# eglrp/PSBA

Measured on AMD Instinct MI355X. Metric: M-observations/sec through Jacobian+Schur build+solve (ms/LM-iter in ms_per_step), higher is better.
Workload: dtype f64; 1 GPU; venice-shaped; n_cams=52, n_pts=64053, n_obs=345364, lm=levmar, TR hand-off disabled, parallelism=points sharded x1

## Files before the change

include/psba_hip.h:

```cpp
#ifndef PSBA_HIP_H
#define PSBA_HIP_H

#ifdef __cplusplus
extern "C" {
#endif

typedef struct psba_ctx *psba_handle;

#define PSBA_OK 0
#define PSBA_NOT_SPD 1
#define PSBA_SINGULAR_V 2
#define PSBA_PCG_MAXIT 4
#define PSBA_E_INVALID (-1)
#define PSBA_E_HIP (-2)
#define PSBA_E_RCCL (-3)
#define PSBA_E_IO (-4)
#define PSBA_E_NOMEM (-5)
#define PSBA_E_STATE (-6)

#define PSBA_ITER_TURN_TO_LM 1
#define PSBA_ITER_TURN_TO_TR 2
#define PSBA_ITER_CONTINUE 3
#define PSBA_ITER_ERR 4
#define PSBA_ITER_DP_NO_CHANGE 5
#define PSBA_ITER_ERR_SMALL_ENOUGH 6
#define PSBA_ITER_PASS 7

#define PSBA_PARAMS_CUR 0
#define PSBA_PARAMS_NEW 1

int psba_create(int device, psba_handle *out);
int psba_destroy(psba_handle h);
const char *psba_last_error(psba_handle h);
const char *psba_version(void);

int psba_upload_problem(psba_handle h, int nCams, int n3Dpts, int n2Dprojs, const double *Kparas,
                        const double *impts, const double *initrot, const double *camsEx,
                        const double *pts3D, const int *iidx, const int *jidx);
int psba_set_params(psba_handle h, const double *camsEx, const double *pts3D);
int psba_reset_params(psba_handle h);
int psba_get_params(psba_handle h, int which, double *camsEx, double *pts3D);
int psba_get_dims(psba_handle h, int *nCams, int *n3Dpts, int *n2Dprojs);

#define PSBA_CAMERA_FIXED_K 0
#define PSBA_CAMERA_FREE_K 1
#define PSBA_CAMERA_FREE_KD 2
int psba_set_camera_model(psba_handle h, int model);
int psba_camera_block(psba_handle h, int *cnp);

int psba_set_intrinsics_mask(psba_handle h, const unsigned char free10[10]);
int psba_intrinsics_mask(psba_handle h, unsigned char out10[10]);

int psba_set_distortion(psba_handle h, const double *kc);
int psba_set_obs_covariance(psba_handle h, const double *cov);
int psba_lens_model(psba_handle h, int *has_distortion, int *has_covariance);

#define PSBA_LOSS_NONE 0
#define PSBA_LOSS_HUBER 1
#define PSBA_LOSS_CAUCHY 2
#define PSBA_LOSS_SOFT_L1 3
int psba_set_robust_loss(psba_handle h, int kind, double scale);
int psba_robust_loss(psba_handle h, int *kind, double *scale);
int psba_obs_sq_residuals(psba_handle h, int which, double *s);

int psba_set_fixed(psba_handle h, const unsigned char *fixed_cams, const unsigned char *fixed_pts);
int psba_fixed_counts(psba_handle h, int *n_fixed_cams, int *n_fixed_pts);
int psba_schur_path(psba_handle h, int *path);


int psba_residual(psba_handle h, int which, double *cost);
int psba_linearize(psba_handle h, double coeff, double coeff_g);
int psba_max_diag(psba_handle h, double *out);
int psba_begin(psba_handle h, double coeff, double coeff_g, double *cost, double *max_diag);
int psba_schur_assemble(psba_handle h, double mu);
int psba_schur_reduce(psba_handle h);
int psba_schur_solve(psba_handle h);

typedef struct {
  int status;
  double dp_l2;
  double gain_den;
  double new_cost;
  double newp_l2;
} psba_try_scalars;

int psba_backsub(psba_handle h, double mu, psba_try_scalars *out);
int psba_backsub_async(psba_handle h, double mu);
int psba_linearize_ahead(psba_handle h);
int psba_backsub_wait(psba_handle h, psba_try_scalars *out);
int psba_accept(psba_handle h);

int psba_compute_exQT(psba_handle h, int which, double *ex);
int psba_compute_jacobiQT(psba_handle h, double *jac_A, double *jac_B);
int psba_compute_U(psba_handle h, double coeff, double *out);
int psba_compute_V(psba_handle h, double coeff, double *out);
int psba_maxElmOfUV(psba_handle h, double *out);
int psba_update_UV(psba_handle h, double mu, double *U, double *V);
int psba_restore_UVdiag(psba_handle h);
int psba_compute_Vinv(psba_handle h, double *Vinv );
int psba_compute_Wblks(psba_handle h, double coeff, double *Wblks);
int psba_compute_Yblks(psba_handle h, double *Yblks);
int psba_compute_S(psba_handle h, double *S );
int psba_compute_g(psba_handle h, double coeff, double *g);
int psba_compute_ea(psba_handle h, double *ea);
int psba_SPDinv_matVec(psba_handle h, double *dpa);
int psba_compute_eb(psba_handle h, double *eb );
int psba_compute_dpb(psba_handle h, double *dp );
int psba_compute_newp(psba_handle h, double *new_p );
int psba_update_p(psba_handle h, double *p );

typedef struct {
  int max_iter;
  int tr_handoff;
  int verbose;
  int log_cap;
  int start_itno;
  double init_mu;
  double stop_cost;
} psba_lm_options;

typedef struct {
  int flag;
  int iters;
  int tries;
  double init_err, final_err, mu0, mu_final;
  int n_log;
  double seconds;
  int pcg_unconverged;
} psba_lm_result;

void psba_lm_default_options(psba_lm_options *o);
int psba_levmar(psba_handle h, const psba_lm_options *opts, psba_lm_result *res, double *log);

int psba_compute_Jmultiply(psba_handle h, const double *x, double *Jmul);
int psba_jmul_dots(psba_handle h, const double *x1, const double *x2, double dots[3]);
int psba_allreduce_scalars(psba_handle h, double *v, int n);
int psba_get_gradient(psba_handle h, double *g);
int psba_get_dp(psba_handle h, double *dp);
int psba_set_step(psba_handle h, const double *dp);
int psba_cholmod_lambda(psba_handle h, int reassemble, double *lambda, double *info3);

typedef struct {
  int max_iter;
  int start_itno;
  int verbose;
  int log_cap;
  double init_lambda;
} psba_tr_options;

typedef struct {
  int flag;
  int iters;
  int tries;
  int chol_fail;
  double init_err, final_err, lambda, delta;
  int n_log;
  double seconds;
} psba_tr_result;

void psba_tr_default_options(psba_tr_options *o);
int psba_trust_region(psba_handle h, const psba_tr_options *opts, psba_tr_result *res, double *log);

typedef struct {
  int flag, iters, lm_calls, tr_calls;
  double init_err, final_err, seconds;
} psba_solve_result;
int psba_solve(psba_handle h, int max_iter, int verbose, psba_solve_result *res);

int psba_partition_points(int n3Dpts, const int *iidx, int n2Dprojs, int nranks, int *pt_begin);
int psba_comm_unique_id(void *id128);
int psba_comm_init(psba_handle h, int nranks, int rank, const void *id128);
int psba_comm_rank(psba_handle h, int *nranks, int *rank);
int psba_set_rank_layout(psba_handle h, int nranks, int rank);
int psba_reduce_buffer_size(psba_handle h, long long *n_doubles);
int psba_get_reduce_buffer(psba_handle h, double *out);
int psba_set_reduce_buffer(psba_handle h, const double *in);

typedef struct {
  int nCams, n3Dpts, n2Dprojs;
  double *Kparas, *impts, *initrot, *camsEx, *pts3D;
  int *iidx, *jidx;
} psba_problem;
int psba_read_problem(const char *cams_file, const char *pts_file, const double *fixedK,
                      psba_problem *out);
void psba_free_problem(psba_problem *p);
typedef struct {
  psba_problem base;
  double *kc, *cov;
} psba_problem_ex;
int psba_read_problem_ex(const char *cams_file, const char *pts_file, const double *fixedK, psba_problem_ex *out);
void psba_free_problem_ex(psba_problem_ex *p);
int psba_write_problem(const char *cams_file, const char *pts_file, int nCams, int n3Dpts, int n2Dprojs,
                       const double *Kparas, const double *initrot, const double *camsEx, const double *pts3D,
                       const double *impts, const int *iidx, const int *jidx, int with_K);
int psba_convert_bal(const char *bal_file, const char *cams_out, const char *pts_out, double *max_abs_k);
int psba_convert_bal_kd(const char *bal_file, const char *cams_out, const char *pts_out);

#define PSBA_K_LINEARIZE 0
#define PSBA_K_SCHUR 1
#define PSBA_K_CHOLESKY 2
#define PSBA_K_BACKSUB 3
#define PSBA_K_RESIDUAL 4
#define PSBA_K_ALLREDUCE 5
#define PSBA_K_SCHUR_REDUCE 6
#define PSBA_K_COUNT 7
int psba_profile_enable(psba_handle h, int on);
int psba_profile_reset(psba_handle h);
int psba_profile_get(psba_handle h, int kernel, double *total_ms, int *launches);
int psba_algorithmic_bytes(psba_handle h, int kernel, double *bytes);

#define PSBA_SOLVER_DENSE 0
#define PSBA_SOLVER_PCG 1
int psba_set_solver(psba_handle h, int solver, double tol, int max_iter);
int psba_pcg_info(psba_handle h, int *iters, double *relres, long long *blocks, long long *dense_blocks);
int psba_get_sparse_S(psba_handle h, int *jk, double *val, double *ea);
int psba_set_sparse_S(psba_handle h, const double *val, const double *ea);
int psba_sparse_pattern(int nCams, int n3Dpts, int n2Dprojs, const int *iidx, const int *jidx, unsigned char *flags);
int psba_set_sparse_pattern(psba_handle h, const unsigned char *flags, long long n);

int psba_chol_dist_shape(psba_handle h, int *n32, int *NB, int *sharded);
int psba_chol_shape(psba_handle h, int *out8);
int psba_chol_dist_exchange_plan(int n32, int NB, int nranks, int JE, long long *out4, int cap);
int psba_chol_dist_begin(psba_handle h);
int psba_chol_dist_superpanel(psba_handle h, int J);
int psba_chol_dist_block(psba_handle h, int B, int set, double *buf, long long *n_doubles);
int psba_chol_dist_finish(psba_handle h);

typedef struct psba_schur_plan *psba_schur_plan_t;
psba_schur_plan_t psba_schur_plan_create(int nCams, int n3Dpts, int n2Dprojs, const int *iidx,
                                         const int *jidx);
int psba_schur_plan_info(psba_schur_plan_t p, long long info[8]);
int psba_schur_plan_copy(psba_schur_plan_t p, unsigned long long *items, long long *wg,
                         int *blockpos, int *glo);
void psba_schur_plan_destroy(psba_schur_plan_t p);

typedef struct psba_owner_plan *psba_owner_plan_t;
psba_owner_plan_t psba_owner_plan_create(int nCams, int n3Dpts, int n2Dprojs, const int *iidx, const int *jidx,
                                         const unsigned char *pattern);
int psba_owner_plan_info(psba_owner_plan_t p, long long info[4]);
int psba_owner_plan_copy(psba_owner_plan_t p, long long *waves, int *units, int *prod, int *blocks, int *diag_slot);
void psba_owner_plan_destroy(psba_owner_plan_t p);

typedef struct psba_blockprod_plan *psba_blockprod_plan_t;
// ... 21 lines not shown
```

psba_amd/build.py:

```python
import os
import subprocess
import sys

HERE = os.path.dirname(os.path.abspath(__file__))
CSRC = os.path.join(HERE, "csrc")
SOURCES = ["psba_api.cpp", "schur_plan.cpp", "lm_loop.cpp", "tr_loop.cpp", "sba_io.cpp", "kernels_linearize.hip",
           "kernels_tr.hip",
           "kernels_schur.hip", "kernels_freek.hip", "kernels_freekd.hip", "blockprod_plan.cpp", "kernels_chol.hip", "kernels_pcg.hip", "kernels_chol_graph.hip", "kernels_backsub.hip"]
EXPERIMENTS = bool(os.environ.get("PSBA_BUILD_EXPERIMENTS"))
if EXPERIMENTS:
    SOURCES += ["kernels_schur_ring.hip", "schur_ring_plan.cpp", "kernels_schur_modes.hip"]
OUT = os.path.join(HERE, "libpsba_hip_exp.so" if EXPERIMENTS else "libpsba_hip.so")
HEADERS = ["psba_internal.h", "dev_buf.h", "camera_model.h", "chol_factor32.h", "schur_common.h", "schur_lds_args.h", os.path.join("..", "..", "include", "psba_hip.h")]
ROCM = os.environ.get("ROCM_PATH", "/opt/rocm")
FLAGS = ["--offload-arch=gfx950", "-O3", "-std=c++17", "-fPIC", "-munsafe-fp-atomics",
         "-Wall", "-Wno-unused-result", "-x", "hip"] + (["-DPSBA_BUILD_EXPERIMENTS"] if EXPERIMENTS else [])


def _stale(obj, deps):
    if not os.path.exists(obj):
        return True
    t = os.path.getmtime(obj)
    return any(os.path.getmtime(d) > t for d in deps)


def build(force=False, verbose=False):
    hipcc = os.path.join(ROCM, "bin", "hipcc")
    objdir = os.path.join(HERE, "build_exp" if EXPERIMENTS else "build")
    os.makedirs(objdir, exist_ok=True)
    hdrs = [os.path.normpath(os.path.join(CSRC, h)) for h in HEADERS]
    objs, rebuilt = [], False
    for s in SOURCES:
        src = os.path.join(CSRC, s)
        obj = os.path.join(objdir, s + ".o")
        objs.append(obj)
        if force or _stale(obj, [src] + hdrs):
            cmd = [hipcc] + FLAGS + ["-c", src, "-o", obj]
            if verbose:
                print(" ".join(cmd), flush=True)
            subprocess.check_call(cmd)
            rebuilt = True
    if rebuilt or not os.path.exists(OUT):
        cmd = [hipcc, "--offload-arch=gfx950", "-shared", "-fPIC", "-o", OUT] + objs + [
            "-L" + os.path.join(ROCM, "lib"), "-lrccl", "-Wl,-rpath," + os.path.join(ROCM, "lib")]
        if verbose:
            print(" ".join(cmd), flush=True)
        subprocess.check_call(cmd)
    return OUT


if __name__ == "__main__":
    print(build(force="--force" in sys.argv, verbose=True))
```

psba_amd/capi.py:

```python
import ctypes as C
import os

import numpy as np

_HERE = os.path.dirname(os.path.abspath(__file__))
lib_path = os.environ.get("PSBA_LIB") or os.path.join(_HERE, "libpsba_hip.so")

if not os.path.exists(lib_path):
    raise ImportError(
        f"{lib_path} is missing: build the HIP extension first (python -m psba_amd.build, or "
        "__graft_entry__.build()). psba_amd has no CPU fallback.")
lib = C.CDLL(lib_path)

PSBA_OK, PSBA_NOT_SPD, PSBA_SINGULAR_V = 0, 1, 2
PARAMS_CUR, PARAMS_NEW = 0, 1
LOSS_NONE, LOSS_HUBER, LOSS_CAUCHY, LOSS_SOFT_L1 = 0, 1, 2, 3
CAMERA_FIXED_K, CAMERA_FREE_K, CAMERA_FREE_KD = 0, 1, 2
INTRINSICS_BAL = (1, 0, 0, 0, 0, 1, 1, 0, 0, 0)
ITER_TURN_TO_LM, ITER_TURN_TO_TR, ITER_CONTINUE, ITER_ERR = 1, 2, 3, 4
ITER_DP_NO_CHANGE, ITER_ERR_SMALL_ENOUGH, ITER_PASS = 5, 6, 7
K_LINEARIZE, K_SCHUR, K_CHOLESKY, K_BACKSUB, K_RESIDUAL, K_ALLREDUCE, K_SCHUR_REDUCE = range(7)
KERNEL_NAMES = ["linearize", "schur", "cholesky", "backsub", "residual", "allreduce", "schur_reduce"]

_h = C.c_void_p
_dp = C.POINTER(C.c_double)
_ip = C.POINTER(C.c_int)


class TryScalars(C.Structure):
    _fields_ = [("status", C.c_int), ("dp_l2", C.c_double), ("gain_den", C.c_double),
                ("new_cost", C.c_double), ("newp_l2", C.c_double)]


class LmOptions(C.Structure):
    _fields_ = [("max_iter", C.c_int), ("tr_handoff", C.c_int), ("verbose", C.c_int),
                ("log_cap", C.c_int), ("start_itno", C.c_int), ("init_mu", C.c_double),
                ("stop_cost", C.c_double)]


class LmResult(C.Structure):
    _fields_ = [("flag", C.c_int), ("iters", C.c_int), ("tries", C.c_int), ("init_err", C.c_double),
                ("final_err", C.c_double), ("mu0", C.c_double), ("mu_final", C.c_double),
                ("n_log", C.c_int), ("seconds", C.c_double), ("pcg_unconverged", C.c_int)]


class TrOptions(C.Structure):
    _fields_ = [("max_iter", C.c_int), ("start_itno", C.c_int), ("verbose", C.c_int), ("log_cap", C.c_int),
                ("init_lambda", C.c_double)]


class TrResult(C.Structure):
    _fields_ = [("flag", C.c_int), ("iters", C.c_int), ("tries", C.c_int), ("chol_fail", C.c_int),
                ("init_err", C.c_double), ("final_err", C.c_double), ("lambda_", C.c_double),
                ("delta", C.c_double), ("n_log", C.c_int), ("seconds", C.c_double)]


class SolveResult(C.Structure):
    _fields_ = [("flag", C.c_int), ("iters", C.c_int), ("lm_calls", C.c_int), ("tr_calls", C.c_int),
                ("init_err", C.c_double), ("final_err", C.c_double), ("seconds", C.c_double)]


class CProblem(C.Structure):
    _fields_ = [("nCams", C.c_int), ("n3Dpts", C.c_int), ("n2Dprojs", C.c_int), ("Kparas", _dp),
                ("impts", _dp), ("initrot", _dp), ("camsEx", _dp), ("pts3D", _dp), ("iidx", _ip),
                ("jidx", _ip)]


class CProblemEx(C.Structure):
    _fields_ = [("base", CProblem), ("kc", _dp), ("cov", _dp)]


SIGNATURES = [
    ("psba_create", C.c_int, [C.c_int, C.POINTER(_h)]),
    ("psba_destroy", C.c_int, [_h]),
    ("psba_last_error", C.c_char_p, [_h]),
    ("psba_version", C.c_char_p, []),
    ("psba_upload_problem", C.c_int, [_h, C.c_int, C.c_int, C.c_int, _dp, _dp, _dp, _dp, _dp, _ip, _ip]),
    ("psba_set_params", C.c_int, [_h, _dp, _dp]),
    ("psba_reset_params", C.c_int, [_h]),
    ("psba_get_params", C.c_int, [_h, C.c_int, _dp, _dp]),
    ("psba_get_dims", C.c_int, [_h, _ip, _ip, _ip]),
    ("psba_schur_path", C.c_int, [_h, C.POINTER(C.c_int)]),
    ("psba_residual", C.c_int, [_h, C.c_int, _dp]),
    ("psba_linearize", C.c_int, [_h, C.c_double, C.c_double]),
    ("psba_max_diag", C.c_int, [_h, _dp]),
    ("psba_begin", C.c_int, [_h, C.c_double, C.c_double, _dp, _dp]),
    ("psba_schur_assemble", C.c_int, [_h, C.c_double]),
    ("psba_schur_reduce", C.c_int, [_h]),
    ("psba_schur_solve", C.c_int, [_h]),
    ("psba_backsub", C.c_int, [_h, C.c_double, C.POINTER(TryScalars)]),
    ("psba_backsub_async", C.c_int, [_h, C.c_double]),
    ("psba_linearize_ahead", C.c_int, [_h]),
    ("psba_backsub_wait", C.c_int, [_h, C.POINTER(TryScalars)]),
    ("psba_accept", C.c_int, [_h]),
    ("psba_compute_exQT", C.c_int, [_h, C.c_int, _dp]),
    ("psba_compute_jacobiQT", C.c_int, [_h, _dp, _dp]),
    ("psba_compute_U", C.c_int, [_h, C.c_double, _dp]),
    ("psba_compute_V", C.c_int, [_h, C.c_double, _dp]),
    ("psba_maxElmOfUV", C.c_int, [_h, _dp]),
    ("psba_update_UV", C.c_int, [_h, C.c_double, _dp, _dp]),
    ("psba_restore_UVdiag", C.c_int, [_h]),
    ("psba_compute_Vinv", C.c_int, [_h, _dp]),
    ("psba_compute_Wblks", C.c_int, [_h, C.c_double, _dp]),
    ("psba_compute_Yblks", C.c_int, [_h, _dp]),
    ("psba_compute_S", C.c_int, [_h, _dp]),
    ("psba_compute_g", C.c_int, [_h, C.c_double, _dp]),
    ("psba_compute_ea", C.c_int, [_h, _dp]),
    ("psba_SPDinv_matVec", C.c_int, [_h, _dp]),
    ("psba_compute_eb", C.c_int, [_h, _dp]),
    ("psba_compute_dpb", C.c_int, [_h, _dp]),
    ("psba_compute_newp", C.c_int, [_h, _dp]),
    ("psba_update_p", C.c_int, [_h, _dp]),
    ("psba_lm_default_options", None, [C.POINTER(LmOptions)]),
    ("psba_levmar", C.c_int, [_h, C.POINTER(LmOptions), C.POINTER(LmResult), _dp]),
    ("psba_partition_points", C.c_int, [C.c_int, _ip, C.c_int, C.c_int, _ip]),
    ("psba_comm_unique_id", C.c_int, [C.c_void_p]),
    ("psba_comm_init", C.c_int, [_h, C.c_int, C.c_int, C.c_void_p]),
    ("psba_comm_rank", C.c_int, [_h, _ip, _ip]),
    ("psba_set_rank_layout", C.c_int, [_h, C.c_int, C.c_int]),
    ("psba_reduce_buffer_size", C.c_int, [_h, C.POINTER(C.c_longlong)]),
    ("psba_get_reduce_buffer", C.c_int, [_h, _dp]),
    ("psba_set_reduce_buffer", C.c_int, [_h, _dp]),
    ("psba_read_problem", C.c_int, [C.c_char_p, C.c_char_p, _dp, C.POINTER(CProblem)]),
    ("psba_free_problem", None, [C.POINTER(CProblem)]),
    ("psba_profile_enable", C.c_int, [_h, C.c_int]),
    ("psba_profile_reset", C.c_int, [_h]),
    ("psba_profile_get", C.c_int, [_h, C.c_int, _dp, _ip]),
    ("psba_algorithmic_bytes", C.c_int, [_h, C.c_int, _dp]),
    ("psba_compute_Jmultiply", C.c_int, [_h, _dp, _dp]),
    ("psba_jmul_dots", C.c_int, [_h, _dp, _dp, _dp]),
    ("psba_get_gradient", C.c_int, [_h, _dp]),
    ("psba_get_dp", C.c_int, [_h, _dp]),
    ("psba_set_step", C.c_int, [_h, _dp]),
    ("psba_cholmod_lambda", C.c_int, [_h, C.c_int, _dp, _dp]),
    ("psba_tr_default_options", None, [C.POINTER(TrOptions)]),
    ("psba_trust_region", C.c_int, [_h, C.POINTER(TrOptions), C.POINTER(TrResult), _dp]),
    ("psba_solve", C.c_int, [_h, C.c_int, C.c_int, C.POINTER(SolveResult)]),
    ("psba_write_problem", C.c_int, [C.c_char_p, C.c_char_p, C.c_int, C.c_int, C.c_int, _dp, _dp, _dp, _dp, _dp, _ip, _ip, C.c_int]),
    ("psba_convert_bal", C.c_int, [C.c_char_p, C.c_char_p, C.c_char_p, _dp]),
    ("psba_allreduce_scalars", C.c_int, [_h, _dp, C.c_int]),
    ("psba_set_solver", C.c_int, [_h, C.c_int, C.c_double, C.c_int]),
    ("psba_pcg_info", C.c_int, [_h, _ip, _dp, C.POINTER(C.c_longlong), C.POINTER(C.c_longlong)]),
    ("psba_get_sparse_S", C.c_int, [_h, _ip, _dp, _dp]),
    ("psba_set_sparse_S", C.c_int, [_h, _dp, _dp]),
    ("psba_sparse_pattern", C.c_int, [C.c_int, C.c_int, C.c_int, _ip, _ip, C.POINTER(C.c_ubyte)]),
    ("psba_set_sparse_pattern", C.c_int, [_h, C.POINTER(C.c_ubyte), C.c_longlong]),
    ("psba_set_camera_model", C.c_int, [_h, C.c_int]),
    ("psba_camera_block", C.c_int, [_h, _ip]),
    ("psba_set_distortion", C.c_int, [_h, _dp]),
    ("psba_set_obs_covariance", C.c_int, [_h, _dp]),
    ("psba_lens_model", C.c_int, [_h, _ip, _ip]),
    ("psba_set_robust_loss", C.c_int, [_h, C.c_int, C.c_double]),
    ("psba_robust_loss", C.c_int, [_h, _ip, _dp]),
    ("psba_obs_sq_residuals", C.c_int, [_h, C.c_int, _dp]),
    ("psba_set_fixed", C.c_int, [_h, C.POINTER(C.c_ubyte), C.POINTER(C.c_ubyte)]),
    ("psba_fixed_counts", C.c_int, [_h, _ip, _ip]),
    ("psba_read_problem_ex", C.c_int, [C.c_char_p, C.c_char_p, _dp, C.POINTER(CProblemEx)]),
    ("psba_free_problem_ex", None, [C.POINTER(CProblemEx)]),
    ("psba_convert_bal_kd", C.c_int, [C.c_char_p, C.c_char_p, C.c_char_p]),
    ("psba_chol_dist_exchange_plan", C.c_int, [C.c_int, C.c_int, C.c_int, C.c_int, C.POINTER(C.c_longlong), C.c_int]),
    ("psba_chol_dist_shape", C.c_int, [_h, _ip, _ip, _ip]),
    ("psba_chol_shape", C.c_int, [_h, _ip]),
    ("psba_chol_dist_begin", C.c_int, [_h]),
    ("psba_chol_dist_superpanel", C.c_int, [_h, C.c_int]),
    ("psba_chol_dist_block", C.c_int, [_h, C.c_int, C.c_int, _dp, C.POINTER(C.c_longlong)]),
    ("psba_chol_dist_finish", C.c_int, [_h]),
    ("psba_schur_plan_create", C.c_void_p, [C.c_int, C.c_int, C.c_int, _ip, _ip]),
    ("psba_schur_plan_info", C.c_int, [C.c_void_p, C.POINTER(C.c_longlong)]),
    ("psba_schur_plan_copy", C.c_int, [C.c_void_p, C.POINTER(C.c_ulonglong), C.POINTER(C.c_longlong), _ip, _ip]),
    ("psba_schur_plan_destroy", None, [C.c_void_p]),
    ("psba_owner_plan_create", C.c_void_p, [C.c_int, C.c_int, C.c_int, _ip, _ip, C.POINTER(C.c_ubyte)]),
    ("psba_owner_plan_info", C.c_int, [C.c_void_p, C.POINTER(C.c_longlong)]),
    ("psba_owner_plan_copy", C.c_int, [C.c_void_p, C.POINTER(C.c_longlong), _ip, _ip, _ip, _ip]),
    ("psba_owner_plan_destroy", None, [C.c_void_p]),
    ("psba_set_intrinsics_mask", C.c_int, [_h, C.POINTER(C.c_ubyte)]),
    ("psba_intrinsics_mask", C.c_int, [_h, C.POINTER(C.c_ubyte)]),
    ("psba_blockprod_plan_create", C.c_void_p, [C.c_int, C.c_int, C.c_int, _ip, _ip, C.c_int]),
    ("psba_blockprod_plan_info", C.c_int, [C.c_void_p, C.POINTER(C.c_longlong)]),
    ("psba_blockprod_plan_copy", C.c_int, [C.c_void_p, _ip, _ip, _ip]),
    ("psba_blockprod_plan_destroy", None, [C.c_void_p]),
]
EXPERIMENT_SIGNATURES = [
    ("psba_ring_plan_create", C.c_void_p, [C.c_int, C.c_int, C.c_int, _ip, _ip]),
    ("psba_ring_plan_info", C.c_int, [C.c_void_p, C.POINTER(C.c_longlong)]),
    ("psba_ring_plan_copy", C.c_int, [C.c_void_p, C.POINTER(C.c_longlong), _ip, C.POINTER(C.c_uint), _ip, _ip, _ip, _ip, _ip]),
    ("psba_ring_plan_destroy", None, [C.c_void_p]),
]
HAS_EXPERIMENTS = hasattr(lib, "psba_ring_plan_create")
for _name, _res, _args in SIGNATURES + (EXPERIMENT_SIGNATURES if HAS_EXPERIMENTS else []):
    _f = getattr(lib, _name)
    _f.restype = _res
    _f.argtypes = _args


class PsbaError(RuntimeError):
    def __init__(self, code, msg):
        super().__init__(f"psba error {code}: {msg}")
        self.code = code


def _d(a):
    return None if a is None else a.ctypes.data_as(_dp)


def _i(a):
    return None if a is None else a.ctypes.data_as(_ip)


def _c(a, dt=np.float64):
    return np.ascontiguousarray(a, dtype=dt)


class Problem(dict):
    """K[nC,5] initrot[nC,4] cams[nC,6] pts[nP,3] impts[nO,2] iidx[nO] jidx[nO] nC nP nO.
    Optional: kc[nC,5], cov[nO,2,2] (read_problem_ex); fixed_cams[nC], fixed_pts[nP] (masks for Psba.set_fixed)."""


def sparse_pattern(prob):
    nC = int(prob["nC"])
    flags = np.zeros(nC * (nC + 1) // 2, dtype=np.uint8)
    ii = np.ascontiguousarray(prob["iidx"], dtype=np.int32)
    jj = np.ascontiguousarray(prob["jidx"], dtype=np.int32)
    rc = lib.psba_sparse_pattern(nC, int(prob["nP"]), int(prob["nO"]), _i(ii), _i(jj),
                                 flags.ctypes.data_as(C.POINTER(C.c_ubyte)))
    if rc != 0:
        raise PsbaError(rc, "psba_sparse_pattern failed")
    return flags


def _problem_from(cp):
    nC, nP, nO = cp.nCams, cp.n3Dpts, cp.n2Dprojs
    arr = lambda p, n, shape: np.ctypeslib.as_array(p, shape=(n,)).copy().reshape(shape)
    return Problem(K=arr(cp.Kparas, 5 * nC, (nC, 5)), initrot=arr(cp.initrot, 4 * nC, (nC, 4)),
                  cams=arr(cp.camsEx, 6 * nC, (nC, 6)), pts=arr(cp.pts3D, 3 * nP, (nP, 3)),
                  impts=arr(cp.impts, 2 * nO, (nO, 2)), iidx=arr(cp.iidx, nO, (nO,)).astype(np.int32),
                  jidx=arr(cp.jidx, nO, (nO,)).astype(np.int32), nC=nC, nP=nP, nO=nO)


def read_problem(cams_file, pts_file, fixedK=None):
    cp = CProblem()
    k = None if fixedK is None else _c(fixedK)
    rc = lib.psba_read_problem(os.fsencode(cams_file), os.fsencode(pts_file), _d(k), C.byref(cp))
    if rc != 0:
        raise PsbaError(rc, f"psba_read_problem({cams_file}, {pts_file}) failed")
    out = _problem_from(cp)
    lib.psba_free_problem(C.byref(cp))
    return out
# ... 186 lines not shown
            self._h = _h()

    def __del__(self):
        try:
            self.close()
        except Exception:
            pass

    def _ck(self, rc):
        if rc < 0:
            raise PsbaError(rc, lib.psba_last_error(self._h).decode())
        return rc

    def set_camera_model(self, model):
        self._ck(lib.psba_set_camera_model(self._h, int(model)))

    def set_intrinsics_mask(self, free=None):
        if free is None:
            return self._ck(lib.psba_set_intrinsics_mask(self._h, None))
        m = np.ascontiguousarray((np.asarray(free).reshape(-1) != 0).astype(np.uint8))
        if m.size != 10:
            raise PsbaError(-1, f"set_intrinsics_mask: {m.size} flags for 10 intrinsics")
        self._ck(lib.psba_set_intrinsics_mask(self._h, m.ctypes.data_as(C.POINTER(C.c_ubyte))))

    def intrinsics_mask(self):
        m = np.zeros(10, dtype=np.uint8)
        self._ck(lib.psba_intrinsics_mask(self._h, m.ctypes.data_as(C.POINTER(C.c_ubyte))))
        return tuple(int(v) for v in m)

    def set_distortion(self, kc):
        k = None if kc is None else _c(kc).reshape(-1)
        if k is not None and k.size != 5 * self.nC:
            raise PsbaError(-1, f"set_distortion: {k.size} values for {self.nC} cameras (5 each)")
        self._ck(lib.psba_set_distortion(self._h, _d(k)))

    def set_obs_covariance(self, cov):
        c = None if cov is None else _c(cov).reshape(-1)
        if c is not None and c.size != 4 * self.nO:
            raise PsbaError(-1, f"set_obs_covariance: {c.size} values for {self.nO} observations (4 each)")
        self._ck(lib.psba_set_obs_covariance(self._h, _d(c)))

    def lens_model(self):
        d, c = C.c_int(), C.c_int()
        self._ck(lib.psba_lens_model(self._h, C.byref(d), C.byref(c)))
        return bool(d.value), bool(c.value)

    def set_robust_loss(self, kind, scale=1.0):
        self._ck(lib.psba_set_robust_loss(self._h, int(kind), float(scale)))

    def robust_loss(self):
        k, c = C.c_int(), C.c_double()
        self._ck(lib.psba_robust_loss(self._h, C.byref(k), C.byref(c)))
        return k.value, c.value

    def set_fixed(self, cams=None, pts=None):
        def mask(a, n, what):
            if a is None:
                return None
            m = (np.asarray(a).reshape(-1) != 0).astype(np.uint8)
            if m.size != n:
                raise PsbaError(-1, f"set_fixed: {m.size} flags for {n} {what}")
            return np.ascontiguousarray(m)
        c, p = mask(cams, self.nC, "cameras"), mask(pts, self.nP, "points")
        ub = C.POINTER(C.c_ubyte)
        self._ck(lib.psba_set_fixed(self._h, None if c is None else c.ctypes.data_as(ub),
                                    None if p is None else p.ctypes.data_as(ub)))

    def fixed_counts(self):
        c, p = C.c_int(), C.c_int()
        self._ck(lib.psba_fixed_counts(self._h, C.byref(c), C.byref(p)))
        return c.value, p.value

    def obs_sq_residuals(self, which=PARAMS_CUR):
        return self._out(lib.psba_obs_sq_residuals, self.nO, which)[1]

    def camera_block(self):
        n = C.c_int()
        self._ck(lib.psba_camera_block(self._h, C.byref(n)))
        return n.value

    def upload_problem(self, prob):
        self.nC, self.nP, self.nO = int(prob["nC"]), int(prob["nP"]), int(prob["nO"])
        self.cnp = self.camera_block()
        self.nA, self.nB = self.cnp * self.nC, 3 * self.nP
        self.nT = self.nA + self.nB
        a = [_c(prob[k]).reshape(-1) for k in ("K", "impts", "initrot", "cams", "pts")]
        ii, jj = _c(prob["iidx"], np.int32), _c(prob["jidx"], np.int32)
        self._ck(lib.psba_upload_problem(self._h, self.nC, self.nP, self.nO, _d(a[0]), _d(a[1]),
                                         _d(a[2]), _d(a[3]), _d(a[4]), _i(ii), _i(jj)))

    def set_params(self, cams, pts):
        c, p = _c(cams).reshape(-1), _c(pts).reshape(-1)
        self._ck(lib.psba_set_params(self._h, _d(c), _d(p)))

    def reset_params(self):
        self._ck(lib.psba_reset_params(self._h))

    def get_params(self, which=PARAMS_CUR):
        c, p = np.empty(self.nA), np.empty(self.nB)
        self._ck(lib.psba_get_params(self._h, which, _d(c), _d(p)))
        return c.reshape(self.nC, self.cnp), p.reshape(self.nP, 3)

    def schur_path(self):
        v = C.c_int()
        self._ck(lib.psba_schur_path(self._h, C.byref(v)))
        return v.value

    def residual(self, which=PARAMS_CUR):
        v = C.c_double()
        self._ck(lib.psba_residual(self._h, which, C.byref(v)))
        return v.value

    def linearize(self, coeff=1.0, coeff_g=1.0):
        self._ck(lib.psba_linearize(self._h, coeff, coeff_g))

    def begin(self, coeff=1.0, coeff_g=1.0):
        c, m = C.c_double(), C.c_double()
        self._ck(lib.psba_begin(self._h, coeff, coeff_g, C.byref(c), C.byref(m)))
        return c.value, m.value

    def max_diag(self):
        v = C.c_double()
        self._ck(lib.psba_max_diag(self._h, C.byref(v)))
        return v.value

    def schur_assemble(self, mu):
        self._ck(lib.psba_schur_assemble(self._h, mu))

    def schur_reduce(self):
        self._ck(lib.psba_schur_reduce(self._h))

    def schur_solve(self):
        return self._ck(lib.psba_schur_solve(self._h))

    def backsub(self, mu):
        s = TryScalars()
        self._ck(lib.psba_backsub(self._h, mu, C.byref(s)))
        return s

    def backsub_async(self, mu):
        self._ck(lib.psba_backsub_async(self._h, mu))

    def linearize_ahead(self):
        self._ck(lib.psba_linearize_ahead(self._h))

    def backsub_wait(self):
        s = TryScalars()
        self._ck(lib.psba_backsub_wait(self._h, C.byref(s)))
        return s

    def accept(self):
        self._ck(lib.psba_accept(self._h))

    def _out(self, fn, n, *pre):
        out = np.empty(n)
        rc = self._ck(fn(self._h, *pre, _d(out)))
        return rc, out

    def compute_exQT(self, which=PARAMS_CUR):
        return self._out(lib.psba_compute_exQT, 2 * self.nO, which)[1]

    def compute_jacobiQT(self):
        JA, JB = np.empty(12 * self.nO), np.empty(6 * self.nO)
        self._ck(lib.psba_compute_jacobiQT(self._h, _d(JA), _d(JB)))
        return JA, JB

    def compute_U(self, coeff=1.0):
        return self._out(lib.psba_compute_U, 36 * self.nC, coeff)[1]

    def compute_V(self, coeff=1.0):
        return self._out(lib.psba_compute_V, 9 * self.nP, coeff)[1]

    def maxElmOfUV(self):
        v = C.c_double()
        self._ck(lib.psba_maxElmOfUV(self._h, C.byref(v)))
        return v.value

    def update_UV(self, mu):
        U, V = np.empty(36 * self.nC), np.empty(9 * self.nP)
        self._ck(lib.psba_update_UV(self._h, mu, _d(U), _d(V)))
        return U, V

    def restore_UVdiag(self):
        self._ck(lib.psba_restore_UVdiag(self._h))

    def compute_Vinv(self):
        return self._out(lib.psba_compute_Vinv, 9 * self.nP)

    def compute_Wblks(self, coeff=1.0):
        return self._out(lib.psba_compute_Wblks, 18 * self.nO, coeff)[1]

    def compute_Yblks(self):
        return self._out(lib.psba_compute_Yblks, 18 * self.nO)[1]

    def compute_S(self):
        return self._out(lib.psba_compute_S, self.nA * self.nA)[1].reshape(self.nA, self.nA)

    def compute_g(self, coeff=1.0):
        return self._out(lib.psba_compute_g, self.nT, coeff)[1]

    def compute_ea(self):
        return self._out(lib.psba_compute_ea, self.nA)[1]

    def SPDinv_matVec(self):
        return self._out(lib.psba_SPDinv_matVec, self.nA)

    def compute_eb(self):
        return self._out(lib.psba_compute_eb, self.nB)[1]

    def compute_dpb(self):
        return self._out(lib.psba_compute_dpb, self.nT)[1]

    def compute_newp(self):
        return self._out(lib.psba_compute_newp, self.nT)[1]

    def update_p(self):
        return self._out(lib.psba_update_p, self.nT)[1]

    def levmar(self, max_iter=50, tr_handoff=False, verbose=False, log_cap=512, start_itno=0, init_mu=0.0,
               stop_cost=0.0):
        opts = LmOptions(max_iter, int(tr_handoff), int(verbose), log_cap, start_itno, init_mu, stop_cost)
        res = LmResult()
        log = np.zeros((max(log_cap, 1), 5))
        self._ck(lib.psba_levmar(self._h, C.byref(opts), C.byref(res), _d(log)))
        return res, log[: res.n_log].copy()

    def set_solver(self, solver, tol=0.0, max_iter=0):
        self._ck(lib.psba_set_solver(self._h, int(solver), float(tol), int(max_iter)))

    def pcg_info(self):
        it, rr, nb, nd = C.c_int(), C.c_double(), C.c_longlong(), C.c_longlong()
        self._ck(lib.psba_pcg_info(self._h, C.byref(it), C.byref(rr), C.byref(nb), C.byref(nd)))
        return it.value, rr.value, nb.value, nd.value

    def get_sparse_S(self):
        nb = self.pcg_info()[2]
        jk = np.empty((nb, 2), dtype=np.int32)
        val = np.empty((nb, 6, 6))
        ea = np.empty(6 * self.nC)
        self._ck(lib.psba_get_sparse_S(self._h, _i(jk), _d(val), _d(ea)))
        return jk, val, ea

    def set_sparse_S(self, val, ea):
        val = np.ascontiguousarray(val, dtype=np.float64)
        ea = np.ascontiguousarray(ea, dtype=np.float64)
        self._ck(lib.psba_set_sparse_S(self._h, _d(val), _d(ea)))

    def set_sparse_pattern(self, flags):
        flags = np.ascontiguousarray(flags, dtype=np.uint8)
        self._ck(lib.psba_set_sparse_pattern(self._h, flags.ctypes.data_as(C.POINTER(C.c_ubyte)), flags.size))

    def chol_dist_shape(self):
        n32, nb, sh = C.c_int(), C.c_int(), C.c_int()
        self._ck(lib.psba_chol_dist_shape(self._h, C.byref(n32), C.byref(nb), C.byref(sh)))
        return n32.value, nb.value, bool(sh.value)

    def chol_shape(self):
        out = (C.c_int * 8)()
        self._ck(lib.psba_chol_shape(self._h, out))
        keys = ("n32", "fused", "fused2", "blocked", "NB", "diag_only", "lookahead", "single")
        return {k: (int(v) if k in ("n32", "NB") else bool(v)) for k, v in zip(keys, out)}

    def chol_dist_begin(self):
        self._ck(lib.psba_chol_dist_begin(self._h))

    def chol_dist_superpanel(self, J):
        self._ck(lib.psba_chol_dist_superpanel(self._h, int(J)))

    def chol_dist_get_block(self, B):
        n = C.c_longlong()
        self._ck(lib.psba_chol_dist_block(self._h, int(B), 0, None, C.byref(n)))
        buf = np.empty(n.value)
        self._ck(lib.psba_chol_dist_block(self._h, int(B), 0, _d(buf), C.byref(n)))
        return buf

    def chol_dist_set_block(self, B, buf):
        n = C.c_longlong()
        self._ck(lib.psba_chol_dist_block(self._h, int(B), 1, _d(_c(buf)), C.byref(n)))

    def chol_dist_finish(self):
        self._ck(lib.psba_chol_dist_finish(self._h))

    def compute_Jmultiply(self, x):
        return self._out(lambda h, out: lib.psba_compute_Jmultiply(h, _d(_c(x)), out), 2 * self.nO)[1]

    def jmul_dots(self, x1, x2=None):
        out = np.empty(3)
        a1 = _c(x1)
        a2 = None if x2 is None else _c(x2)
        self._ck(lib.psba_jmul_dots(self._h, _d(a1), _d(a2), _d(out)))
        return out

    def get_gradient(self):
        return self._out(lib.psba_get_gradient, self.nT)[1]

    def get_dp(self):
        return self._out(lib.psba_get_dp, self.nT)[1]

    def set_step(self, dp):
        self._ck(lib.psba_set_step(self._h, _d(_c(dp))))

    def cholmod_lambda(self, reassemble=True):
        lam, info = C.c_double(), np.empty(3)
        self._ck(lib.psba_cholmod_lambda(self._h, int(reassemble), C.byref(lam), _d(info)))
        return lam.value, info

# ... 58 lines not shown
```

psba_amd/csrc/kernels_linearize.hip:

```cpp
#include <cstdlib>

#include "camera_model.h"
#include "psba_internal.h"

namespace psba {

struct LinArgs {
  const double *camconst, *cams, *pts, *impts;
  const int *iidx, *jidx, *ptr;
  const int4 *tile_desc;
  double *W, *PV, *campart;
  double *camacc;
  double *dbg_ex, *dbg_JA, *dbg_JB;
  double coeff, coeff_g;
  int nC, nTiles;
  int mode;
  const double *pub_src;
  double *pub_dst;
  double pub_stamp;
  const double *kc, *wl;
};

template <bool DUMP, bool GACC, int LM>
__global__ __launch_bounds__(TILE_OBS) void k_linearize(LinArgs p, RobustLoss rl, FixedMask fm) {
  __shared__ double sBE[TILE_OBS][9];
  __shared__ double sW[(TILE_OBS / 2) * 19];
  extern __shared__ double sAcc[];
  const int tid = threadIdx.x;
  if (p.pub_dst && blockIdx.x == 0) {
    if (tid < NSCAL) p.pub_dst[tid] = p.pub_src[tid];
    __threadfence_system();
    __syncthreads();
    if (tid == 0) p.pub_dst[NSCAL] = p.pub_stamp;
  }
  const int nAcc = GACC ? 0 : p.nC * CAM_ACC;
  for (int t = tid; t < nAcc; t += TILE_OBS) sAcc[t] = 0.0;
  __syncthreads();

  int tile = blockIdx.x;
  int4 dsc = tile < p.nTiles ? p.tile_desc[tile] : make_int4(0, 0, 0, 0);
  int i = 0, j = 0;
  if (dsc.z + tid < dsc.w) {
    i = p.iidx[dsc.z + tid];
    j = p.jidx[dsc.z + tid];
  }
  for (; tile < p.nTiles; tile += gridDim.x) {
    const int p0 = dsc.x, p1 = dsc.y, o0 = dsc.z, o1 = dsc.w;
    const int a = o0 + tid;
    const int tn = tile + gridDim.x;
    const int4 dn = tn < p.nTiles ? p.tile_desc[tn] : make_int4(0, 0, 0, 0);
    constexpr int NTASK = (9 * TILE_PTS + TILE_OBS - 1) / TILE_OBS;
    int pb[NTASK][2];
#pragma unroll
    for (int u = 0; u < NTASK; u++) {
      const int ip = (tid + u * TILE_OBS) / 9;
      pb[u][0] = ip < p1 - p0 ? p.ptr[p0 + ip] - o0 : 0;
      pb[u][1] = ip < p1 - p0 ? p.ptr[p0 + ip + 1] - o0 : 0;
    }
    double Wv[18];
    if (a < o1) {
      double cc[9], cam[6], M[3], e[2], A[12], B[6], kc[5], wl[3];
#pragma unroll
      for (int k = 0; k < 9; k++) cc[k] = p.camconst[9 * j + k];
#pragma unroll
      for (int k = 0; k < 6; k++) cam[k] = p.cams[6 * j + k];
#pragma unroll
      for (int k = 0; k < 3; k++) M[k] = p.pts[3 * i + k];
      lens_load_kc<LM>(p.kc, j, kc);
      lens_load_w<LM>(p.wl, a, wl);
      const double2 m = reinterpret_cast<const double2 *>(p.impts)[a];
      lens_linearize<LM>(cc, cam, M, kc, wl, rl, m.x, m.y, e, A, B);
      fix_mask<LM>(fix_load<LM>(fm, i, j), A, B);
      if (DUMP) {
        p.dbg_ex[2 * a] = e[0];
        p.dbg_ex[2 * a + 1] = e[1];
#pragma unroll
        for (int k = 0; k < 12; k++) p.dbg_JA[12 * (size_t)a + k] = A[k];
#pragma unroll
        for (int k = 0; k < 6; k++) p.dbg_JB[6 * (size_t)a + k] = B[k];
      }
#pragma unroll
      for (int r = 0; r < 6; r++)
#pragma unroll
        for (int c = 0; c < 3; c++) Wv[3 * r + c] = p.coeff * (A[r] * B[c] + A[6 + r] * B[3 + c]);
      if (tid < TILE_OBS / 2) {
        double *w = sW + 19 * tid;
#pragma unroll
        for (int k = 0; k < 18; k++) w[k] = Wv[k];
      }
#pragma unroll
      for (int k = 0; k < 6; k++) sBE[tid][k] = B[k];
      sBE[tid][6] = e[0];
      sBE[tid][7] = e[1];
      double *acc = sAcc + CAM_ACC * (size_t)j;
      int k = 0;
      if (p.mode != 1 && !GACC) {
#pragma unroll
      for (int r = 0; r < 6; r++)
#pragma unroll
        for (int c = r; c < 6; c++) atomicAdd(&acc[k++], A[r] * A[c] + A[6 + r] * A[6 + c]);
#pragma unroll
      for (int r = 0; r < 6; r++) atomicAdd(&acc[21 + r], A[r] * e[0] + A[6 + r] * e[1]);
      }
    }
    __syncthreads();
    if (p.mode != 2) {
      double *dst = p.W + 18 * (size_t)o0;
      const int n = 18 * (o1 - o0 < TILE_OBS / 2 ? o1 - o0 : TILE_OBS / 2);
      for (int t = tid; t < n; t += TILE_OBS) dst[t] = sW[19 * (t / 18) + t % 18];
    }
#pragma unroll
    for (int u = 0; u < NTASK; u++) {
      const int t = tid + u * TILE_OBS;
      if (t >= 9 * (p1 - p0) || p.mode == 3) continue;
      const int comp = t % 9;
      const int b0 = pb[u][0], b1 = pb[u][1];
      int r, c1, c2;
      if (comp < 6) {
        r = comp < 3 ? 0 : (comp < 5 ? 1 : 2);
        const int c = comp < 3 ? comp : (comp < 5 ? comp - 2 : 2);
        c1 = c;
        c2 = 3 + c;
      } else {
        r = comp - 6;
        c1 = 6;
        c2 = 7;
      }
      double acc = 0.0;
      for (int b = b0; b < b1; b++) {
        const double *B = sBE[b];
        acc += B[r] * B[c1] + B[3 + r] * B[c2];
      }
      p.PV[9 * (size_t)p0 + t] = (comp < 6 ? p.coeff : p.coeff_g) * acc;
    }
    if (o1 - o0 > TILE_OBS / 2) {
      __syncthreads();
      if (tid >= TILE_OBS / 2 && a < o1) {
        double *w = sW + 19 * (tid - TILE_OBS / 2);
#pragma unroll
        for (int k = 0; k < 18; k++) w[k] = Wv[k];
      }
      __syncthreads();
      if (p.mode != 2) {
        double *dst = p.W + 18 * (size_t)(o0 + TILE_OBS / 2);
        const int n = 18 * (o1 - o0 - TILE_OBS / 2);
        for (int t = tid; t < n; t += TILE_OBS) dst[t] = sW[19 * (t / 18) + t % 18];
      }
    }
    dsc = dn;
    i = j = 0;
    if (dsc.z + tid < dsc.w) {
      i = p.iidx[dsc.z + tid];
      j = p.jidx[dsc.z + tid];
    }
    __syncthreads();
  }
  if (GACC) return;
  double *slab = p.campart + (size_t)blockIdx.x * nAcc;
  for (int t = tid; t < nAcc; t += TILE_OBS) slab[t] = sAcc[t];
}

template <bool DUMP, bool GACC, int LM>
__global__ __launch_bounds__(TILE_OBS) void k_linearize2(LinArgs p, RobustLoss rl, FixedMask fm) {
  __shared__ double sW[TILE_OBS * 19];
  __shared__ double sCarV[TILE_OBS / 64][9];
  __shared__ int sCarP[TILE_OBS / 64][3];
  extern __shared__ double sAcc[];
  const int tid = threadIdx.x, lane = tid & 63, wave = tid >> 6;
  if (p.pub_dst && blockIdx.x == 0) {
    if (tid < NSCAL) p.pub_dst[tid] = p.pub_src[tid];
    __threadfence_system();
    __syncthreads();
    if (tid == 0) p.pub_dst[NSCAL] = p.pub_stamp;
  }
  const int nAcc = GACC ? 0 : p.nC * CAM_ACC;
  for (int t = tid; t < nAcc; t += TILE_OBS) sAcc[t] = 0.0;
  __syncthreads();

  int tile = blockIdx.x;
  int4 dsc = tile < p.nTiles ? p.tile_desc[tile] : make_int4(0, 0, 0, 0);
  int i = 0, j = 0;
  double cc[9], cam[6], M[3], kc[5], wl[3];
  double2 m = make_double2(0.0, 0.0);
  int fx = 0;
  if (dsc.z + tid < dsc.w) {
    i = p.iidx[dsc.z + tid];
    j = p.jidx[dsc.z + tid];
    fx = fix_load<LM>(fm, i, j);
#pragma unroll
    for (int k = 0; k < 9; k++) cc[k] = p.camconst[9 * j + k];
#pragma unroll
    for (int k = 0; k < 6; k++) cam[k] = p.cams[6 * j + k];
#pragma unroll
    for (int k = 0; k < 3; k++) M[k] = p.pts[3 * (size_t)i + k];
    lens_load_kc<LM>(p.kc, j, kc);
    lens_load_w<LM>(p.wl, dsc.z + tid, wl);
    m = reinterpret_cast<const double2 *>(p.impts)[dsc.z + tid];
  }
  for (; tile < p.nTiles; tile += gridDim.x) {
    const int o0 = dsc.z, o1 = dsc.w;
    const int a = o0 + tid;
    const bool act = a < o1;
    const int tn = tile + gridDim.x;
    const int4 dn = tn < p.nTiles ? p.tile_desc[tn] : make_int4(0, 0, 0, 0);
    double v[9];
#pragma unroll
    for (int k = 0; k < 9; k++) v[k] = 0.0;
    const int pi = act ? i : -1 - tid;
    const int jc = j;
    if (act) {
      double e[2], A[12], B[6];
      lens_linearize<LM>(cc, cam, M, kc, wl, rl, m.x, m.y, e, A, B);
      fix_mask<LM>(fx, A, B);
      if (DUMP) {
        p.dbg_ex[2 * (size_t)a] = e[0];
        p.dbg_ex[2 * (size_t)a + 1] = e[1];
#pragma unroll
        for (int k = 0; k < 12; k++) p.dbg_JA[12 * (size_t)a + k] = A[k];
#pragma unroll
        for (int k = 0; k < 6; k++) p.dbg_JB[6 * (size_t)a + k] = B[k];
      }
      double *w = sW + 19 * tid;
#pragma unroll
      for (int r = 0; r < 6; r++)
#pragma unroll
        for (int c = 0; c < 3; c++) w[3 * r + c] = p.coeff * (A[r] * B[c] + A[6 + r] * B[3 + c]);
      int q = 0;
#pragma unroll
      for (int r = 0; r < 3; r++)
#pragma unroll
        for (int c = r; c < 3; c++) v[q++] = B[r] * B[c] + B[3 + r] * B[3 + c];
#pragma unroll
      for (int r = 0; r < 3; r++) v[6 + r] = B[r] * e[0] + B[3 + r] * e[1];
      if (p.mode != 1 && !GACC) {
        double *acc = sAcc + CAM_ACC * (size_t)jc;
        int k = 0;
#pragma unroll
        for (int r = 0; r < 6; r++)
#pragma unroll
          for (int c = r; c < 6; c++) atomicAdd(&acc[k++], A[r] * A[c] + A[6 + r] * A[6 + c]);
#pragma unroll
        for (int r = 0; r < 6; r++) atomicAdd(&acc[21 + r], A[r] * e[0] + A[6 + r] * e[1]);
      }
    }
    i = j = 0;
    if (dn.z + tid < dn.w) {
      i = p.iidx[dn.z + tid];
      j = p.jidx[dn.z + tid];
      fx = fix_load<LM>(fm, i, j);
#pragma unroll
      for (int k = 0; k < 9; k++) cc[k] = p.camconst[9 * j + k];
#pragma unroll
      for (int k = 0; k < 6; k++) cam[k] = p.cams[6 * j + k];
#pragma unroll
      for (int k = 0; k < 3; k++) M[k] = p.pts[3 * (size_t)i + k];
      lens_load_kc<LM>(p.kc, j, kc);
      lens_load_w<LM>(p.wl, dn.z + tid, wl);
      m = reinterpret_cast<const double2 *>(p.impts)[dn.z + tid];
    }
    if (p.mode != 3) {
#pragma unroll
      for (int d = 1; d < 64; d <<= 1) {
        const int pu = __shfl_up(pi, d, 64);
        const bool ok = lane >= d && pu == pi;
        if (!__any(ok)) break;
#pragma unroll
        for (int k = 0; k < 9; k++) {
          const double vu = __shfl_up(v[k], d, 64);
          v[k] += ok ? vu : 0.0;
        }
      }
    }
    const int pn = __shfl_down(pi, 1, 64);
    const int p_first = __shfl(pi, 0, 64), p_last = __shfl(pi, 63, 64);
    if (lane == 63) {
#pragma unroll
      for (int k = 0; k < 9; k++) sCarV[wave][k] = v[k];
      sCarP[wave][0] = p_first;
      sCarP[wave][1] = p_last;
      sCarP[wave][2] = p_first == p_last;
    }
    __syncthreads();
    if (p.mode != 2) {
      double *dst = p.W + 18 * (size_t)o0;
      const int n = 18 * (o1 - o0);
      for (int t = tid; t < n; t += TILE_OBS) dst[t] = sW[19 * (t / 18) + t % 18];
    }
    if (act && p.mode != 3) {
      const bool cont = lane == 63 && wave + 1 < TILE_OBS / 64 && sCarP[wave + 1][0] == pi;
      const bool tail = lane == 63 ? !cont : pn != pi;
      if (tail) {
        if (pi == p_first) {
          for (int w2 = wave - 1; w2 >= 0 && sCarP[w2][1] == pi; w2--) {
#pragma unroll
            for (int k = 0; k < 9; k++) v[k] += sCarV[w2][k];
            if (!sCarP[w2][2]) break;
          }
        }
        double *pv = p.PV + 9 * (size_t)pi;
#pragma unroll
        for (int k = 0; k < 9; k++) pv[k] = (k < 6 ? p.coeff : p.coeff_g) * v[k];
      }
    }
    dsc = dn;
    __syncthreads();
  }
  if (GACC) return;
  double *slab = p.campart + (size_t)blockIdx.x * nAcc;
  for (int t = tid; t < nAcc; t += TILE_OBS) slab[t] = sAcc[t];
}

template <bool DUMP, bool GACC, int LM>
__global__ __launch_bounds__(TILE_OBS) void k_linearize_long(LinArgs p, const int *long_pts, double *cam_slab, RobustLoss rl, FixedMask fm) {
  __shared__ double sRed[TILE_OBS / 64][9];
  const int tid = threadIdx.x, i = long_pts[blockIdx.x];
  const int o0 = p.ptr[i], o1 = p.ptr[i + 1];
  double M[3], acc[9];
#pragma unroll
  for (int k = 0; k < 3; k++) M[k] = p.pts[3 * (size_t)i + k];
#pragma unroll
  for (int k = 0; k < 9; k++) acc[k] = 0.0;
  for (int a = o0 + tid; a < o1; a += TILE_OBS) {
    const int j = p.jidx[a];
    double cc[9], cam[6], e[2], A[12], B[6], kc[5], wl[3];
#pragma unroll
    for (int k = 0; k < 9; k++) cc[k] = p.camconst[9 * (size_t)j + k];
#pragma unroll
    for (int k = 0; k < 6; k++) cam[k] = p.cams[6 * (size_t)j + k];
    lens_load_kc<LM>(p.kc, j, kc);
    lens_load_w<LM>(p.wl, a, wl);
    const double2 m = reinterpret_cast<const double2 *>(p.impts)[a];
    lens_linearize<LM>(cc, cam, M, kc, wl, rl, m.x, m.y, e, A, B);
    fix_mask<LM>(fix_load<LM>(fm, i, j), A, B);
    if (DUMP) {
      p.dbg_ex[2 * (size_t)a] = e[0];
      p.dbg_ex[2 * (size_t)a + 1] = e[1];
#pragma unroll
      for (int k = 0; k < 12; k++) p.dbg_JA[12 * (size_t)a + k] = A[k];
#pragma unroll
      for (int k = 0; k < 6; k++) p.dbg_JB[6 * (size_t)a + k] = B[k];
    }
    double *w = p.W + 18 * (size_t)a;
#pragma unroll
    for (int r = 0; r < 6; r++)
#pragma unroll
      for (int c = 0; c < 3; c++) w[3 * r + c] = p.coeff * (A[r] * B[c] + A[6 + r] * B[3 + c]);
    int k = 0;
#pragma unroll
    for (int r = 0; r < 3; r++)
#pragma unroll
      for (int c = r; c < 3; c++) acc[k++] += B[r] * B[c] + B[3 + r] * B[3 + c];
#pragma unroll
    for (int r = 0; r < 3; r++) acc[6 + r] += B[r] * e[0] + B[3 + r] * e[1];
    if (!GACC) {
      double *cs = cam_slab + CAM_ACC * (size_t)j;
      int q = 0;
#pragma unroll
      for (int r = 0; r < 6; r++)
#pragma unroll
        for (int c = r; c < 6; c++) atomicAdd(&cs[q++], A[r] * A[c] + A[6 + r] * A[6 + c]);
#pragma unroll
      for (int r = 0; r < 6; r++) atomicAdd(&cs[21 + r], A[r] * e[0] + A[6 + r] * e[1]);
    }
  }
#pragma unroll
  for (int k = 0; k < 9; k++) {
    double v = acc[k];
#pragma unroll
    for (int off = 32; off > 0; off >>= 1) v += __shfl_down(v, off, 64);
    if ((tid & 63) == 0) sRed[tid >> 6][k] = v;
  }
  __syncthreads();
  if (tid < 9) {
    double v = 0.0;
    for (int q = 0; q < TILE_OBS / 64; q++) v += sRed[q][tid];
    p.PV[9 * (size_t)i + tid] = (tid < 6 ? p.coeff : p.coeff_g) * v;
  }
}

template <int LM>
__global__ __launch_bounds__(256) void k_cam_sums(LinArgs p, const int *cam_obs, const int4 *units, int nUnits, RobustLoss rl, FixedMask fm) {
  const int lane = threadIdx.x & 63;
  const int u = blockIdx.x * 4 + (threadIdx.x >> 6);
  if (u >= nUnits) return;
  const int4 un = units[u];
  const int j = un.x;
  double cc[9], cam[6], acc[CAM_ACC], kc[5];
#pragma unroll
  for (int k = 0; k < 9; k++) cc[k] = p.camconst[9 * (size_t)j + k];
#pragma unroll
  for (int k = 0; k < 6; k++) cam[k] = p.cams[6 * (size_t)j + k];
  lens_load_kc<LM>(p.kc, j, kc);
#pragma unroll
  for (int k = 0; k < CAM_ACC; k++) acc[k] = 0.0;
  for (int t = un.y + lane; t < un.z; t += 64) {
    const int a = cam_obs[t];
    const int i = p.iidx[a];
    double M[3], e[2], A[12], B[6], wl[3];
#pragma unroll
    for (int k = 0; k < 3; k++) M[k] = p.pts[3 * (size_t)i + k];
    lens_load_w<LM>(p.wl, a, wl);
    const double2 m = reinterpret_cast<const double2 *>(p.impts)[a];
    lens_linearize<LM>(cc, cam, M, kc, wl, rl, m.x, m.y, e, A, B);
    fix_mask<LM>(fix_load<LM>(fm, i, j), A, B);
    int k = 0;
#pragma unroll
    for (int r = 0; r < 6; r++)
#pragma unroll
      for (int c = r; c < 6; c++) acc[k++] += A[r] * A[c] + A[6 + r] * A[6 + c];
#pragma unroll
    for (int r = 0; r < 6; r++) acc[21 + r] += A[r] * e[0] + A[6 + r] * e[1];
  }
#pragma unroll
  for (int k = 0; k < CAM_ACC; k++) {
#pragma unroll
    for (int d = 32; d >= 1; d >>= 1) acc[k] += __shfl_down(acc[k], d, 64);
  }
  if (lane) return;
  double *dst = p.camacc + CAM_ACC * (size_t)j;
#pragma unroll
  for (int k = 0; k < CAM_ACC; k++) atomicAdd(&dst[k], acc[k]);
}

__global__ __launch_bounds__(256) void k_cam_finalize(const double *camacc, int nC, double coeff, double coeff_g,
                                                      double *U, double *ga) {
  const int t = blockIdx.x * blockDim.x + threadIdx.x;
  if (t >= 42 * nC) return;
  const int j = t / 42, e = t % 42;
  const double *src = camacc + (size_t)j * CAM_ACC;
  if (e < 36) {
    const int r = e / 6, c = e % 6;
    const int lo = r < c ? r : c, hi = r < c ? c : r;
    U[36 * (size_t)j + e] = coeff * src[lo * 6 - lo * (lo - 1) / 2 + (hi - lo)];
  } else {
    ga[6 * (size_t)j + e - 36] = coeff_g * src[21 + e - 36];
  }
}

__global__ __launch_bounds__(1024) void k_cam_reduce(const double *campart, int nPart, int nC,
                                                     double coeff, double coeff_g, double *U,
                                                     double *ga) {
  __shared__ double sPart[32][33];
  const int j = blockIdx.x, e = threadIdx.x & 31, s = threadIdx.x >> 5;
  double acc = 0.0;
  if (e < CAM_ACC) {
    const double *src = campart + (size_t)j * CAM_ACC + e;
    const size_t stride = (size_t)nC * CAM_ACC;
    int q = s;
    for (; q + 96 < nPart; q += 128) {
      const double x0 = src[(size_t)q * stride], x1 = src[(size_t)(q + 32) * stride];
      const double x2 = src[(size_t)(q + 64) * stride], x3 = src[(size_t)(q + 96) * stride];
      acc += x0;
      acc += x1;
      acc += x2;
      acc += x3;
    }
    for (; q < nPart; q += 32) acc += src[(size_t)q * stride];
  }
  sPart[s][e] = acc;
  __syncthreads();
  if (s == 0 && e < CAM_ACC) {
    double t = sPart[0][e];
    for (int q = 1; q < 32; q++) t += sPart[q][e];
    sPart[0][e] = t;
  }
  __syncthreads();
  if (threadIdx.x < 36) {
    const int r = threadIdx.x / 6, c = threadIdx.x % 6;
    const int lo = r < c ? r : c, hi = r < c ? c : r;
    const int k = lo * 6 - lo * (lo - 1) / 2 + (hi - lo);
    U[36 * j + threadIdx.x] = coeff * sPart[0][k];
  } else if (threadIdx.x < 42) {
    ga[6 * j + threadIdx.x - 36] = coeff_g * sPart[0][21 + threadIdx.x - 36];
  }
}

__global__ __launch_bounds__(256) void k_fixed_diag(FixedMask fm, int nC, int nP, double coeff, double cam_diag, double *U,
                                                    double *ga, double *PV) {
  const int t = blockIdx.x * blockDim.x + threadIdx.x;
  if (t < nC) {
    if (fm.cams && fm.cams[t]) {
      for (int e = 0; e < 36; e++) U[36 * (size_t)t + e] = (e % 7 == 0) ? cam_diag : 0.0;
      for (int e = 0; e < 6; e++) ga[6 * (size_t)t + e] = 0.0;
    }
  } else if (t - nC < nP) {
    const int i = t - nC;
    if (fm.pts && fm.pts[i]) {
      double *pv = PV + 9 * (size_t)i;
      pv[0] = coeff; pv[1] = 0.0; pv[2] = 0.0; pv[3] = coeff; pv[4] = 0.0; pv[5] = coeff;
      pv[6] = 0.0; pv[7] = 0.0; pv[8] = 0.0;
    }
  }
}

template <int LM>
__global__ __launch_bounds__(256) void k_residual(const double *camconst, const double *cams,
                                                  const double *pts, const double *impts,
                                                  const int *iidx, const int *jidx, int nO,
                                                  double *ex_out, double *cost, const double *kcs,
                                                  const double *wls, RobustLoss rl, double *s_out) {
  __shared__ double sRed[4];
  double sum = 0.0;
  for (int a = blockIdx.x * blockDim.x + threadIdx.x; a < nO; a += gridDim.x * blockDim.x) {
    const int i = iidx[a], j = jidx[a];
    double cc[9], cam[6], M[3], e0, e1, kc[5], wl[3];
#pragma unroll
    for (int k = 0; k < 9; k++) cc[k] = camconst[9 * j + k];
#pragma unroll
    for (int k = 0; k < 6; k++) cam[k] = cams[6 * j + k];
#pragma unroll
    for (int k = 0; k < 3; k++) M[k] = pts[3 * i + k];
    lens_load_kc<LM>(kcs, j, kc);
    lens_load_w<LM>(wls, a, wl);
    const double2 m = reinterpret_cast<const double2 *>(impts)[a];
    lens_residual<LM>(cc, cam, M, kc, wl, m.x, m.y, e0, e1);
    const double f = lens_cost<LM>(rl, e0, e1, s_out ? s_out + a : nullptr);
    if (ex_out) {
      ex_out[2 * a] = e0;
      ex_out[2 * a + 1] = e1;
    }
    sum += f;
  }
#pragma unroll
  for (int off = 32; off > 0; off >>= 1) sum += __shfl_down(sum, off, 64);
  if ((threadIdx.x & 63) == 0) sRed[threadIdx.x >> 6] = sum;
  __syncthreads();
  if (threadIdx.x == 0) atomicAdd(cost, sRed[0] + sRed[1] + sRed[2] + sRed[3]);
}

__global__ __launch_bounds__(256) void k_max_diag(const double *U, const double *PV, int nC,
                                                  int nP, double *out) {
  __shared__ double sRed[4];
  double m = 0.0;
  const int gtid = blockIdx.x * blockDim.x + threadIdx.x, gsize = gridDim.x * blockDim.x;
  for (int t = gtid; t < 6 * nC; t += gsize) m = fmax(m, U[36 * (t / 6) + 7 * (t % 6)]);
  for (int i = gtid; i < nP; i += gsize) {
    const double *v = PV + 9 * (size_t)i;
    m = fmax(m, fmax(v[0], fmax(v[3], v[5])));
  }
#pragma unroll
  for (int off = 32; off > 0; off >>= 1) m = fmax(m, __shfl_down(m, off, 64));
  if ((threadIdx.x & 63) == 0) sRed[threadIdx.x >> 6] = m;
  __syncthreads();
  if (threadIdx.x == 0) {
    m = fmax(fmax(sRed[0], sRed[1]), fmax(sRed[2], sRed[3]));
    atomicMax(reinterpret_cast<unsigned long long *>(out),
              (unsigned long long)__double_as_longlong(m));
  }
}

__global__ __launch_bounds__(256) void k_max_diag_fixed(const double *U, const double *PV, int nC, int nP, double *out,
                                                        FixedMask fm) {
  __shared__ double sRed[4];
  double m = 0.0;
  const int gtid = blockIdx.x * blockDim.x + threadIdx.x, gsize = gridDim.x * blockDim.x;
  for (int t = gtid; t < 6 * nC; t += gsize)
    if (!(fm.cams && fm.cams[t / 6])) m = fmax(m, U[36 * (t / 6) + 7 * (t % 6)]);
  for (int i = gtid; i < nP; i += gsize) {
    if (fm.pts && fm.pts[i]) continue;
    const double *v = PV + 9 * (size_t)i;
    m = fmax(m, fmax(v[0], fmax(v[3], v[5])));
  }
#pragma unroll
  for (int off = 32; off > 0; off >>= 1) m = fmax(m, __shfl_down(m, off, 64));
  if ((threadIdx.x & 63) == 0) sRed[threadIdx.x >> 6] = m;
  __syncthreads();
  if (threadIdx.x == 0) {
    m = fmax(fmax(sRed[0], sRed[1]), fmax(sRed[2], sRed[3]));
    atomicMax(reinterpret_cast<unsigned long long *>(out), (unsigned long long)__double_as_longlong(m));
  }
}

template <int LM>
static int set_lin_attrs(psba_ctx *h) {
  const auto attr = hipFuncAttributeMaxDynamicSharedMemorySize;
  PSBA_HIP(h, hipFuncSetAttribute((const void *)k_linearize<true, false, LM>, attr, 100 * 1024));
  PSBA_HIP(h, hipFuncSetAttribute((const void *)k_linearize<false, false, LM>, attr, 100 * 1024));
  PSBA_HIP(h, hipFuncSetAttribute((const void *)k_linearize2<true, false, LM>, attr, 100 * 1024));
  PSBA_HIP(h, hipFuncSetAttribute((const void *)k_linearize2<false, false, LM>, attr, 100 * 1024));
  return PSBA_OK;
}

template <int LM>
static void enqueue_linearize(psba_ctx *h, const LinArgs &a, const RobustLoss &rl, const FixedMask &fm, bool dump, bool v1, size_t lds, double *Uo, double *gao) {
  const Dims &d = h->d;
  if (h->cam_global) {
    const int grid = d.nTiles < 2048 ? d.nTiles : 2048;
    if (v1 && dump)
      hipLaunchKernelGGL((k_linearize<true, true, LM>), dim3(grid), dim3(TILE_OBS), 0, h->stream, a, rl, fm);
    else if (v1)
      hipLaunchKernelGGL((k_linearize<false, true, LM>), dim3(grid), dim3(TILE_OBS), 0, h->stream, a, rl, fm);
    else if (dump)
      hipLaunchKernelGGL((k_linearize2<true, true, LM>), dim3(grid), dim3(TILE_OBS), 0, h->stream, a, rl, fm);
    else
      hipLaunchKernelGGL((k_linearize2<false, true, LM>), dim3(grid), dim3(TILE_OBS), 0, h->stream, a, rl, fm);
    if (h->nLong) {
      if (dump)
        hipLaunchKernelGGL((k_linearize_long<true, true, LM>), dim3(h->nLong), dim3(TILE_OBS), 0, h->stream, a, h->long_pts, (double *)nullptr, rl, fm);
      else
        hipLaunchKernelGGL((k_linearize_long<false, true, LM>), dim3(h->nLong), dim3(TILE_OBS), 0, h->stream, a, h->long_pts, (double *)nullptr, rl, fm);
    }
    hipLaunchKernelGGL(k_cam_sums<LM>, dim3((h->nCamUnits + 3) / 4), dim3(256), 0, h->stream, a, h->cam_obs,
                       h->cam_units, h->nCamUnits, rl, fm);
    hipLaunchKernelGGL(k_cam_finalize, dim3((42 * d.nC + 255) / 256), dim3(256), 0, h->stream, h->camacc, d.nC,
                       h->coeff, h->coeff_g, Uo, gao);
  } else {
    if (v1 && dump)
      hipLaunchKernelGGL((k_linearize<true, false, LM>), dim3(h->nPart), dim3(TILE_OBS), lds, h->stream, a, rl, fm);
    else if (v1)
      hipLaunchKernelGGL((k_linearize<false, false, LM>), dim3(h->nPart), dim3(TILE_OBS), lds, h->stream, a, rl, fm);
    else if (dump)
      hipLaunchKernelGGL((k_linearize2<true, false, LM>), dim3(h->nPart), dim3(TILE_OBS), lds, h->stream, a, rl, fm);
    else
      hipLaunchKernelGGL((k_linearize2<false, false, LM>), dim3(h->nPart), dim3(TILE_OBS), lds, h->stream, a, rl, fm);
    int nslab = h->nPart;
    if (h->nLong) {
      double *slab = h->campart + (size_t)h->nPart * d.nC * CAM_ACC;
      if (dump)
        hipLaunchKernelGGL((k_linearize_long<true, false, LM>), dim3(h->nLong), dim3(TILE_OBS), 0, h->stream, a, h->long_pts, slab, rl, fm);
      else
        hipLaunchKernelGGL((k_linearize_long<false, false, LM>), dim3(h->nLong), dim3(TILE_OBS), 0, h->stream, a, h->long_pts, slab, rl, fm);
      nslab++;
    }
    hipLaunchKernelGGL(k_cam_reduce, dim3(d.nC), dim3(1024), 0, h->stream, h->campart, nslab, d.nC, h->coeff,
                       h->coeff_g, Uo, gao);
  }
}

int launch_linearize(psba_ctx *h, bool dump, bool ahead, bool publish) {
  if (h->cnp != 6) return dump ? fail(h, PSBA_E_STATE, "the sba_func.h mirror is six-parameter only (not PSBA_CAMERA_FREE_K / PSBA_CAMERA_FREE_KD)") : h->cnp == KD_CNP ? launch_linearize_kd(h, ahead, publish) : launch_linearize_fk(h, ahead, publish);
  const Dims &d = h->d;
  LinArgs a;
  a.camconst = h->camconst;
  const int set = ahead ? 1 - h->cur : h->cur;
  a.cams = h->cams[set];
  a.pts = h->pts[set];
  a.impts = h->impts;
  a.iidx = h->iidx;
  a.jidx = h->jidx;
  a.ptr = h->ptr;
  a.tile_desc = h->tile_desc;
  a.W = ahead ? h->W_alt : h->W;
  a.PV = ahead ? h->PV_alt : h->PV;
  a.campart = h->campart;
  a.camacc = h->camacc;
  a.dbg_ex = h->dbg_ex;
  a.dbg_JA = h->dbg_JA;
  a.dbg_JB = h->dbg_JB;
  a.coeff = h->coeff;
  h->coeff_w = h->coeff;
  a.coeff_g = h->coeff_g;
  a.nC = d.nC;
  a.nTiles = d.nTiles;
  a.pub_src = h->scal;
  a.pub_dst = publish ? h->h_scal_dev : nullptr;
  a.pub_stamp = h->pub_seq;
  a.kc = h->lens_kc;
  a.wl = h->lens_w;
  const RobustLoss rl = make_robust_loss(h->loss_kind, h->loss_c);
  const FixedMask fm = {h->fix_cams, h->fix_pts};
  {
    const char *m = getenv("PSBA_LIN_MODE");
    a.mode = m ? atoi(m) : 0;
  }
  const bool v1 = getenv("PSBA_LIN_V1") != nullptr;
  const size_t lds = h->cam_global ? 0 : sizeof(double) * CAM_ACC * (size_t)d.nC;
  if (!h->lin_attr_set && lds > 8 * 1024) {
    int rc = PSBA_OK;
    for (int lm = 0; lm < 2 * LENS_MODELS && rc == PSBA_OK; lm++)
      lens_dispatch_fixed(lm % LENS_MODELS, lm >= LENS_MODELS, [&](auto m) { rc = set_lin_attrs<decltype(m)::value>(h); });
    if (rc != PSBA_OK) return rc;
    h->lin_attr_set = true;
  }
  double *Uo = ahead ? h->U_alt : h->U, *gao = ahead ? h->ga_alt : h->ga;
  {
    ProfScope ps(h, PSBA_K_LINEARIZE);
    if (h->cam_global)
      PSBA_HIP(h, hipMemsetAsync(h->camacc, 0, sizeof(double) * CAM_ACC * (size_t)d.nC, h->stream));
    else if (h->nLong)
      PSBA_HIP(h, hipMemsetAsync(h->campart + (size_t)h->nPart * d.nC * CAM_ACC, 0, sizeof(double) * CAM_ACC * (size_t)d.nC,
                                 h->stream));
    lens_dispatch_fixed(h->lens, h->has_fixed, [&](auto m) { enqueue_linearize<decltype(m)::value>(h, a, rl, fm, dump, v1, lds, Uo, gao); });
    if (h->has_fixed)
      hipLaunchKernelGGL(k_fixed_diag, dim3((d.nC + d.nP + 255) / 256), dim3(256), 0, h->stream, fm, d.nC, d.nP, h->coeff,
                         h->rank == 0 ? h->coeff : 0.0, Uo, gao, a.PV);
  }
  PSBA_HIP(h, hipGetLastError());
  return PSBA_OK;
}

int launch_residual(psba_ctx *h, int which, double *ex_out_dev, double *s_out_dev) {
  if (h->cnp != 6) return ex_out_dev || s_out_dev ? fail(h, PSBA_E_STATE, "the sba_func.h mirror is six-parameter only (not PSBA_CAMERA_FREE_K / PSBA_CAMERA_FREE_KD)") : h->cnp == KD_CNP ? launch_residual_kd(h, which) : launch_residual_fk(h, which);
  const Dims &d = h->d;
  const int set = which == PSBA_PARAMS_NEW ? 1 - h->cur : h->cur;
  PSBA_HIP(h, hipMemsetAsync(h->scal + SC_COST, 0, sizeof(double), h->stream));
  int grid = (d.nO + 255) / 256;
  if (grid > 256) grid = 256;
  {
    ProfScope ps(h, PSBA_K_RESIDUAL);
    const RobustLoss rl = make_robust_loss(h->loss_kind, h->loss_c);
    lens_dispatch(h->lens | (s_out_dev ? LENS_ROBUST : 0), [&](auto m) {
      hipLaunchKernelGGL(k_residual<decltype(m)::value>, dim3(grid), dim3(256), 0, h->stream, h->camconst, h->cams[set],
                         h->pts[set], h->impts, h->iidx, h->jidx, d.nO, ex_out_dev, h->scal + SC_COST, h->lens_kc,
                         h->lens_w, rl, s_out_dev);
    });
  }
  PSBA_HIP(h, hipGetLastError());
  return PSBA_OK;
}

int launch_max_diag(psba_ctx *h) {
  if (h->cnp != 6) return h->cnp == KD_CNP ? launch_max_diag_kd(h) : launch_max_diag_fk(h);
  PSBA_HIP(h, hipMemsetAsync(h->scal + SC_MAXDIAG, 0, sizeof(double), h->stream));
  int grid = (h->d.nP + 255) / 256;
  if (grid > 512) grid = 512;
  if (h->has_fixed)
    hipLaunchKernelGGL(k_max_diag_fixed, dim3(grid), dim3(256), 0, h->stream, h->U, h->PV, h->d.nC, h->d.nP,
                       h->scal + SC_MAXDIAG, FixedMask{h->fix_cams, h->fix_pts});
  else
    hipLaunchKernelGGL(k_max_diag, dim3(grid), dim3(256), 0, h->stream, h->U, h->PV, h->d.nC, h->d.nP,
                       h->scal + SC_MAXDIAG);
  PSBA_HIP(h, hipGetLastError());
  return PSBA_OK;
}

}
```

psba_amd/csrc/kernels_schur.hip:

```cpp
#include "camera_model.h"
#include <cstdlib>

#include "schur_common.h"
#include "schur_lds_args.h"

namespace psba {

struct SchurArgs {
  const double *W, *PV;
  const int *iidx, *jidx, *ptr, *tile_pt;
  double *S, *ea;
  int *status;
  double *dbg_Y, *dbg_Vinv;
  double mu;
  int nC, nA, nTiles;
  int ld;
  int try_id;
};

template <bool DUMP>
__global__ __launch_bounds__(TILE_OBS) void k_schur_atomic(SchurArgs p) {
  __shared__ double sW[TILE_OBS * 18];
  __shared__ double sVi[TILE_OBS][9];
  __shared__ int sJ[TILE_OBS];
// ... 36 lines not shown
    __syncthreads();
    if (tid < nobs) {
      const int a = o0 + tid;
      const int i = p.iidx[a];
      const int ja = sJ[tid];
      const double *vi = sVi[i - p0];
      const double i00 = vi[0], i01 = vi[1], i02 = vi[2], i11 = vi[3], i12 = vi[4], i22 = vi[5];
      const double g0 = vi[6], g1 = vi[7], g2 = vi[8];
      double Y[18];
#pragma unroll
      for (int r = 0; r < 6; r++) {
        const double w0 = sW[18 * tid + 3 * r], w1 = sW[18 * tid + 3 * r + 1],
                     w2 = sW[18 * tid + 3 * r + 2];
        Y[3 * r] = w0 * i00 + w1 * i01 + w2 * i02;
        Y[3 * r + 1] = w0 * i01 + w1 * i11 + w2 * i12;
        Y[3 * r + 2] = w0 * i02 + w1 * i12 + w2 * i22;
        atomicAdd(&sEa[6 * ja + r], -(Y[3 * r] * g0 + Y[3 * r + 1] * g1 + Y[3 * r + 2] * g2));
      }
      if (DUMP) {
#pragma unroll
        for (int k = 0; k < 18; k++) p.dbg_Y[18 * (size_t)a + k] = Y[k];
      }
      const int b0 = p.ptr[i] - o0;
      for (int b = b0; b <= tid; b++) {
        const int jb = sJ[b];
        double *Sblk = p.S + (size_t)(6 * ja) * p.ld + 6 * jb;
        const double *wb = sW + 18 * b;
#pragma unroll
        for (int c = 0; c < 6; c++) {
          const double w0 = wb[3 * c], w1 = wb[3 * c + 1], w2 = wb[3 * c + 2];
#pragma unroll
          for (int r = 0; r < 6; r++)
            atomicAdd(&Sblk[(size_t)r * p.ld + c],
                      -(Y[3 * r] * w0 + Y[3 * r + 1] * w1 + Y[3 * r + 2] * w2));
        }
      }
    }
  }
  __syncthreads();
  for (int t = tid; t < p.nA; t += TILE_OBS)
    if (sEa[t] != 0.0) atomicAdd(&p.ea[t], sEa[t]);
}

template <bool DUMP>
__global__ __launch_bounds__(TILE_OBS) void k_schur_long(SchurArgs p, const int *long_pts) {
  const int tid = threadIdx.x, i = long_pts[blockIdx.x];
  const int o0 = p.ptr[i], o1 = p.ptr[i + 1];
  const double *pv = p.PV + 9 * (size_t)i;
  double v[6], vi[6];
#pragma unroll
  for (int k = 0; k < 6; k++) v[k] = pv[k];
  v[0] += p.mu;
  v[3] += p.mu;
  v[5] += p.mu;
  if (sym3_inverse(v, vi)) p.status[0] = p.try_id;
  const double g0 = pv[6], g1 = pv[7], g2 = pv[8];
  if (DUMP && tid == 0) {
    double *o = p.dbg_Vinv + 9 * (size_t)i;
    o[0] = vi[0]; o[1] = vi[1]; o[2] = vi[2];
    o[3] = vi[1]; o[4] = vi[3]; o[5] = vi[4];
    o[6] = vi[2]; o[7] = vi[4]; o[8] = vi[5];
  }
  for (int a = o0 + tid; a < o1; a += TILE_OBS) {
    const int ja = p.jidx[a];
    const double *w = p.W + 18 * (size_t)a;
    double Y[18];
#pragma unroll
    for (int r = 0; r < 6; r++) {
      const double w0 = w[3 * r], w1 = w[3 * r + 1], w2 = w[3 * r + 2];
      Y[3 * r] = w0 * vi[0] + w1 * vi[1] + w2 * vi[2];
      Y[3 * r + 1] = w0 * vi[1] + w1 * vi[3] + w2 * vi[4];
      Y[3 * r + 2] = w0 * vi[2] + w1 * vi[4] + w2 * vi[5];
      atomicAdd(&p.ea[6 * ja + r], -(Y[3 * r] * g0 + Y[3 * r + 1] * g1 + Y[3 * r + 2] * g2));
    }
    if (DUMP) {
#pragma unroll
      for (int k = 0; k < 18; k++) p.dbg_Y[18 * (size_t)a + k] = Y[k];
    }
    for (int b = o0; b <= a; b++) {
      double *Sblk = p.S + (size_t)(6 * ja) * p.ld + 6 * p.jidx[b];
      const double *wb = p.W + 18 * (size_t)b;
#pragma unroll
      for (int c = 0; c < 6; c++) {
        const double w0 = wb[3 * c], w1 = wb[3 * c + 1], w2 = wb[3 * c + 2];
#pragma unroll
        for (int r = 0; r < 6; r++)
          atomicAdd(&Sblk[(size_t)r * p.ld + c], -(Y[3 * r] * w0 + Y[3 * r + 1] * w1 + Y[3 * r + 2] * w2));
      }
    }
  }
}



template <bool DUMP>
__device__ __forceinline__ void schur_a_side(const SchurLdsArgs &p, int a, int i, double (&v)[6], double g0, double g1,
                                             double g2, const double (&w)[18], double (&Y)[18], double (&e)[6],
                                             bool dump_y) {
  double vi[6];
  v[0] += p.mu;
  v[3] += p.mu;
  v[5] += p.mu;
  if (sym3_inverse(v, vi)) p.status[0] = p.try_id;
  if (DUMP) {
    double *o = p.dbg_Vinv + 9 * (size_t)i;
    o[0] = vi[0]; o[1] = vi[1]; o[2] = vi[2];
    o[3] = vi[1]; o[4] = vi[3]; o[5] = vi[4];
    o[6] = vi[2]; o[7] = vi[4]; o[8] = vi[5];
  }
#pragma unroll
  for (int k = 0; k < 6; k++) vi[k] = -vi[k];
#pragma unroll
  for (int r = 0; r < 6; r++) {
    const double w0 = w[3 * r], w1 = w[3 * r + 1], w2 = w[3 * r + 2];
    Y[3 * r] = w0 * vi[0] + w1 * vi[1] + w2 * vi[2];
    Y[3 * r + 1] = w0 * vi[1] + w1 * vi[3] + w2 * vi[4];
    Y[3 * r + 2] = w0 * vi[2] + w1 * vi[4] + w2 * vi[5];
    e[r] = Y[3 * r] * g0 + Y[3 * r + 1] * g1 + Y[3 * r + 2] * g2;
  }
  if (DUMP && dump_y) {
#pragma unroll
    for (int k = 0; k < 18; k++) p.dbg_Y[18 * (size_t)a + k] = -Y[k];
  }
}

__device__ __forceinline__ void schur_block_add(double *blk, const double (&Y)[18], const double (&wb)[18], bool self,
                                                const double (&e)[6]) {
#pragma unroll
  for (int r = 0; r < 6; r++) {
    double val[6];
#pragma unroll
    for (int c = 0; c < 6; c++) val[c] = Y[3 * r] * wb[3 * c];
#pragma unroll
    for (int c = 0; c < 6; c++) val[c] = fma(Y[3 * r + 1], wb[3 * c + 1], val[c]);
#pragma unroll
    for (int c = 0; c < 6; c++) val[c] = fma(Y[3 * r + 2], wb[3 * c + 2], val[c]);
#pragma unroll
    for (int c = 0; c < 6; c++) {
      if (r == 0 && c >= 1) val[c] = self ? e[c - 1] : val[c];
      if (r == 1 && c == 2) val[c] = self ? e[5] : val[c];
    }
#pragma unroll
    for (int c = 0; c < 6; c++) atomicAdd(&blk[6 * r + c], val[c]);
  }
}

template <bool DUMP>
__global__ __launch_bounds__(SCHUR_THREADS) void k_schur_lds(SchurLdsArgs p) {
  extern __shared__ double sPart[];
  const int tid = threadIdx.x;
  int w = blockIdx.x;
  if ((p.nWg & 7) == 0) w = (blockIdx.x & 7) * (p.nWg >> 3) + (blockIdx.x >> 3);
  const SchurWg wg = p.wg[w];
  for (int t = tid; t < BLK_STRIDE * wg.nblk; t += SCHUR_THREADS) sPart[t] = 0.0;
  __syncthreads();

#ifdef PSBA_BUILD_EXPERIMENTS
  {
    const long long s1 = wg.itemD;
    unsigned long long item_next = (wg.item0 + tid < s1) ? p.items[wg.item0 + tid] : SCHUR_NULL_ITEM;
    for (long long t = wg.item0 + tid; t < s1; t += SCHUR_THREADS) {
      const unsigned long long item = item_next;
      if (t + SCHUR_THREADS < s1) item_next = p.items[t + SCHUR_THREADS];
      if (item == SCHUR_NULL_ITEM) continue;
      const int a = wg.obs0 + (int)(item & ((1u << PAIR_OBS_BITS) - 1));
      const int i = wg.pt0 + (int)((item >> PAIR_OBS_BITS) & ((1u << PAIR_PT_BITS) - 1));
      const int boff = (int)((item >> (PAIR_OBS_BITS + PAIR_PT_BITS)) & ((1u << ITEM_BOFF_BITS) - 1));
      const int pos = (int)((item >> (PAIR_OBS_BITS + PAIR_PT_BITS + ITEM_BOFF_BITS)) & ((1u << ITEM_POS_BITS) - 1));
      const int pos2 = (int)((item >> (PAIR_OBS_BITS + PAIR_PT_BITS + ITEM_BOFF_BITS + ITEM_POS_BITS)) & ((1u << ITEM_POS_BITS) - 1));
      const double *pv = p.PV + 9 * (size_t)i;
      const double2 *wa = reinterpret_cast<const double2 *>(p.W + 18 * (size_t)a);
      const double2 *wb2 = reinterpret_cast<const double2 *>(p.W + 18 * (size_t)(a - boff));
      double v[6], w[18], wb[18];
#pragma unroll
      for (int k = 0; k < 6; k++) v[k] = pv[k];
      const double g0 = pv[6], g1 = pv[7], g2 = pv[8];
#pragma unroll
      for (int k = 0; k < 9; k++) {
        const double2 q = wa[k];
        w[2 * k] = q.x;
        w[2 * k + 1] = q.y;
      }
#pragma unroll
      for (int k = 0; k < 9; k++) {
        const double2 q = wb2[k];
        wb[2 * k] = q.x;
        wb[2 * k + 1] = q.y;
      }
      double Y[18], e[6];
      schur_a_side<DUMP>(p, a, i, v, g0, g1, g2, w, Y, e, boff == 1);
      schur_block_add(sPart + BLK_STRIDE * pos, Y, wb, false, e);
      asm volatile("" ::: "memory");
#pragma unroll
      for (int k = 0; k < 9; k++) {
        const double2 q = wb2[9 + k];
        wb[2 * k] = q.x;
        wb[2 * k + 1] = q.y;
      }
      schur_block_add(sPart + BLK_STRIDE * pos2, Y, wb, boff == 1, e);
    }
  }
#endif
  const long long s1 = wg.item1;
  unsigned long long item_next = (wg.itemD + tid < s1) ? p.items[wg.itemD + tid] : SCHUR_NULL_ITEM;
  for (long long t = wg.itemD + tid; t < s1; t += SCHUR_THREADS) {
    const unsigned long long item = item_next;
    if (t + SCHUR_THREADS < s1) item_next = p.items[t + SCHUR_THREADS];
    if (item == SCHUR_NULL_ITEM) continue;
    const int a = wg.obs0 + (int)(item & ((1u << ITEM_OBS_BITS) - 1));
    const int i = wg.pt0 + (int)((item >> ITEM_OBS_BITS) & ((1u << ITEM_PT_BITS) - 1));
    const int boff = (int)((item >> (ITEM_OBS_BITS + ITEM_PT_BITS)) & ((1u << ITEM_BOFF_BITS) - 1));
    const int pos = (int)(item >> (ITEM_OBS_BITS + ITEM_PT_BITS + ITEM_BOFF_BITS));
    const double *pv = p.PV + 9 * (size_t)i;
    const double2 *wa = reinterpret_cast<const double2 *>(p.W + 18 * (size_t)a);
    const double2 *wb2 = reinterpret_cast<const double2 *>(p.W + 18 * (size_t)(a - boff));
    double v[6], w[18], wb[18];
#pragma unroll
    for (int k = 0; k < 6; k++) v[k] = pv[k];
    const double g0 = pv[6], g1 = pv[7], g2 = pv[8];
#pragma unroll
    for (int k = 0; k < 9; k++) {
      const double2 q = wa[k];
      w[2 * k] = q.x;
      w[2 * k + 1] = q.y;
    }
#pragma unroll
    for (int k = 0; k < 9; k++) {
      const double2 q = wb2[k];
      wb[2 * k] = q.x;
      wb[2 * k + 1] = q.y;
    }
    const bool self = boff == 0;
    double Y[18], e[6];
    schur_a_side<DUMP>(p, a, i, v, g0, g1, g2, w, Y, e, self);
    schur_block_add(sPart + BLK_STRIDE * pos, Y, wb, self, e);
  }
  __syncthreads();
  double2 *slab = reinterpret_cast<double2 *>(p.slab + wg.slab_off);
  for (int t = tid; t < 18 * wg.nblk; t += SCHUR_THREADS) {
    const double *src = sPart + BLK_STRIDE * (t / 18) + 2 * (t % 18);
    slab[t] = make_double2(src[0], src[1]);
  }
  if (p.diag0 && tid < 21 * 36) {
    const int b = tid / 36, rc = tid % 36;
    if (p.diag_grp[b] == wg.group) {
      const double v = sPart[BLK_STRIDE * p.diag_pos[b] + rc];
      if (v != 0.0) atomicAdd(&p.diag0[tid], v);
    }
  }
}

template <bool DUMP>
__global__ __launch_bounds__(RUN_THREADS) void k_schur_lds_runs(SchurLdsArgs p) {
  extern __shared__ double sPart[];
  const int tid = threadIdx.x;
  int w = blockIdx.x;
  if ((p.nWg & 7) == 0) w = (blockIdx.x & 7) * (p.nWg >> 3) + (blockIdx.x >> 3);
  const SchurWg wg = p.wg[w];
  for (int t = tid; t < BLK_STRIDE * wg.nblk; t += RUN_THREADS) sPart[t] = 0.0;
  __syncthreads();
  double acc[36];
#pragma unroll
  for (int k = 0; k < 36; k++) acc[k] = 0.0;
  int cur = -1;
  unsigned long long item_next = (wg.item0 + tid < wg.item1) ? p.items[wg.item0 + tid] : SCHUR_NULL_ITEM;
  for (long long t = wg.item0 + tid; t < wg.item1; t += RUN_THREADS) {
    const unsigned long long item = item_next;
    if (t + RUN_THREADS < wg.item1) item_next = p.items[t + RUN_THREADS];
    if (item == SCHUR_NULL_ITEM) continue;
    const int a = wg.obs0 + (int)(item & ((1u << ITEM_OBS_BITS) - 1));
    const int i = wg.pt0 + (int)((item >> ITEM_OBS_BITS) & ((1u << ITEM_PT_BITS) - 1));
    const int boff = (int)((item >> (ITEM_OBS_BITS + ITEM_PT_BITS)) & ((1u << ITEM_BOFF_BITS) - 1));
    const int pos = (int)(item >> (ITEM_OBS_BITS + ITEM_PT_BITS + ITEM_BOFF_BITS));
    const double *pv = p.PV + 9 * (size_t)i;
    const double2 *wa = reinterpret_cast<const double2 *>(p.W + 18 * (size_t)a);
    const double2 *wb2 = reinterpret_cast<const double2 *>(p.W + 18 * (size_t)(a - boff));
    double v[6], vi[6], wv[18], wb[18];
#pragma unroll
    for (int k = 0; k < 6; k++) v[k] = pv[k];
    const double g0 = pv[6], g1 = pv[7], g2 = pv[8];
#pragma unroll
    for (int k = 0; k < 9; k++) {
      const double2 q = wa[k];
      wv[2 * k] = q.x;
      wv[2 * k + 1] = q.y;
    }
#pragma unroll
    for (int k = 0; k < 9; k++) {
      const double2 q = wb2[k];
      wb[2 * k] = q.x;
      wb[2 * k + 1] = q.y;
    }
    if (pos != cur) {
      if (cur >= 0) {
        double *blk = sPart + BLK_STRIDE * cur;
#pragma unroll
        for (int k = 0; k < 36; k++) atomicAdd(&blk[k], acc[k]);
      }
#pragma unroll
      for (int k = 0; k < 36; k++) acc[k] = 0.0;
      cur = pos;
    }
    v[0] += p.mu;
    v[3] += p.mu;
    v[5] += p.mu;
    if (sym3_inverse(v, vi)) p.status[0] = p.try_id;
    if (DUMP) {
      double *o = p.dbg_Vinv + 9 * (size_t)i;
      o[0] = vi[0]; o[1] = vi[1]; o[2] = vi[2];
      o[3] = vi[1]; o[4] = vi[3]; o[5] = vi[4];
      o[6] = vi[2]; o[7] = vi[4]; o[8] = vi[5];
    }
    const bool self = boff == 0;
#pragma unroll
    for (int k = 0; k < 6; k++) vi[k] = -vi[k];
    double Y[18], e[6];
#pragma unroll
    for (int r = 0; r < 6; r++) {
      const double w0 = wv[3 * r], w1 = wv[3 * r + 1], w2 = wv[3 * r + 2];
      Y[3 * r] = w0 * vi[0] + w1 * vi[1] + w2 * vi[2];
      Y[3 * r + 1] = w0 * vi[1] + w1 * vi[3] + w2 * vi[4];
      Y[3 * r + 2] = w0 * vi[2] + w1 * vi[4] + w2 * vi[5];
      e[r] = Y[3 * r] * g0 + Y[3 * r + 1] * g1 + Y[3 * r + 2] * g2;
    }
    if (DUMP && self) {
#pragma unroll
      for (int k = 0; k < 18; k++) p.dbg_Y[18 * (size_t)a + k] = -Y[k];
    }
#pragma unroll
    for (int r = 0; r < 6; r++)
#pragma unroll
      for (int c = 0; c < 6; c++) {
        double val = fma(Y[3 * r + 2], wb[3 * c + 2], fma(Y[3 * r + 1], wb[3 * c + 1], Y[3 * r] * wb[3 * c]));
        if (r == 0 && c >= 1) val = self ? e[c - 1] : val;
        if (r == 1 && c == 2) val = self ? e[5] : val;
        acc[6 * r + c] += val;
      }
  }
  if (cur >= 0) {
    double *blk = sPart + BLK_STRIDE * cur;
#pragma unroll
    for (int k = 0; k < 36; k++) atomicAdd(&blk[k], acc[k]);
  }
  __syncthreads();
  double2 *slab = reinterpret_cast<double2 *>(p.slab + wg.slab_off);
  for (int t = tid; t < 18 * wg.nblk; t += RUN_THREADS) {
    const double *src = sPart + BLK_STRIDE * (t / 18) + 2 * (t % 18);
    slab[t] = make_double2(src[0], src[1]);
  }
  if (p.diag0) {
    for (int t = tid; t < 21 * 36; t += RUN_THREADS) {
      const int b = t / 36, rc = t % 36;
      if (p.diag_grp[b] == wg.group) {
        const double v = sPart[BLK_STRIDE * p.diag_pos[b] + rc];
        if (v != 0.0) atomicAdd(&p.diag0[t], v);
      }
    }
  }
}

__global__ __launch_bounds__(256) void k_schur_reduce(SchurReduceArgs p) {
  __shared__ double2 sAcc[8][32];
  __shared__ Factor32Lds sF;
  if ((int)blockIdx.x == p.diag_wg) {
    reduce_first_diag_block(p, sF);
    return;
  }
  if (blockIdx.x == 0 && threadIdx.x < 4 * SC_NPART) p.scal[SC_PART + threadIdx.x] = 0.0;
  if (blockIdx.x == 0 && threadIdx.x == 64) p.status[3] = p.try_id;
  if (!p.packed)
    write_padding(p.S, p.nA, p.n32, p.pad_one, (size_t)blockIdx.x * blockDim.x + threadIdx.x,
                  (size_t)(gridDim.x - (p.diag_wg >= 0 ? 1 : 0)) * blockDim.x);
  const int o = threadIdx.x & 31, q = threadIdx.x >> 5;
  const int L = 8 / p.chunks, slot = q / L, sub = q % L;
  const long long chunk = (long long)blockIdx.x * p.chunks + slot;
  double2 acc = make_double2(0.0, 0.0);
  if (chunk < p.nchunks) {
    const ReduceGroup gr = p.grp16[chunk / 9];
    const int n = gr.nwg;
    const size_t stride = (size_t)18 * gr.nblk;
    const double2 *s = reinterpret_cast<const double2 *>(p.slab + gr.slab) + (chunk * 32 + o - 18LL * gr.pos0);
    int k = sub;
    for (; k + 3 * L < n; k += 4 * L) {
      const double2 x0 = s[(size_t)k * stride];
      const double2 x1 = s[(size_t)(k + L) * stride];
      const double2 x2 = s[(size_t)(k + 2 * L) * stride];
      const double2 x3 = s[(size_t)(k + 3 * L) * stride];
      acc.x += x0.x; acc.y += x0.y;
      acc.x += x1.x; acc.y += x1.y;
      acc.x += x2.x; acc.y += x2.y;
      acc.x += x3.x; acc.y += x3.y;
    }
    for (; k < n; k += L) {
      const double2 x = s[(size_t)k * stride];
      acc.x += x.x; acc.y += x.y;
    }
  }
  if (L == 1) {
    if (chunk < p.nchunks) {
      reduce_scatter(p, 2 * (chunk * 32 + o), acc.x);
      reduce_scatter(p, 2 * (chunk * 32 + o) + 1, acc.y);
    }
    return;
  }
  sAcc[q][o] = acc;
  __syncthreads();
  if ((int)threadIdx.x >= 64 * p.chunks) return;
  const int fslot = threadIdx.x >> 6, po = (threadIdx.x & 63) >> 1, hi = threadIdx.x & 1;
  const long long fchunk = (long long)blockIdx.x * p.chunks + fslot;
  if (fchunk >= p.nchunks) return;
  double sum = 0.0;
  for (int t = 0; t < L; t++) sum += hi ? sAcc[fslot * L + t][po].y : sAcc[fslot * L + t][po].x;
// ... 61 lines not shown
  a.Lx = h->chol_L;
  a.linv = h->chol_ws;
  a.status = h->status;
  a.total = (int)h->packed_doubles;
  a.nA = h->d.nA;
  a.n32 = h->n32;
  a.try_id = h->try_id;
  const int grid = (a.total + 255) / 256;
  const bool fuse = !h->diag_done && !getenv("PSBA_CHOL_SEPARATE_DIAG");
  a.diag_wg = fuse ? grid : -1;
  for (int j = 0, b = 0; j < 6; j++)
    for (int k = 0; k <= j; k++, b++) a.diag_slot[b] = j < h->d.nC ? 36 * (j * (j + 1) / 2 + k) : 0;
  hipLaunchKernelGGL(k_schur_expand, dim3(grid + (fuse ? 1 : 0)), dim3(256), 0, h->stream, a);
  PSBA_HIP(h, hipGetLastError());
  if (fuse) h->diag_done = true;
  return PSBA_OK;
}

__global__ __launch_bounds__(256) void k_schur_finalize(double *S, double *ea, const double *U,
                                                        const double *ga, double mu_add, int nA,
                                                        int n32, double pad_one, double *scal,
                                                        int *status, int try_id) {
  if (blockIdx.x == 0 && threadIdx.x < 4 * SC_NPART) scal[SC_PART + threadIdx.x] = 0.0;
  if (blockIdx.x == 0 && threadIdx.x == 64) status[3] = try_id;
  const size_t n2 = (size_t)nA * nA;
  const size_t gtid = (size_t)blockIdx.x * blockDim.x + threadIdx.x;
  const size_t gsize = (size_t)gridDim.x * blockDim.x;
  for (size_t t = gtid; t < n2; t += gsize) {
    const int r = (int)(t / nA), c = (int)(t % nA);
    const int kb = r / 6, lb = c / 6;
    const size_t at = (size_t)r * n32 + c;
    if (lb > kb) {
      S[at] = S[(size_t)c * n32 + r];
    } else if (lb == kb) {
      double v = S[at] + U[36 * kb + 6 * (r - 6 * kb) + (c - 6 * lb)];
      if (r == c) v += mu_add;
      S[at] = v;
    }
  }
  for (size_t t = gtid; t < (size_t)nA; t += gsize) ea[t] += ga[t];
  write_padding(S, nA, n32, pad_one, gtid, gsize);
}

struct SchurOwnerArgs {
  const double *W, *PV;
  const int *iidx;
  const int2 *prod;
  const OwnerWave *waves;
  const OwnerUnit *units;
  double *S, *ea;
  int *status;
  double mu;
  int nWaves, ld, try_id;
  int bsr;
};

__global__ __launch_bounds__(256) void k_schur_owner(SchurOwnerArgs p) {
  const int lane = threadIdx.x & 63;
  const int w = blockIdx.x * 4 + (threadIdx.x >> 6);
  if (w >= p.nWaves) return;
  const OwnerWave wv = p.waves[w];
  const OwnerUnit un = p.units[(size_t)w * 64 + lane];
  const bool diag = un.j == un.k;
  double acc[36], ea[6];
#pragma unroll
  for (int t = 0; t < 36; t++) acc[t] = 0.0;
#pragma unroll
  for (int t = 0; t < 6; t++) ea[t] = 0.0;
  const int2 *pr = p.prod + (size_t)wv.row0 * 64 + lane;
  int2 ab = wv.len > 0 ? pr[0] : make_int2(-1, -1);
  for (int t = 0; t < wv.len; t++) {
    const int2 nxt = t + 1 < wv.len ? pr[(size_t)(t + 1) * 64] : make_int2(-1, -1);
    if (ab.x >= 0) {
      const int i = p.iidx[ab.x];
      const double *pv = p.PV + 9 * (size_t)i;
      const double2 *wa = reinterpret_cast<const double2 *>(p.W + 18 * (size_t)ab.x);
      const double2 *wb2 = reinterpret_cast<const double2 *>(p.W + 18 * (size_t)ab.y);
      double v[6], vi[6], wr[18], wb[18];
#pragma unroll
      for (int q = 0; q < 6; q++) v[q] = pv[q];
      const double g0 = pv[6], g1 = pv[7], g2 = pv[8];
#pragma unroll
      for (int q = 0; q < 9; q++) {
        const double2 x = wa[q], y = wb2[q];
        wr[2 * q] = x.x;
        wr[2 * q + 1] = x.y;
        wb[2 * q] = y.x;
        wb[2 * q + 1] = y.y;
      }
      v[0] += p.mu;
      v[3] += p.mu;
      v[5] += p.mu;
      if (sym3_inverse(v, vi)) p.status[0] = p.try_id;
      double Y[18];
#pragma unroll
      for (int r = 0; r < 6; r++) {
        const double w0 = wr[3 * r], w1 = wr[3 * r + 1], w2 = wr[3 * r + 2];
        Y[3 * r] = w0 * vi[0] + w1 * vi[1] + w2 * vi[2];
        Y[3 * r + 1] = w0 * vi[1] + w1 * vi[3] + w2 * vi[4];
        Y[3 * r + 2] = w0 * vi[2] + w1 * vi[4] + w2 * vi[5];
      }
      if (diag) {
#pragma unroll
        for (int r = 0; r < 6; r++) ea[r] -= Y[3 * r] * g0 + Y[3 * r + 1] * g1 + Y[3 * r + 2] * g2;
      }
#pragma unroll
      for (int r = 0; r < 6; r++)
#pragma unroll
        for (int c = 0; c < 6; c++)
          acc[6 * r + c] -= Y[3 * r] * wb[3 * c] + Y[3 * r + 1] * wb[3 * c + 1] + Y[3 * r + 2] * wb[3 * c + 2];
    }
    ab = nxt;
  }
  if (un.slot < 0) return;
  const int ldb = p.bsr ? 6 : p.ld;
  double *Sb = p.bsr ? p.S + 36 * (size_t)un.slot : p.S + (size_t)(6 * un.j) * p.ld + 6 * un.k;
  if (un.multi) {
#pragma unroll
    for (int r = 0; r < 6; r++)
#pragma unroll
      for (int c = 0; c < 6; c++) atomicAdd(&Sb[(size_t)r * ldb + c], acc[6 * r + c]);
  } else {
#pragma unroll
    for (int r = 0; r < 6; r++)
#pragma unroll
      for (int c = 0; c < 6; c++) Sb[(size_t)r * ldb + c] = acc[6 * r + c];
  }
  if (diag) {
#pragma unroll
    for (int r = 0; r < 6; r++) atomicAdd(&p.ea[6 * un.j + r], ea[r]);
  }
}

static int launch_schur_lds(psba_ctx *h, double mu, bool dump) {
  const Dims &d = h->d;
  SchurLdsArgs a;
  a.W = h->W;
  a.PV = h->PV;
  a.wg = h->wg;
  a.items = h->items;
  a.slab = h->slab;
  a.status = h->status;
  a.dbg_Y = h->dbg_Y;
  a.dbg_Vinv = h->dbg_Vinv;
  a.mu = mu;
  a.nWg = h->nWg;
  a.try_id = h->try_id;
  const bool fuse_diag = h->nranks == 1 && h->diag0 && !getenv("PSBA_CHOL_SEPARATE_DIAG") &&
                         !getenv("PSBA_SCHUR_NO_FLUSH_DIAG");
  a.diag0 = fuse_diag ? h->diag0 : nullptr;
  for (int b = 0; b < 21; b++) {
    a.diag_grp[b] = h->h_diaggrp[b];
    a.diag_pos[b] = h->h_diagpos[b];
  }
  SchurReduceArgs r;
  r.slab = h->slab;
  r.U = h->U;
  r.ga = h->ga;
  r.posblock = h->posblock;
  r.S = h->red;
  r.ea = h->red + (size_t)h->n32 * h->n32;
  r.scal = h->scal;
  r.status = h->status;
  r.mu_add = h->rank == 0 ? mu : 0.0;
  r.pad_one = h->rank == 0 ? 1.0 : 0.0;
  r.nA = d.nA;
  r.n32 = h->n32;
  r.nGroups = h->nGroups;
  r.try_id = h->try_id;
  r.diag0 = h->diag0;
  r.packed = (h->comm || (h->nranks > 1 && getenv("PSBA_SCHUR_PACKED"))) ? h->redp : nullptr;
  h->packed_pending = r.packed != nullptr;
  r.Lx = h->chol_L;
  r.linv = h->chol_ws;
  r.ring_copies = 0;
  r.ring_stride = 0;
  int worst = 0;
  long long npos = 0;
  for (int g = 0; g < h->nGroups; g++) {
    npos += h->gnblk[g];
    if (h->gnblk[g] > worst) worst = h->gnblk[g];
  }
  const size_t lds = sizeof(double) * BLK_STRIDE * (size_t)worst;
  int most = 1;
  for (int g = 0; g < h->nGroups; g++) most = h->gnwg[g] > most ? h->gnwg[g] : most;
  r.grp16 = h->gtab;
  r.chunks = most > 4 ? 4 : 8;
  if (const char *e = getenv("PSBA_REDUCE_CHUNKS")) r.chunks = atoi(e) == 2 || atoi(e) == 4 || atoi(e) == 8 ? atoi(e) : 1;
  r.nchunks = 36 * npos / 64;
  const int rgrid = (int)((r.nchunks + r.chunks - 1) / r.chunks);
  r.diag_wg = fuse_diag ? rgrid : -1;
  const bool pair = (h->prof & (1u << PSBA_K_SCHUR)) && !(h->prof & (1u << PSBA_K_SCHUR_REDUCE));
  {
    ProfScope pp(h, pair ? PSBA_K_SCHUR : -1);
    {
      ProfScope ps(h, pair ? -1 : PSBA_K_SCHUR);
      const char *m = getenv("PSBA_SCHUR_MODE");
      const int mode = m ? atoi(m) : 0;
      const dim3 G(h->nWg), B(SCHUR_THREADS);
      bool launched = false;
      if (h->schur_runs) {
        const dim3 Br(RUN_THREADS);
        if (dump)
          hipLaunchKernelGGL((k_schur_lds_runs<true>), G, Br, lds, h->stream, a);
        else
          hipLaunchKernelGGL((k_schur_lds_runs<false>), G, Br, lds, h->stream, a);
        launched = true;
      }
#ifdef PSBA_BUILD_EXPERIMENTS
      if (!launched && !dump && mode > 0 && !h->schur_pairs) launched = launch_schur_lds_mode(mode, G, B, lds, h->stream, a);
#endif
      (void)mode;
      if (launched) {
      } else if (dump)
        hipLaunchKernelGGL((k_schur_lds<true>), G, B, lds, h->stream, a);
      else
        hipLaunchKernelGGL((k_schur_lds<false>), G, B, lds, h->stream, a);
    }
    PSBA_HIP(h, hipGetLastError());
    {
      ProfScope ps(h, pair ? -1 : PSBA_K_SCHUR_REDUCE);
      hipLaunchKernelGGL(k_schur_reduce, dim3(rgrid + (r.diag_wg >= 0 ? 1 : 0)), dim3(256), 0, h->stream, r);
    }
  }
  h->diag_done = r.diag_wg >= 0;
  PSBA_HIP(h, hipGetLastError());
  return PSBA_OK;
}

static int launch_schur_sparse(psba_ctx *h, double mu) {
  PSBA_HIP(h, hipMemsetAsync(h->bs_val, 0, sizeof(double) * ((size_t)36 * h->bs_nblk + h->d.nA), h->stream));
  SchurOwnerArgs o;
  o.W = h->W;
  o.PV = h->PV;
  o.iidx = h->iidx;
  o.prod = h->own_prod;
  o.waves = h->own_waves;
  o.units = h->own_units;
  o.S = h->bs_val;
  o.ea = h->bs_ea;
  o.status = h->status;
  o.mu = mu;
  o.nWaves = h->own_nwaves;
  o.ld = 6;
  o.try_id = h->try_id;
  o.bsr = 1;
  const bool pair = (h->prof & (1u << PSBA_K_SCHUR)) && !(h->prof & (1u << PSBA_K_SCHUR_REDUCE));
  {
    ProfScope pp(h, pair ? PSBA_K_SCHUR : -1);
    {
      ProfScope ps(h, pair ? -1 : PSBA_K_SCHUR);
      hipLaunchKernelGGL(k_schur_owner, dim3((h->own_nwaves + 3) / 4), dim3(256), 0, h->stream, o);
    }
    {
      ProfScope ps(h, pair ? -1 : PSBA_K_SCHUR_REDUCE);
      const int rc = launch_bsr_finalize(h, mu);
      if (rc != PSBA_OK) return rc;
    }
  }
  PSBA_HIP(h, hipGetLastError());
  return PSBA_OK;
}

int launch_schur(psba_ctx *h, double mu, bool dump) {
  if (h->cnp != 6) return dump ? fail(h, PSBA_E_STATE, "the sba_func.h mirror is six-parameter only (not PSBA_CAMERA_FREE_K / PSBA_CAMERA_FREE_KD)") : h->cnp == KD_CNP ? launch_schur_kd(h, mu) : launch_schur_fk(h, mu);
  h->try_id++;
  h->diag_done = false;
  h->packed_pending = false;
  if (h->solver == PSBA_SOLVER_PCG) {
    if (dump) return fail(h, PSBA_E_INVALID, "the sba_func.h mirror verbs need the dense S: PSBA_SOLVER_DENSE");
    return launch_schur_sparse(h, mu);
  }
#ifdef PSBA_BUILD_EXPERIMENTS
  if (h->ring_nWg > 0 && !getenv("PSBA_SCHUR_ATOMIC")) return launch_schur_ring(h, mu, dump);
#endif
  if (h->nGroups > 0 && !getenv("PSBA_SCHUR_ATOMIC")) {
    if (!h->lds_attr_set) {
      const int dyn = 163840 - 256;
      const auto attr = hipFuncAttributeMaxDynamicSharedMemorySize;
      PSBA_HIP(h, hipFuncSetAttribute((const void *)k_schur_lds<true>, attr, dyn));
      PSBA_HIP(h, hipFuncSetAttribute((const void *)k_schur_lds<false>, attr, dyn));
      PSBA_HIP(h, hipFuncSetAttribute((const void *)k_schur_lds_runs<true>, attr, dyn));
      PSBA_HIP(h, hipFuncSetAttribute((const void *)k_schur_lds_runs<false>, attr, dyn));
      h->lds_attr_set = true;
    }
    return launch_schur_lds(h, mu, dump);
  }
  const Dims &d = h->d;
  SchurArgs a;
  a.W = h->W;
  a.PV = h->PV;
  a.iidx = h->iidx;
  a.jidx = h->jidx;
  a.ptr = h->ptr;
  a.tile_pt = h->tile_pt;
  a.S = h->red;
  a.ea = h->red + (size_t)h->n32 * h->n32;
  a.ld = h->n32;
  a.status = h->status;
  a.dbg_Y = h->dbg_Y;
  a.dbg_Vinv = h->dbg_Vinv;
  a.mu = mu;
  a.nC = d.nC;
  a.nA = d.nA;
  a.nTiles = d.nTilesAll;
  a.try_id = h->try_id;
  PSBA_HIP(h, hipMemsetAsync(h->red, 0, sizeof(double) * (size_t)(h->n32 + 1) * h->n32, h->stream));
  const bool owner = h->own_nwaves > 0 && !dump && !getenv("PSBA_SCHUR_ATOMIC");
  int grid = d.nTilesAll < 2048 ? d.nTilesAll : 2048;
  const size_t lds = sizeof(double) * (size_t)d.nA;
  if (!owner && lds > 100 * 1024)
    return fail(h, PSBA_E_INVALID, "global-atomic S assembly: 6 nCams = %d needs %zu B of LDS for e_a (> 100 KiB)",
                d.nA, lds);
  if (!owner && !h->atomic_attr_set && lds > 8 * 1024) {
    const auto attr = hipFuncAttributeMaxDynamicSharedMemorySize;
    PSBA_HIP(h, hipFuncSetAttribute((const void *)k_schur_atomic<true>, attr, 100 * 1024));
    PSBA_HIP(h, hipFuncSetAttribute((const void *)k_schur_atomic<false>, attr, 100 * 1024));
    h->atomic_attr_set = true;
  }
  const bool pair = (h->prof & (1u << PSBA_K_SCHUR)) && !(h->prof & (1u << PSBA_K_SCHUR_REDUCE));
  const double mu_add = h->rank == 0 ? mu : 0.0;
  size_t n2 = (size_t)d.nA * d.nA;
  size_t fg = (n2 + 255) / 256;
  const int fgrid = fg > 4096 ? 4096 : (int)fg;
  {
    ProfScope pp(h, pair ? PSBA_K_SCHUR : -1);
    {
      ProfScope ps(h, pair ? -1 : PSBA_K_SCHUR);
      if (owner) {
        SchurOwnerArgs o;
        o.W = h->W;
        o.PV = h->PV;
        o.iidx = h->iidx;
        o.prod = h->own_prod;
        o.waves = h->own_waves;
        o.units = h->own_units;
        o.S = a.S;
        o.ea = a.ea;
        o.status = h->status;
        o.mu = mu;
        o.nWaves = h->own_nwaves;
        o.ld = h->n32;
        o.try_id = h->try_id;
        o.bsr = 0;
        hipLaunchKernelGGL(k_schur_owner, dim3((h->own_nwaves + 3) / 4), dim3(256), 0, h->stream, o);
      } else {
        if (dump)
          hipLaunchKernelGGL(k_schur_atomic<true>, dim3(grid), dim3(TILE_OBS), lds, h->stream, a);
        else
          hipLaunchKernelGGL(k_schur_atomic<false>, dim3(grid), dim3(TILE_OBS), lds, h->stream, a);
        if (h->nLong) {
          if (dump)
            hipLaunchKernelGGL(k_schur_long<true>, dim3(h->nLong), dim3(TILE_OBS), 0, h->stream, a, h->long_pts);
          else
            hipLaunchKernelGGL(k_schur_long<false>, dim3(h->nLong), dim3(TILE_OBS), 0, h->stream, a, h->long_pts);
        }
      }
    }
    {
      ProfScope ps(h, pair ? -1 : PSBA_K_SCHUR_REDUCE);
      hipLaunchKernelGGL(k_schur_finalize, dim3(fgrid), dim3(256), 0, h->stream, a.S, a.ea, h->U, h->ga,
                         mu_add, d.nA, h->n32, h->rank == 0 ? 1.0 : 0.0, h->scal, h->status, h->try_id);
    }
  }
  PSBA_HIP(h, hipGetLastError());
  return PSBA_OK;
}

}
```

psba_amd/csrc/psba_api.cpp:

```cpp
#include <algorithm>
#include <cmath>
#include <cstdarg>
#include <cstdio>
#include <cstdlib>
#include <cstring>
#include <string>
#include <new>
#include <vector>

#include "camera_model.h"
#include "psba_internal.h"

using namespace psba;

static thread_local std::string g_create_err;

namespace psba {

int fail(psba_ctx *h, int code, const char *fmt, ...) {
  char buf[1024];
  va_list ap;
  va_start(ap, fmt);
  vsnprintf(buf, sizeof buf, fmt, ap);
  va_end(ap);
  if (h)
    h->err = buf;
  else
    g_create_err = buf;
  return code;
}

ProfScope::ProfScope(psba_ctx *hh, int kind) : h(hh) {
  if (kind < 0 || !(h->prof & (1u << kind))) return;
  if (h->spans_used == h->spans.size()) {
    psba_ctx::Span s;
    s.kind = kind;
    if (hipEventCreateWithFlags(&s.a, hipEventDisableSystemFence) != hipSuccess ||
        hipEventCreateWithFlags(&s.b, hipEventDisableSystemFence) != hipSuccess)
      return;
    h->spans.push_back(s);
  }
  idx = (int)h->spans_used++;
  h->spans[idx].kind = kind;
  (void)hipEventRecord(h->spans[idx].a, h->stream);
}
ProfScope::~ProfScope() {
  if (idx >= 0) (void)hipEventRecord(h->spans[idx].b, h->stream);
}

}

#define CHECK_H_NOJOIN(h)                 \
  do {                                    \
    if (!(h)) return PSBA_E_INVALID;      \
    (void)hipSetDevice((h)->device);      \
  } while (0)
#define CHECK_H(h)                                                         \
  do {                                                                     \
    CHECK_H_NOJOIN(h);                                                     \
    if ((h)->scal_side) {                                                  \
      (void)hipStreamWaitEvent((h)->stream, (h)->scal_event, 0);           \
      (h)->scal_side = false;                                              \
    }                                                                      \
  } while (0)
#define NEED(h, cond, what)                                             \
  do {                                                                  \
    if (!(cond)) return fail((h), PSBA_E_STATE, "%s: %s", __func__, what); \
  } while (0)
#define RCCL(h, call)                                                                   \
  do {                                                                                  \
    ncclResult_t r__ = (call);                                                          \
    if (r__ != ncclSuccess)                                                             \
      return fail((h), PSBA_E_RCCL, "%s failed: %s", #call, ncclGetErrorString(r__));   \
  } while (0)
#define TRY(expr)                 \
  do {                            \
    int rc__ = (expr);            \
    if (rc__ < 0) return rc__;    \
  } while (0)

namespace psba {
int alloc_bytes(psba_ctx *h, void **p, size_t bytes, bool pinned) {
  *p = nullptr;
  if (pinned) {
    if (hipHostMalloc(p, bytes) != hipSuccess) return fail(h, PSBA_E_NOMEM, "no pinned memory (%zu bytes)", bytes);
    return PSBA_OK;
  }
  PSBA_HIP(h, hipMalloc(p, bytes));
  static const bool poison = getenv("PSBA_DEBUG_POISON") != nullptr;
  if (poison) {
    PSBA_HIP(h, hipMemsetAsync(*p, 0xFF, bytes, h->stream));
    PSBA_HIP(h, hipStreamSynchronize(h->stream));
  }
  return PSBA_OK;
}
}

template <typename T>
static int upload(psba_ctx *h, DevBuf<T> &dst, const std::vector<T> &v) {
  TRY(dst.alloc(h, v.size()));
  if (!v.empty()) PSBA_HIP(h, hipMemcpy(dst, v.data(), sizeof(T) * v.size(), hipMemcpyHostToDevice));
  return PSBA_OK;
}

static void drop_problem(psba_ctx *h) { static_cast<ProblemState &>(*h) = ProblemState{}; }

extern "C" {

const char *psba_version(void) { return "psba_hip 0.1 (gfx950, fp64)"; }

const char *psba_last_error(psba_handle h) { return h ? h->err.c_str() : g_create_err.c_str(); }

static hipError_t create_main_stream(hipStream_t *s) {
  int least = 0, greatest = 0;
  if (getenv("PSBA_STREAM_PRIO_DEFAULT") || hipDeviceGetStreamPriorityRange(&least, &greatest) != hipSuccess)
    return hipStreamCreateWithFlags(s, hipStreamNonBlocking);
  return hipStreamCreateWithPriority(s, hipStreamNonBlocking, greatest);
}

int psba_create(int device, psba_handle *out) {
  if (!out) return PSBA_E_INVALID;
  *out = nullptr;
  int ndev = 0;
  hipError_t e = hipGetDeviceCount(&ndev);
  if (e != hipSuccess || ndev == 0)
    return fail(nullptr, PSBA_E_HIP, "no HIP device available (%s); this library has no CPU path",
                e == hipSuccess ? "device count 0" : hipGetErrorString(e));
  if (device < 0 || device >= ndev)
    return fail(nullptr, PSBA_E_INVALID, "device %d out of range (%d devices)", device, ndev);
  psba_ctx *h = new psba_ctx();
  h->device = device;
  if ((e = hipSetDevice(device)) != hipSuccess ||
      (e = create_main_stream(&h->stream)) != hipSuccess ||
      (e = hipEventCreateWithFlags(&h->scal_event, hipEventDisableTiming)) != hipSuccess) {
    int rc = fail(nullptr, PSBA_E_HIP, "psba_create: %s", hipGetErrorString(e));
    psba_destroy(h);
    return rc;
  }
  if (h->scal.alloc(h, NSCAL) != PSBA_OK || h->h_scal.alloc(h, NSCAL + 8) != PSBA_OK) {
    int rc = fail(nullptr, PSBA_E_HIP, "psba_create: %s", h->err.c_str());
    psba_destroy(h);
    return rc;
  }
  if (hipHostGetDevicePointer((void **)&h->h_scal_dev, h->h_scal, 0) != hipSuccess) h->h_scal_dev = nullptr;
  h->status = reinterpret_cast<int *>(h->scal + 8);
  h->h_status = reinterpret_cast<int *>(h->h_scal + 8);
  (void)hipMemsetAsync(h->scal, 0, sizeof(double) * NSCAL, h->stream);
  (void)hipStreamSynchronize(h->stream);
  h->h_scal[NSCAL] = 0.0;
  *out = h;
  return PSBA_OK;
}

int psba_destroy(psba_handle h) {
  CHECK_H(h);
  (void)hipSetDevice(h->device);
  if (h->stream) (void)hipStreamSynchronize(h->stream);
  if (h->stream2) (void)hipStreamSynchronize(h->stream2);
  if (h->comm) ncclCommDestroy(h->comm);
  if (h->k3_event) (void)hipEventDestroy(h->k3_event);
  for (hipEvent_t e : h->chol_events) (void)hipEventDestroy(e);
  if (h->chol_side) {
    (void)hipStreamSynchronize(h->chol_side);
    (void)hipStreamDestroy(h->chol_side);
  }
  if (h->stream2) (void)hipStreamDestroy(h->stream2);
  if (h->scal_event) (void)hipEventDestroy(h->scal_event);
  for (auto &s : h->spans) {
    (void)hipEventDestroy(s.a);
    (void)hipEventDestroy(s.b);
  }
  if (h->stream) (void)hipStreamDestroy(h->stream);
  delete h;
  return PSBA_OK;
}

int psba_schur_path(psba_handle h, int *path) {
  CHECK_H(h);
  NEED(h, h->uploaded, "no problem uploaded");
  if (path) *path = h->cnp == KD_CNP ? 5 : h->solver == PSBA_SOLVER_PCG ? 4 : getenv("PSBA_SCHUR_ATOMIC") ? 2 : h->ring_nWg > 0 ? 3 : h->nGroups > 0 ? 0 : 1;
  return PSBA_OK;
}

int psba_set_camera_model(psba_handle h, int model) {
  CHECK_H(h);
  if (model != PSBA_CAMERA_FIXED_K && model != PSBA_CAMERA_FREE_K && model != PSBA_CAMERA_FREE_KD)
    return fail(h, PSBA_E_INVALID, "unknown camera model %d", model);
  NEED(h, !h->uploaded, "psba_set_camera_model before psba_upload_problem (every buffer depends on the camera block)");
  h->cnp = model == PSBA_CAMERA_FREE_KD ? KD_CNP : model == PSBA_CAMERA_FREE_K ? FK_CNP : 6;
  return PSBA_OK;
}

static int lens_settable(psba_ctx *h, const char *what) {
  if (!h->uploaded) return fail(h, PSBA_E_STATE, "%s: no problem uploaded", what);
  if (h->cnp != 6)
    return fail(h, PSBA_E_STATE, "%s: the fixed-intrinsics camera block only (not PSBA_CAMERA_FREE_K / PSBA_CAMERA_FREE_KD)", what);
  if (h->backsub_pending) return fail(h, PSBA_E_STATE, "%s: a damping try is in flight (psba_backsub_wait first)", what);
  return PSBA_OK;
}

static void lens_changed(psba_ctx *h) {
  h->ahead = false;
  h->lin_is_ahead = false;
  h->linearized = h->assembled = h->solved = false;
}

static int set_start_distortion(psba_ctx *h, const double *kc) {
  if (h->backsub_pending) return fail(h, PSBA_E_STATE, "psba_set_distortion: a damping try is in flight (psba_backsub_wait first)");
  const int nC = h->d.nC;
  for (int t = 0; kc && t < 5 * nC; t++)
    if (!std::isfinite(kc[t])) return fail(h, PSBA_E_INVALID, "psba_set_distortion: kc[%d] of camera %d is not finite", t % 5, t / 5);
  std::vector<double> c((size_t)h->d.nA);
  double *dst[2] = {h->cams[h->cur], h->params0};
  for (int k = 0; k < 2; k++) {
    PSBA_HIP(h, hipMemcpyAsync(c.data(), dst[k], sizeof(double) * c.size(), hipMemcpyDeviceToHost, h->stream));
    PSBA_HIP(h, hipStreamSynchronize(h->stream));
    for (int j = 0; j < nC; j++)
      for (int q = 0; q < 5; q++) c[(size_t)KD_CNP * j + 5 + q] = kc ? kc[5 * j + q] : 0.0;
    PSBA_HIP(h, hipMemcpyAsync(dst[k], c.data(), sizeof(double) * c.size(), hipMemcpyHostToDevice, h->stream));
    PSBA_HIP(h, hipStreamSynchronize(h->stream));
  }
  h->ahead = h->lin_is_ahead = false;
  h->linearized = h->assembled = h->solved = h->backsubbed = false;
  return PSBA_OK;
}

int psba_set_distortion(psba_handle h, const double *kc) {
  CHECK_H(h);
  if (h->uploaded && h->cnp == KD_CNP) return set_start_distortion(h, kc);
  TRY(lens_settable(h, __func__));
  if (!kc) {
    h->lens_kc.reset();
    h->lens &= ~LENS_DIST;
  } else {
    for (int t = 0; t < 5 * h->d.nC; t++)
      if (!std::isfinite(kc[t])) return fail(h, PSBA_E_INVALID, "%s: kc[%d] of camera %d is not finite", __func__, t % 5, t / 5);
    if (!h->lens_kc) TRY(h->lens_kc.alloc(h, (size_t)5 * h->d.nC));
    PSBA_HIP(h, hipMemcpyAsync(h->lens_kc, kc, sizeof(double) * 5 * (size_t)h->d.nC, hipMemcpyHostToDevice, h->stream));
    PSBA_HIP(h, hipStreamSynchronize(h->stream));
    h->lens |= LENS_DIST;
  }
  lens_changed(h);
  return PSBA_OK;
}

int psba_set_obs_covariance(psba_handle h, const double *cov) {
  CHECK_H(h);
  TRY(lens_settable(h, __func__));
  if (!cov) {
    h->lens_w.reset();
    h->lens &= ~LENS_COV;
    lens_changed(h);
    return PSBA_OK;
  }
  std::vector<double> w((size_t)LENS_WSTRIDE * h->d.nO, 0.0);
  for (int a = 0; a < h->d.nO; a++) {
    const double *c = cov + 4 * (size_t)a;
    const double p = c[0], r = c[3];
    const double big = std::fmax(std::fmax(std::fabs(c[0]), std::fabs(c[1])), std::fmax(std::fabs(c[2]), std::fabs(c[3])));
    if (!(std::isfinite(p) && std::isfinite(c[1]) && std::isfinite(c[2]) && std::isfinite(r)))
      return fail(h, PSBA_E_INVALID, "%s: covariance of observation %d is not finite", __func__, a);
    if (std::fabs(c[1] - c[2]) > 1e-12 * big)
      return fail(h, PSBA_E_INVALID, "%s: covariance of observation %d is not symmetric (%.17g vs %.17g)", __func__, a, c[1], c[2]);
    const double q = 0.5 * (c[1] + c[2]);
    const double det = p * r - q * q;
    if (!(p > 0.0) || !(det > 0.0))
      return fail(h, PSBA_E_INVALID, "%s: covariance of observation %d is not positive definite", __func__, a);
    const double i00 = r / det, i01 = -q / det, i11 = p / det;
    const double l00 = std::sqrt(i00), l01 = i01 / l00;
    const double t = i11 - l01 * l01;
    if (!(t > 0.0)) return fail(h, PSBA_E_INVALID, "%s: covariance of observation %d is not positive definite", __func__, a);
    w[(size_t)LENS_WSTRIDE * a] = l00;
    w[(size_t)LENS_WSTRIDE * a + 1] = l01;
    w[(size_t)LENS_WSTRIDE * a + 2] = std::sqrt(t);
  }
  if (!h->lens_w) TRY(h->lens_w.alloc(h, w.size()));
  PSBA_HIP(h, hipMemcpyAsync(h->lens_w, w.data(), sizeof(double) * w.size(), hipMemcpyHostToDevice, h->stream));
  PSBA_HIP(h, hipStreamSynchronize(h->stream));
  h->lens |= LENS_COV;
  lens_changed(h);
  return PSBA_OK;
}

int psba_lens_model(psba_handle h, int *has_distortion, int *has_covariance) {
  CHECK_H(h);
  if (has_distortion) *has_distortion = ((h->lens & LENS_DIST) || h->cnp == KD_CNP) ? 1 : 0;
  if (has_covariance) *has_covariance = (h->lens & LENS_COV) ? 1 : 0;
  return PSBA_OK;
}

static_assert(PSBA_LOSS_NONE == LOSS_NONE && PSBA_LOSS_HUBER == LOSS_HUBER && PSBA_LOSS_CAUCHY == LOSS_CAUCHY &&
                  PSBA_LOSS_SOFT_L1 == LOSS_SOFT_L1,
              "loss kinds of the C ABI and the kernels");

int psba_set_robust_loss(psba_handle h, int kind, double scale) {
  CHECK_H(h);
  TRY(lens_settable(h, __func__));
  if (kind < PSBA_LOSS_NONE || kind > PSBA_LOSS_SOFT_L1) return fail(h, PSBA_E_INVALID, "%s: unknown loss kind %d", __func__, kind);
  if (!(std::isfinite(scale) && scale > 0.0))
    return fail(h, PSBA_E_INVALID, "%s: the scale must be finite and > 0 (got %.17g)", __func__, scale);
  h->loss_kind = kind;
  h->loss_c = scale;
  if (kind == PSBA_LOSS_NONE)
    h->lens &= ~LENS_ROBUST;
  else
    h->lens |= LENS_ROBUST;
  lens_changed(h);
  return PSBA_OK;
}

int psba_robust_loss(psba_handle h, int *kind, double *scale) {
  CHECK_H(h);
  if (kind) *kind = h->loss_kind;
  if (scale) *scale = h->loss_c;
  return PSBA_OK;
}

int psba_set_fixed(psba_handle h, const unsigned char *fixed_cams, const unsigned char *fixed_pts) {
  CHECK_H(h);
  TRY(lens_settable(h, __func__));
  const int nC = h->d.nC, nP = h->d.nP;
  int nfc = 0, nfp = 0;
  for (int j = 0; fixed_cams && j < nC; j++) nfc += fixed_cams[j] ? 1 : 0;
  for (int i = 0; fixed_pts && i < nP; i++) nfp += fixed_pts[i] ? 1 : 0;
  if (h->nranks == 1 && nfc == nC && nfp == nP)
    return fail(h, PSBA_E_INVALID, "%s: every camera and every point is fixed: no free parameter is left", __func__);
  std::vector<unsigned char> fc, fp;
  DevBuf<unsigned char> new_c, new_p;
  auto stage = [&]() -> int {
    if (nfc) {
      fc.resize((size_t)nC);
      for (int j = 0; j < nC; j++) fc[j] = fixed_cams[j] ? 1 : 0;
      TRY(new_c.alloc(h, (size_t)nC));
      PSBA_HIP(h, hipMemcpyAsync(new_c, fc.data(), fc.size(), hipMemcpyHostToDevice, h->stream));
    }
    if (nfp) {
      fp.resize((size_t)nP);
      for (int i = 0; i < nP; i++) fp[i] = fixed_pts[i] ? 1 : 0;
      TRY(new_p.alloc(h, (size_t)nP));
      PSBA_HIP(h, hipMemcpyAsync(new_p, fp.data(), fp.size(), hipMemcpyHostToDevice, h->stream));
    }
    PSBA_HIP(h, hipStreamSynchronize(h->stream));
    return PSBA_OK;
  };
  const int rc = stage();
  if (rc != PSBA_OK) {
    (void)hipStreamSynchronize(h->stream);
    return rc;
  }
  h->fix_cams = std::move(new_c);
  h->fix_pts = std::move(new_p);
  h->n_fix_cams = nfc;
  h->n_fix_pts = nfp;
  h->has_fixed = nfc > 0 || nfp > 0;
  h->struct_only = nfc == nC;
  h->try_shortcut = false;
  lens_changed(h);
  return PSBA_OK;
}

int psba_fixed_counts(psba_handle h, int *n_fixed_cams, int *n_fixed_pts) {
  CHECK_H(h);
  if (n_fixed_cams) *n_fixed_cams = h->n_fix_cams;
  if (n_fixed_pts) *n_fixed_pts = h->n_fix_pts;
  return PSBA_OK;
}

int psba_set_intrinsics_mask(psba_handle h, const unsigned char *free10) {
  CHECK_H(h);
  NEED(h, h->uploaded, "no problem uploaded");
  NEED(h, h->cnp == KD_CNP, "psba_set_intrinsics_mask: PSBA_CAMERA_FREE_KD only");
  NEED(h, !h->backsub_pending, "psba_set_intrinsics_mask: a damping try is in flight (psba_backsub_wait first)");
  unsigned m = 0;
  for (int k = 0; k < 10; k++) m |= (!free10 || free10[k]) ? 1u << k : 0u;
  h->kd_mask = m;
  lens_changed(h);
  return PSBA_OK;
}

int psba_intrinsics_mask(psba_handle h, unsigned char *out10) {
  CHECK_H(h);
  NEED(h, h->uploaded, "no problem uploaded");
  NEED(h, h->cnp == KD_CNP, "psba_intrinsics_mask: PSBA_CAMERA_FREE_KD only");
  for (int k = 0; out10 && k < 10; k++) out10[k] = (h->kd_mask >> k) & 1u;
  return PSBA_OK;
}

static int d2h(psba_ctx *h, void *dst, const void *src, size_t bytes);

int psba_obs_sq_residuals(psba_handle h, int which, double *s) {
  CHECK_H(h);
  NEED(h, h->uploaded, "no problem uploaded");
  NEED(h, h->cnp == 6, "six-parameter camera blocks only (not PSBA_CAMERA_FREE_K / PSBA_CAMERA_FREE_KD)");
  if (which != PSBA_PARAMS_CUR && which != PSBA_PARAMS_NEW) return fail(h, PSBA_E_INVALID, "%s: which = %d", __func__, which);
  if (!h->obs_s) TRY(h->obs_s.alloc(h, (size_t)h->d.nO));
  TRY(launch_residual(h, which, nullptr, h->obs_s));
  return d2h(h, s, h->obs_s, sizeof(double) * (size_t)h->d.nO);
}

int psba_camera_block(psba_handle h, int *cnp) {
  CHECK_H(h);
  if (cnp) *cnp = h->cnp;
  return PSBA_OK;
}

int psba_get_dims(psba_handle h, int *nCams, int *n3Dpts, int *n2Dprojs) {
  CHECK_H(h);
  NEED(h, h->uploaded, "no problem uploaded");
  if (nCams) *nCams = h->d.nC;
  if (n3Dpts) *n3Dpts = h->d.nP;
  if (n2Dprojs) *n2Dprojs = h->d.nO;
  return PSBA_OK;
}

namespace {
struct Upload {
  int nC, nP, nO;
  const double *Kparas, *impts, *initrot, *camsEx, *pts3D;
  const int *iidx, *jidx;
  std::vector<int> ptr;
  std::vector<int> tile_pt;
  std::vector<int> long_pts;
  int maxTrack = 0;
};
}

static int build_point_csr(psba_ctx *h, Upload &u) {
  if (u.nC <= 0 || u.nP <= 0 || u.nO <= 0 || !u.Kparas || !u.impts || !u.initrot || !u.camsEx || !u.pts3D || !u.iidx ||
      !u.jidx)
    return fail(h, PSBA_E_INVALID, "psba_upload_problem: null pointer or non-positive size");
  if (h->cnp == KD_CNP && (h->solver == PSBA_SOLVER_PCG || h->nranks > 1 || h->comm))
    return fail(h, PSBA_E_STATE, "PSBA_CAMERA_FREE_KD: dense solver, single rank only");
  if (h->cnp != 6 && (h->solver == PSBA_SOLVER_PCG || h->nranks > 1 || h->comm))
    return fail(h, PSBA_E_INVALID, "free intrinsics: dense solver, single rank only");
  u.ptr.assign((size_t)u.nP + 1, 0);
  for (int a = 0; a < u.nO; a++) {
    const int i = u.iidx[a], j = u.jidx[a];
    if (i < 0 || i >= u.nP || j < 0 || j >= u.nC)
      return fail(h, PSBA_E_INVALID, "observation %d: point %d / camera %d out of range", a, i, j);
    if (a > 0 && (i < u.iidx[a - 1] || (i == u.iidx[a - 1] && j <= u.jidx[a - 1])))
      return fail(h, PSBA_E_INVALID,
                  "observations must be sorted point-major with ascending, distinct cameras "
                  "inside a point (violated at observation %d)", a);
    u.ptr[(size_t)i + 1]++;
  }
  for (int i = 0; i < u.nP; i++) {
    if (u.ptr[(size_t)i + 1] > u.maxTrack) u.maxTrack = u.ptr[(size_t)i + 1];
    u.ptr[(size_t)i + 1] += u.ptr[i];
  }
  return PSBA_OK;
}

static void cut_tiles(Upload &u) {
  const std::vector<int> &ptr = u.ptr;
  u.tile_pt.push_back(0);
  for (int p0 = 0; p0 < u.nP;) {
    int p1 = p0;
    if (ptr[(size_t)p0 + 1] - ptr[p0] > TILE_OBS) {
      u.long_pts.push_back(p0);
      p1 = p0 + 1;
    } else {
      while (p1 < u.nP && (ptr[(size_t)p1 + 1] - ptr[p0]) <= TILE_OBS && (p1 - p0) < TILE_PTS) p1++;
    }
    u.tile_pt.push_back(p1);
    p0 = p1;
  }
}

static void set_dims(psba_ctx *h, const Upload &u) {
  const int cnp = h->cnp;
  Dims d;
  d.nC = u.nC;
  d.nP = u.nP;
  d.nO = u.nO;
  d.nA = cnp * u.nC;
  d.nB = 3 * u.nP;
  d.nT = d.nA + d.nB;
  d.nTilesAll = (int)u.tile_pt.size() - 1;
  d.nTiles = d.nTilesAll - (int)u.long_pts.size();
  if (d.nTiles < 1) d.nTiles = 1;
  d.maxTrack = u.maxTrack;
  h->d = d;
  h->nLong = (int)u.long_pts.size();
  const size_t cam_lds_max = getenv("PSBA_LIN_LDS_ACC") ? 96 * 1024 : 48 * 1024;
  h->cam_global = cnp == 6 && ((size_t)CAM_ACC * u.nC * sizeof(double) > cam_lds_max || getenv("PSBA_LIN_GLOBAL_ACC"));
  h->nPart = d.nTiles < 768 ? d.nTiles : 768;
  if (const char *e = getenv("PSBA_LIN_GRID")) h->nPart = atoi(e) > 0 && atoi(e) < d.nTiles ? atoi(e) : d.nTiles;
  h->n32 = (d.nA + 31) / 32 * 32;
}

static int alloc_work_buffers(psba_ctx *h) {
  const Dims &d = h->d;
  const int cnp = h->cnp;
  TRY(h->cams[0].alloc(h, (size_t)d.nA));
  TRY(h->cams[1].alloc(h, (size_t)d.nA));
  TRY(h->pts[0].alloc(h, (size_t)d.nB));
  TRY(h->pts[1].alloc(h, (size_t)d.nB));
  TRY(h->params0.alloc(h, (size_t)d.nT));
  TRY(h->impts.alloc(h, (size_t)2 * d.nO));
  TRY(h->iidx.alloc(h, (size_t)d.nO));
  TRY(h->jidx.alloc(h, (size_t)d.nO));
  TRY(h->W.alloc(h, (size_t)3 * cnp * d.nO));
  TRY(h->W_alt.alloc(h, (size_t)3 * cnp * d.nO));
  TRY(h->PV.alloc(h, (size_t)9 * d.nP));
  TRY(h->PV_alt.alloc(h, (size_t)9 * d.nP));
  PSBA_HIP(h, hipMemsetAsync(h->PV, 0, sizeof(double) * 9 * (size_t)d.nP, h->stream));
  PSBA_HIP(h, hipMemsetAsync(h->PV_alt, 0, sizeof(double) * 9 * (size_t)d.nP, h->stream));
  TRY(h->U.alloc(h, (size_t)cnp * cnp * d.nC));
  TRY(h->U_alt.alloc(h, (size_t)cnp * cnp * d.nC));
// ... 161 lines not shown
            8e-6 * (double)rp.nS * (double)h->packedN);
  }
  return PSBA_OK;
}
#endif

static int plan_schur_lds(psba_ctx *h, const Upload &u) {
  SchurPlanHost plan;
  TRY(build_schur_plan(h, u.nC, u.nP, u.nO, u.iidx, u.jidx, u.ptr.data(), plan));
  if (!h->nGroups) {
    OwnerPlanHost op;
    TRY(build_owner_plan(u.nC, u.nO, u.iidx, u.jidx, u.ptr.data(), op));
    TRY(upload_owner_plan(h, op));
    if (getenv("PSBA_SCHUR_PLAN_INFO"))
      fprintf(stderr, "[psba] K2 owner route (%d cameras): %lld products in %zu ELL slots (fill %.3f), %d waves\n",
              u.nC, op.products, op.prod.size(), (double)op.products / (double)op.prod.size(), h->own_nwaves);
    return PSBA_OK;
  }
  h->schur_runs = plan.runs;
  h->schur_pairs = plan.pair_items > 0;
  TRY(upload(h, h->items, plan.items));
  TRY(upload(h, h->wg, plan.wgs));
  TRY(upload(h, h->posblock, plan.posblock));
  TRY(h->slab.alloc(h, plan.slab_doubles));
  for (int j = 0, b = 0; j < 6; j++)
    for (int k = 0; k <= j; k++, b++) {
      h->h_diagpos[b] = j < u.nC ? plan.blockpos[(size_t)b] : 0;
      int g = -1;
      if (j < u.nC)
        for (g = 0; b >= h->gblk0[g + 1];) g++;
      h->h_diaggrp[b] = g;
    }
  std::vector<ReduceGroup> tab;
  long long pos0 = 0;
  for (int g = 0; g < h->nGroups; g++) {
    tab.insert(tab.end(), (size_t)h->gnblk[g] / 16, ReduceGroup{h->gnwg[g], h->gnblk[g], pos0, h->gslab[g], 0});
    pos0 += h->gnblk[g];
  }
  TRY(upload(h, h->gtab, tab));
  h->packed_doubles = h->packedN;
  TRY(h->redp.alloc(h, h->packed_doubles));
  TRY(h->diag0.alloc(h, (size_t)21 * 36));
  PSBA_HIP(h, hipMemsetAsync(h->diag0, 0, sizeof(double) * 21 * 36, h->stream));
  if (getenv("PSBA_SCHUR_PLAN_INFO"))
    fprintf(stderr, "[psba] K2 plan%s: %d groups, %d workgroups, %lld products in %zu item slots (fill %.3f), slabs %.1f MB\n",
            plan.runs ? " (runs layout)" : "", h->nGroups, h->nWg, plan.real_items, plan.items.size(),
            plan.items.size() ? (double)plan.real_items / (double)plan.items.size() : 1.0,
            8e-6 * (double)plan.slab_doubles);
  return PSBA_OK;
}

static int plan_schur_blockprod(psba_ctx *h, const Upload &u) {
  int seg = KD_SEG_DEFAULT;
  if (const char *e = getenv("PSBA_FKD_SEG"))
    if (atoi(e) > 0) seg = atoi(e);
  BlockProdPlanHost plan;
  if (build_blockprod_plan(u.nC, u.nO, u.iidx, u.jidx, u.ptr.data(), seg, plan) != PSBA_OK)
    return fail(h, PSBA_E_INVALID, "PSBA_CAMERA_FREE_KD: more than 2^31 products Y_a W_b^T");
  TRY(upload(h, h->kd_blocks, plan.blocks));
  TRY(upload(h, h->kd_segs, plan.segs));
  TRY(upload(h, h->kd_prods, plan.prods));
  if (!plan.multi.empty()) TRY(upload(h, h->kd_multi, plan.multi));
  TRY(h->kd_tiles.alloc(h, (size_t)256 * (plan.ntiles ? plan.ntiles : 1)));
  h->kd_nsegs = (int)plan.segs.size();
  h->kd_nmulti = (int)plan.multi.size();
  return PSBA_OK;
}

static int plan_schur(psba_ctx *h, const Upload &u) {
  if (h->solver == PSBA_SOLVER_PCG) return plan_schur_sparse(h, u);
#ifdef PSBA_BUILD_EXPERIMENTS
  TRY(plan_schur_ring(h, u));
  if (h->ring_nWg) return PSBA_OK;
#endif
  if (h->cnp == KD_CNP) return plan_schur_blockprod(h, u);
  if (h->cnp != 6) return PSBA_OK;
  return plan_schur_lds(h, u);
}

static int copy_inputs(psba_ctx *h, const Upload &u) {
  const Dims &d = h->d;
  std::vector<double> cc((size_t)u.nC * 9);
  for (int j = 0; j < u.nC; j++) {
    for (int k = 0; k < 5; k++) cc[(size_t)9 * j + k] = u.Kparas[5 * j + k];
    for (int k = 0; k < 4; k++) cc[(size_t)9 * j + 5 + k] = u.initrot[4 * j + k];
  }
  TRY(upload(h, h->camconst, cc));
  TRY(upload(h, h->ptr, u.ptr));
  TRY(upload(h, h->tile_pt, u.tile_pt));
  if (h->nLong) TRY(upload(h, h->long_pts, u.long_pts));
  std::vector<int4> tile_desc;
  for (int t = 0; t < d.nTilesAll; t++)
    if (u.ptr[u.tile_pt[t + 1]] - u.ptr[u.tile_pt[t]] <= TILE_OBS)
      tile_desc.push_back(make_int4(u.tile_pt[t], u.tile_pt[t + 1], u.ptr[u.tile_pt[t]], u.ptr[u.tile_pt[t + 1]]));
  if (tile_desc.empty()) tile_desc.push_back(make_int4(0, 0, 0, 0));
  TRY(upload(h, h->tile_desc, tile_desc));
  const double *cams = u.camsEx;
  std::vector<double> cam11;
  if (h->cnp != 6) {
    cam11.assign((size_t)d.nA, 0.0);
    for (int j = 0; j < u.nC; j++) {
      for (int k = 0; k < 5; k++) cam11[(size_t)h->cnp * j + k] = u.Kparas[5 * j + k];
      for (int k = 0; k < 6; k++) cam11[(size_t)h->cnp * j + h->cnp - 6 + k] = u.camsEx[6 * j + k];
    }
    cams = cam11.data();
  }
  auto H2D = [&](void *dst, const void *src, size_t bytes) {
    return hipMemcpyAsync(dst, src, bytes, hipMemcpyHostToDevice, h->stream);
  };
  PSBA_HIP(h, H2D(h->cams[0], cams, sizeof(double) * d.nA));
  PSBA_HIP(h, H2D(h->pts[0], u.pts3D, sizeof(double) * d.nB));
  PSBA_HIP(h, H2D(h->params0, cams, sizeof(double) * d.nA));
  PSBA_HIP(h, H2D(h->params0 + d.nA, u.pts3D, sizeof(double) * d.nB));
  PSBA_HIP(h, H2D(h->impts, u.impts, sizeof(double) * 2 * (size_t)d.nO));
  PSBA_HIP(h, H2D(h->iidx, u.iidx, sizeof(int) * (size_t)d.nO));
  PSBA_HIP(h, H2D(h->jidx, u.jidx, sizeof(int) * (size_t)d.nO));
  PSBA_HIP(h, hipStreamSynchronize(h->stream));
  return PSBA_OK;
}

int psba_upload_problem(psba_handle h, int nCams, int n3Dpts, int n2Dprojs, const double *Kparas,
                        const double *impts, const double *initrot, const double *camsEx,
                        const double *pts3D, const int *iidx, const int *jidx) {
  CHECK_H(h);
  Upload u{nCams, n3Dpts, n2Dprojs, Kparas, impts, initrot, camsEx, pts3D, iidx, jidx};
  TRY(build_point_csr(h, u));
  cut_tiles(u);
  PSBA_HIP(h, hipSetDevice(h->device));
  drop_problem(h);
  set_dims(h, u);
  TRY(alloc_work_buffers(h));
  if (h->cam_global || h->cnp == KD_CNP) TRY(upload_camera_index(h, u));
  TRY(plan_schur(h, u));
  TRY(copy_inputs(h, u));
  PSBA_HIP(h, hipDeviceSynchronize());
  h->uploaded = true;
  return PSBA_OK;
}

int psba_set_params(psba_handle h, const double *camsEx, const double *pts3D) {
  CHECK_H(h);
  NEED(h, h->uploaded, "no problem uploaded");
  PSBA_HIP(h, hipMemcpyAsync(h->cams[h->cur], camsEx, sizeof(double) * h->d.nA,
                             hipMemcpyHostToDevice, h->stream));
  PSBA_HIP(h, hipMemcpyAsync(h->pts[h->cur], pts3D, sizeof(double) * h->d.nB,
                             hipMemcpyHostToDevice, h->stream));
  PSBA_HIP(h, hipStreamSynchronize(h->stream));
  h->linearized = h->assembled = h->solved = h->backsubbed = false;
  h->ahead = h->lin_is_ahead = h->backsub_pending = h->publish_deferred = h->publish_in_k1 = false;
  return PSBA_OK;
}

int psba_reset_params(psba_handle h) {
  CHECK_H(h);
  NEED(h, h->uploaded, "no problem uploaded");
  PSBA_HIP(h, hipMemcpyAsync(h->cams[h->cur], h->params0, sizeof(double) * h->d.nA, hipMemcpyDeviceToDevice,
                             h->stream));
  PSBA_HIP(h, hipMemcpyAsync(h->pts[h->cur], h->params0 + h->d.nA, sizeof(double) * h->d.nB,
                             hipMemcpyDeviceToDevice, h->stream));
  h->linearized = h->assembled = h->solved = h->backsubbed = false;
  h->ahead = h->lin_is_ahead = h->backsub_pending = h->publish_deferred = h->publish_in_k1 = false;
  return PSBA_OK;
}

int psba_get_params(psba_handle h, int which, double *camsEx, double *pts3D) {
  CHECK_H(h);
  NEED(h, h->uploaded, "no problem uploaded");
  const int set = which == PSBA_PARAMS_NEW ? 1 - h->cur : h->cur;
  if (camsEx)
    PSBA_HIP(h, hipMemcpyAsync(camsEx, h->cams[set], sizeof(double) * h->d.nA,
                               hipMemcpyDeviceToHost, h->stream));
  if (pts3D)
    PSBA_HIP(h, hipMemcpyAsync(pts3D, h->pts[set], sizeof(double) * h->d.nB,
                               hipMemcpyDeviceToHost, h->stream));
  PSBA_HIP(h, hipStreamSynchronize(h->stream));
  return PSBA_OK;
}


static int fetch_scalars(psba_ctx *h) {
  PSBA_HIP(h, hipMemcpyAsync(h->h_scal, h->scal, sizeof(double) * NSCAL, hipMemcpyDeviceToHost,
                             h->stream));
  PSBA_HIP(h, hipStreamSynchronize(h->stream));
  return PSBA_OK;
}

static int enqueue_residual(psba_ctx *h, int which) {
  TRY(launch_residual(h, which, nullptr));
  if (h->comm)
    RCCL(h, ncclAllReduce(h->scal + SC_COST, h->scal + SC_COST, 1, ncclDouble, ncclSum, h->comm,
                          h->stream));
  return PSBA_OK;
}

int psba_residual(psba_handle h, int which, double *cost) {
  CHECK_H(h);
  NEED(h, h->uploaded, "no problem uploaded");
  TRY(enqueue_residual(h, which));
  TRY(fetch_scalars(h));
  if (cost) *cost = h->h_scal[SC_COST];
  return PSBA_OK;
}

int psba_linearize(psba_handle h, double coeff, double coeff_g) {
  CHECK_H(h);
  NEED(h, h->uploaded, "no problem uploaded");
  if (!(h->lin_is_ahead && coeff == h->coeff && coeff_g == h->coeff_g)) {
    h->coeff = coeff;
    h->coeff_g = coeff_g;
    TRY(launch_linearize(h, false));
  }
  h->lin_is_ahead = false;
  h->ahead = false;
  h->linearized = true;
  h->assembled = h->solved = h->backsubbed = false;
  return PSBA_OK;
}

static int enqueue_max_diag(psba_ctx *h) {
  if (h->comm) {
    double *tmp = h->dp;
    PSBA_HIP(h, hipMemcpyAsync(tmp, h->U, sizeof(double) * 36 * h->d.nC, hipMemcpyDeviceToDevice,
                               h->stream));
    RCCL(h, ncclAllReduce(tmp, tmp, (size_t)36 * h->d.nC, ncclDouble, ncclSum, h->comm, h->stream));
    std::swap(h->U, h->dp);
    int rc = launch_max_diag(h);
    std::swap(h->U, h->dp);
    TRY(rc);
    RCCL(h, ncclAllReduce(h->scal + SC_MAXDIAG, h->scal + SC_MAXDIAG, 1, ncclDouble, ncclMax,
                          h->comm, h->stream));
  } else {
    TRY(launch_max_diag(h));
  }
  return PSBA_OK;
}

int psba_begin(psba_handle h, double coeff, double coeff_g, double *cost, double *max_diag) {
  CHECK_H(h);
  NEED(h, h->uploaded, "no problem uploaded");
  TRY(enqueue_residual(h, PSBA_PARAMS_CUR));
  h->coeff = coeff;
  h->coeff_g = coeff_g;
  TRY(launch_linearize(h, false));
  h->linearized = true;
  h->assembled = h->solved = h->backsubbed = false;
  h->ahead = false;
  TRY(enqueue_max_diag(h));
  TRY(fetch_scalars(h));
  if (cost) *cost = h->h_scal[SC_COST];
  if (max_diag) *max_diag = h->h_scal[SC_MAXDIAG];
  h->lin_is_ahead = true;
  return PSBA_OK;
}

int psba_max_diag(psba_handle h, double *out) {
  CHECK_H(h);
  NEED(h, h->linearized, "psba_linearize first");
  TRY(enqueue_max_diag(h));
  TRY(fetch_scalars(h));
  if (out) *out = h->h_scal[SC_MAXDIAG];
  return PSBA_OK;
}

int psba_schur_assemble(psba_handle h, double mu) {
  CHECK_H(h);
  NEED(h, h->linearized, "psba_linearize first");
  h->mu = mu;
  h->try_shortcut = h->struct_only && h->cnp == 6 && !getenv("PSBA_FIXED_NO_SHORTCUT");
  if (h->try_shortcut)
    TRY(launch_struct_only_try(h, mu));
  else
    TRY(launch_schur(h, mu, false));
  h->assembled = true;
  h->solved = h->backsubbed = false;
  return PSBA_OK;
}

static int allreduce_schur(psba_ctx *h) {
  if (h->solver == PSBA_SOLVER_PCG) {
    if (h->comm)
      RCCL(h, ncclAllReduce(h->bs_val, h->bs_val, (size_t)36 * h->bs_nblk + h->d.nA, ncclDouble, ncclSum, h->comm, h->stream));
    return PSBA_OK;
  }
  if (h->packed_pending) {
    if (h->comm)
      RCCL(h, ncclAllReduce(h->redp, h->redp, h->packed_doubles, ncclDouble, ncclSum, h->comm, h->stream));
    TRY(launch_schur_expand(h));
    h->packed_pending = false;
  } else if (h->comm) {
    const size_t n = (size_t)(h->n32 + 1) * h->n32;
    RCCL(h, ncclAllReduce(h->red, h->red, n, ncclDouble, ncclSum, h->comm, h->stream));
  }
  return PSBA_OK;
}

int psba_schur_reduce(psba_handle h) {
  CHECK_H(h);
  NEED(h, h->assembled, "psba_schur_assemble first");
  if (!h->comm || h->try_shortcut) return PSBA_OK;
  ProfScope ps(h, PSBA_K_ALLREDUCE);
  TRY(allreduce_schur(h));
  return PSBA_OK;
}

int psba_schur_solve(psba_handle h) {
  CHECK_H(h);
  NEED(h, h->assembled, "psba_schur_assemble first");
  if (h->try_shortcut) {
    h->assembled = false;
    h->solved = true;
    return PSBA_OK;
  }
  if (h->packed_pending) TRY(allreduce_schur(h));
  if (h->solver == PSBA_SOLVER_PCG) {
    TRY(launch_pcg_solve(h));
    h->assembled = false;
    h->solved = true;
    return h->pcg_exhausted ? PSBA_PCG_MAXIT : PSBA_OK;
  }
  TRY(launch_chol_solve(h));
  if (h->chol_tim) {
    long long t[32];
    PSBA_HIP(h, hipMemcpyAsync(t, h->chol_tim, sizeof t, hipMemcpyDeviceToHost, h->stream));
    PSBA_HIP(h, hipStreamSynchronize(h->stream));
    fprintf(stderr, "chol stamps (cycles since the first):");
    for (int k = 1; k < 32; k++) fprintf(stderr, " %lld", t[k] ? t[k] - t[0] : 0);
    fprintf(stderr, "\n");
  }
  h->assembled = false;
  h->solved = true;
  return PSBA_OK;
}

static int publish_scalars(psba_ctx *h, hipStream_t s) {
  if (h->h_scal_dev && !getenv("PSBA_SCAL_MEMCPY"))
    TRY(launch_publish_scal(h, s));
  else
    PSBA_HIP(h, hipMemcpyAsync(h->h_scal, h->scal, sizeof(double) * NSCAL, hipMemcpyDeviceToHost, s));
  PSBA_HIP(h, hipEventRecord(h->scal_event, s));
  return PSBA_OK;
}

int psba_backsub_async(psba_handle h, double mu) {
  CHECK_H(h);
  NEED(h, h->solved, "psba_schur_solve first");
  TRY(launch_backsub(h, mu, false));
  hipStream_t s = h->stream;
  if (h->comm) {
    if (h->stream2 && getenv("PSBA_COMM_SIDE_STREAM")) {
      PSBA_HIP(h, hipEventRecord(h->k3_event, h->stream));
      PSBA_HIP(h, hipStreamWaitEvent(h->stream2, h->k3_event, 0));
      s = h->stream2;
      h->scal_side = true;
    }
    RCCL(h, ncclAllReduce(h->scal + SC_PART, h->scal + SC_PART, 4 * SC_NPART + 2, ncclDouble, ncclSum, h->comm, s));
  }
  h->publish_in_k1 = false;
  h->publish_deferred = !h->comm && h->h_scal_dev && !getenv("PSBA_SCAL_MEMCPY") && !getenv("PSBA_SCAL_KERNEL");
  if (!h->publish_deferred) TRY(publish_scalars(h, s));
  h->solved = false;
  h->backsub_pending = true;
  h->ahead = false;
  return PSBA_OK;
}

int psba_linearize_ahead(psba_handle h) {
  CHECK_H_NOJOIN(h);
  NEED(h, h->backsub_pending || h->backsubbed, "psba_backsub_async / psba_backsub first");
  const bool carry = h->backsub_pending && h->publish_deferred;
  if (carry) h->pub_seq += 1.0;
  TRY(launch_linearize(h, false, true, carry));
  if (carry) {
    h->publish_deferred = false;
    h->publish_in_k1 = true;
  }
  h->ahead = true;
  return PSBA_OK;
}

int psba_backsub_wait(psba_handle h, psba_try_scalars *out) {
  CHECK_H_NOJOIN(h);
  NEED(h, h->backsub_pending, "psba_backsub_async first");
  if (h->publish_deferred) {
    TRY(publish_scalars(h, h->stream));
    h->publish_deferred = false;
  }
  if (h->publish_in_k1) {
    volatile double *stamp = h->h_scal + NSCAL;
    long long spin = 0;
    while (*stamp != h->pub_seq && ++spin < 200000000LL) {
      if ((spin & 0xfffff) == 0 && hipStreamQuery(h->stream) != hipErrorNotReady) break;
    }
    if (*stamp != h->pub_seq) {
      PSBA_HIP(h, hipStreamSynchronize(h->stream));
      if (*stamp != h->pub_seq) return fail(h, PSBA_E_HIP, "the try's scalars did not reach the host");
    }
    __sync_synchronize();
    h->publish_in_k1 = false;
  } else {
    for (int spin = 0; spin < 20000 && hipEventQuery(h->scal_event) == hipErrorNotReady; spin++) {
    }
    PSBA_HIP(h, hipEventSynchronize(h->scal_event));
  }
  h->scal_side = false;
  h->backsub_pending = false;
  for (int q = 0; q < 4; q++) {
    double v = 0.0;
    for (int s = 0; s < SC_NPART; s++) v += h->h_scal[SC_PART + 4 * s + q];
    h->h_scal[SC_DP_L2 + q] = v;
  }
  const int st0 = h->h_scal[SC_STATUS_V] > 0.0 ? h->try_id : 0;
  const int st1 = h->h_scal[SC_STATUS_SPD] > 0.0 ? h->try_id : 0;
  h->backsubbed = true;
  if (out) {
    out->status = (st1 == h->try_id ? PSBA_NOT_SPD : 0) | (st0 == h->try_id ? PSBA_SINGULAR_V : 0);
    out->dp_l2 = h->h_scal[SC_DP_L2];
    out->gain_den = h->h_scal[SC_GAIN_DEN];
    out->new_cost = h->h_scal[SC_NEW_COST];
    out->newp_l2 = h->h_scal[SC_NEWP_L2];
  }
  return PSBA_OK;
}

int psba_backsub(psba_handle h, double mu, psba_try_scalars *out) {
  TRY(psba_backsub_async(h, mu));
  return psba_backsub_wait(h, out);
}

int psba_accept(psba_handle h) {
  CHECK_H(h);
  NEED(h, h->backsubbed, "psba_backsub first");
  h->cur = 1 - h->cur;
  h->linearized = h->assembled = h->solved = h->backsubbed = false;
  if (h->ahead) {
    std::swap(h->W, h->W_alt);
    std::swap(h->PV, h->PV_alt);
    std::swap(h->U, h->U_alt);
    std::swap(h->ga, h->ga_alt);
  }
  h->lin_is_ahead = h->ahead;
  h->ahead = false;
  return PSBA_OK;
}


static int d2h(psba_ctx *h, void *dst, const void *src, size_t bytes);

int psba_chol_dist_shape(psba_handle h, int *n32, int *NB, int *sharded) {
  CHECK_H(h);
  NEED(h, h->uploaded, "no problem uploaded");
  int nb = 0, bl = 0;
  TRY(chol_dist_shape(h, &nb, &bl));
  if (n32) *n32 = h->n32;
  if (NB) *NB = nb;
  if (sharded) *sharded = bl;
  return PSBA_OK;
}
int psba_chol_shape(psba_handle h, int *out8) {
  CHECK_H(h);
  NEED(h, h->uploaded, "no problem uploaded");
  if (!out8) return fail(h, PSBA_E_INVALID, "psba_chol_shape: null pointer");
  return chol_shape(h, out8);
}
int psba_chol_dist_exchange_plan(int n32, int NB, int nranks, int JE, long long *out4, int cap) {
  if (!out4 || cap <= 0) return PSBA_E_INVALID;
  return psba::chol_dist_exchange_plan(n32, NB, nranks, JE, reinterpret_cast<long long(*)[4]>(out4), cap);
}
int psba_chol_dist_begin(psba_handle h) {
  CHECK_H(h);
  NEED(h, h->assembled, "psba_schur_assemble (and the reduction over ranks) first");
  if (h->packed_pending) {
    TRY(launch_schur_expand(h));
    h->packed_pending = false;
  }
  return chol_dist_begin(h);
}
int psba_chol_dist_superpanel(psba_handle h, int J) {
  CHECK_H(h);
  NEED(h, h->assembled, "psba_schur_assemble first");
  if (J < 0 || J >= h->n32) return fail(h, PSBA_E_INVALID, "super-panel column %d out of range", J);
  return chol_dist_superpanel(h, J);
}
int psba_chol_dist_block(psba_handle h, int B, int set, double *buf, long long *n_doubles) {
  CHECK_H(h);
  NEED(h, h->assembled, "psba_schur_assemble first");
  if (B < 0 || 64 * B >= h->n32) return fail(h, PSBA_E_INVALID, "column block %d out of range", B);
  const int ncols = h->n32 - 64 * B < 64 ? h->n32 - 64 * B : 64;
  const long long n = (long long)(h->n32 + 1 - 64 * B) * ncols;
  if (n_doubles) *n_doubles = n;
  if (!buf) return PSBA_OK;
  if (!h->dist_buf) TRY(h->dist_buf.alloc(h, (size_t)(h->n32 + 1) * 64 * 8));
  if (set) {
    PSBA_HIP(h, hipMemcpyAsync(h->dist_buf, buf, sizeof(double) * (size_t)n, hipMemcpyHostToDevice, h->stream));
    return chol_dist_block(h, B, h->dist_buf, 1);
  }
  TRY(chol_dist_block(h, B, h->dist_buf, 0));
  return d2h(h, buf, h->dist_buf, sizeof(double) * (size_t)n);
}
int psba_chol_dist_finish(psba_handle h) {
  CHECK_H(h);
  NEED(h, h->assembled, "psba_schur_assemble first");
  TRY(chol_dist_finish(h));
  h->assembled = false;
  h->solved = true;
  return PSBA_OK;
}

static int ensure_trv(psba_ctx *h) {
  for (int k = 0; k < 2; k++)
    if (!h->trv[k]) TRY(h->trv[k].alloc(h, (size_t)h->d.nT));
  return PSBA_OK;
}

int psba_jmul_dots(psba_handle h, const double *x1, const double *x2, double dots[3]) {
  CHECK_H(h);
  NEED(h, h->cnp == 6, "six-parameter camera blocks only (PSBA_CAMERA_FREE_K / PSBA_CAMERA_FREE_KD: the fused verbs and psba_levmar)");
  NEED(h, h->uploaded, "no problem uploaded");
  if (!x1 || !dots) return fail(h, PSBA_E_INVALID, "psba_jmul_dots: null pointer");
  TRY(ensure_trv(h));
  const size_t bytes = sizeof(double) * (size_t)h->d.nT;
  PSBA_HIP(h, hipMemcpyAsync(h->trv[0], x1, bytes, hipMemcpyHostToDevice, h->stream));
  if (x2 && x2 != x1) PSBA_HIP(h, hipMemcpyAsync(h->trv[1], x2, bytes, hipMemcpyHostToDevice, h->stream));
  TRY(launch_jmul(h, h->trv[0], (x2 && x2 != x1) ? h->trv[1] : h->trv[0], nullptr, h->scal + SC_TR_DOTS));
  if (h->comm)
    RCCL(h, ncclAllReduce(h->scal + SC_TR_DOTS, h->scal + SC_TR_DOTS, 3, ncclDouble, ncclSum, h->comm, h->stream));
  TRY(fetch_scalars(h));
  for (int k = 0; k < 3; k++) dots[k] = h->h_scal[SC_TR_DOTS + k];
  return PSBA_OK;
}

int psba_set_solver(psba_handle h, int solver, double tol, int max_iter) {
  CHECK_H(h);
  if (solver != PSBA_SOLVER_DENSE && solver != PSBA_SOLVER_PCG) return fail(h, PSBA_E_INVALID, "unknown solver %d", solver);
  NEED(h, !h->uploaded || solver == h->solver, "psba_set_solver before psba_upload_problem (the buffers depend on it)");
  h->solver = solver;
  if (tol > 0) h->pcg_tol = tol;
  if (max_iter > 0) h->pcg_maxit = max_iter;
  return PSBA_OK;
}

int psba_pcg_info(psba_handle h, int *iters, double *relres, long long *blocks, long long *dense_blocks) {
  CHECK_H(h);
  NEED(h, h->uploaded && h->solver == PSBA_SOLVER_PCG, "PSBA_SOLVER_PCG and an uploaded problem");
  if (iters) *iters = h->pcg_iters;
  if (relres) *relres = h->pcg_relres;
  if (blocks) *blocks = h->bs_nblk;
  if (dense_blocks) *dense_blocks = (long long)h->d.nC * (h->d.nC + 1) / 2;
  return PSBA_OK;
}

int psba_get_sparse_S(psba_handle h, int *jk, double *val, double *ea) {
  CHECK_H(h);
  NEED(h, h->assembled && h->solver == PSBA_SOLVER_PCG, "psba_schur_assemble with PSBA_SOLVER_PCG first");
  NEED(h, !h->try_shortcut, "every camera is fixed: this try assembled no S (PSBA_FIXED_NO_SHORTCUT=1 keeps the general route)");
  if (jk) TRY(d2h(h, jk, h->bs_jk, sizeof(int2) * (size_t)h->bs_nblk));
  if (val) TRY(d2h(h, val, h->bs_val, sizeof(double) * 36 * (size_t)h->bs_nblk));
  if (ea) TRY(d2h(h, ea, h->bs_ea, sizeof(double) * (size_t)h->d.nA));
  return PSBA_OK;
}

int psba_set_sparse_S(psba_handle h, const double *val, const double *ea) {
  CHECK_H(h);
  NEED(h, h->assembled && h->solver == PSBA_SOLVER_PCG, "psba_schur_assemble with PSBA_SOLVER_PCG first");
  NEED(h, !h->try_shortcut, "every camera is fixed: this try assembled no S (PSBA_FIXED_NO_SHORTCUT=1 keeps the general route)");
  if (val) PSBA_HIP(h, hipMemcpyAsync(h->bs_val, val, sizeof(double) * 36 * (size_t)h->bs_nblk, hipMemcpyHostToDevice, h->stream));
  if (ea) PSBA_HIP(h, hipMemcpyAsync(h->bs_ea, ea, sizeof(double) * (size_t)h->d.nA, hipMemcpyHostToDevice, h->stream));
  PSBA_HIP(h, hipStreamSynchronize(h->stream));
  h->solved = h->backsubbed = false;
  return PSBA_OK;
}

int psba_sparse_pattern(int nCams, int n3Dpts, int n2Dprojs, const int *iidx, const int *jidx, unsigned char *flags) {
  if (nCams <= 0 || n3Dpts <= 0 || n2Dprojs <= 0 || !iidx || !jidx || !flags) return PSBA_E_INVALID;
  std::vector<int> ptr((size_t)n3Dpts + 1, 0);
  for (int a = 0; a < n2Dprojs; a++) {
    if (iidx[a] < 0 || iidx[a] >= n3Dpts || jidx[a] < 0 || jidx[a] >= nCams) return PSBA_E_INVALID;
    if (a && (iidx[a] < iidx[a - 1] || (iidx[a] == iidx[a - 1] && jidx[a] <= jidx[a - 1]))) return PSBA_E_INVALID;
    ptr[(size_t)iidx[a] + 1]++;
  }
  for (int i = 0; i < n3Dpts; i++) ptr[(size_t)i + 1] += ptr[(size_t)i];
  return psba::sparse_pattern(nCams, n2Dprojs, iidx, jidx, ptr.data(), flags);
}

int psba_set_sparse_pattern(psba_handle h, const unsigned char *flags, long long n) {
  CHECK_H(h);
  if (!flags || n <= 0) return fail(h, PSBA_E_INVALID, "psba_set_sparse_pattern: null pattern");
  NEED(h, !h->uploaded, "psba_set_sparse_pattern before psba_upload_problem (the block list depends on it)");
  h->bs_pattern.assign(flags, flags + n);
  return PSBA_OK;
}

int psba_allreduce_scalars(psba_handle h, double *v, int n) {
  CHECK_H(h);
  if (!v || n < 0 || n > 8) return fail(h, PSBA_E_INVALID, "psba_allreduce_scalars: at most 8 values");
// ... 693 lines not shown
```

psba_amd/csrc/psba_internal.h:

```cpp
#pragma once
#include <hip/hip_runtime.h>
#include <rccl/rccl.h>

#include <string>
#include <vector>

#include "../../include/psba_hip.h"
#include "dev_buf.h"

namespace psba {

constexpr int TILE_OBS = 256;
constexpr int TILE_PTS = 128;
constexpr int MAX_GROUPS = 128;
constexpr int CAM_ACC = 27;
constexpr int NSCAL = 104;
constexpr int SC_NPART = 16;

enum {
  SC_COST = 0,
  SC_DP_L2 = 1,
  SC_GAIN_DEN = 2,
  SC_NEW_COST = 3,
  SC_NEWP_L2 = 4,
  SC_MAXDIAG = 7,
  SC_PART = 16,
  SC_STATUS_V = 80,
  SC_STATUS_SPD = 81,
  SC_TR_DOTS = 84,
  SC_CHOLMOD = 88,
  SC_SUMS = 96,
};

struct Dims {
  int nC = 0, nP = 0, nO = 0;
  int nA = 0, nB = 0, nT = 0;
  int nTiles = 0;
  int nTilesAll = 0;
  int maxTrack = 0;
};

constexpr int ITEM_OBS_BITS = 24, ITEM_PT_BITS = 22, ITEM_BOFF_BITS = 8, ITEM_POS_BITS = 10;
struct SchurWg {
  int group, nblk;
  int obs0, pt0;
  long long item0, item1;
  unsigned long long slab_off;
  long long itemD;
};
constexpr int PAIR_OBS_BITS = 18, PAIR_PT_BITS = 16;
constexpr unsigned long long SCHUR_NULL_ITEM = ~0ull;
struct ReduceGroup {
  int nwg, nblk;
  long long pos0;
  unsigned long long slab;
  unsigned long long pad;
};

struct OwnerWave {
  long long row0;
  int len;
  int pad;
};
struct OwnerUnit {
  int j, k;
  int multi;
  int slot;
};
struct OwnerPlanHost {
  std::vector<int2> prod;
  std::vector<OwnerWave> waves;
  std::vector<OwnerUnit> units;
  std::vector<int2> blocks;
  std::vector<int> diag_slot;
  long long products = 0;
};
#ifdef PSBA_BUILD_EXPERIMENTS
constexpr int RING_LANES = 256;
constexpr int RING_MOVERS = 4;
constexpr int RING_PREPPERS = 4;
constexpr int RING_PREP_JOBS = 32;
constexpr int RING_PAGE = 7;
constexpr int RING_SLOTS = 992;
constexpr int RING_MAXOPS = 16;
constexpr unsigned RING_NULL_ENTRY = 0xFFFFFFFFu;
struct RingStep { int op_begin, op_end, job_begin, job_end; };
struct RingJob {
  int obs, point;
  int slots;
  int earow;
};
struct RingWg {
  int blk0, nblk;
  int row0, nrows;
  int copy, nsteps;
  int nwslots, pad;
  long long step0, ent0, op0, job0, lane0, bl0;
};
struct RingPlanHost {
  int nR = 0, nS = 0, nWg = 0, lat = 2;
  std::vector<int> rb;
  std::vector<RingWg> wgs;
  std::vector<RingStep> steps;
  std::vector<unsigned> entries;
  std::vector<int> ops;
  std::vector<RingJob> jobs;
  std::vector<int> lane_blk;
  std::vector<int> blk_lane0;
  long long products = 0, slots = 0, loaded_recs = 0;
};
#endif
struct SchurPlanHost {
  std::vector<unsigned long long> items;
  std::vector<SchurWg> wgs;
  std::vector<int> blockpos;
  std::vector<int> posblock;
  size_t slab_doubles = 0;
  long long real_items = 0;
  bool runs = false;
  long long tasks = 0;
  long long pair_items = 0;
};
struct BlockProdPlanHost {
  std::vector<int2> blocks;
  std::vector<int4> segs;
  std::vector<int2> prods;
  std::vector<int4> multi;
  int ntiles = 0;
  int seg_len = 0;
};
constexpr int KD_UNIT = 64;
constexpr int KD_SEG_DEFAULT = 64;
constexpr int KD_RED = 4 * 520;
constexpr int RUN_THREADS = 512;
constexpr int RUN_MAX = 32;
}

struct ProblemState {
  psba::Dims d;
  psba::DevBuf<double> camconst;
  psba::DevBuf<double> cams[2];
  psba::DevBuf<double> pts[2];
  psba::DevBuf<double> params0;
  psba::DevBuf<double> impts;
  int lens = 0;
  int loss_kind = 0;
  double loss_c = 1.0;
  psba::DevBuf<double> obs_s;
  psba::DevBuf<double> lens_kc;
  psba::DevBuf<double> lens_w;
  psba::DevBuf<unsigned char> fix_cams, fix_pts;
  int n_fix_cams = 0, n_fix_pts = 0;
  bool has_fixed = false, struct_only = false;
  bool try_shortcut = false;
  psba::DevBuf<int> iidx;
  psba::DevBuf<int> jidx;
  psba::DevBuf<int> ptr;
  psba::DevBuf<int> tile_pt;
  psba::DevBuf<int> long_pts;
  int nLong = 0;
  psba::DevBuf<int4> tile_desc;
  psba::DevBuf<double> W;
  psba::DevBuf<double> PV;
  psba::DevBuf<double> U;
  psba::DevBuf<double> ga;
  psba::DevBuf<double> W_alt, PV_alt, U_alt, ga_alt;
  bool ahead = false;
  bool lin_is_ahead = false;
  bool scal_side = false;
  psba::DevBuf<double> campart;
  int nPart = 0;
  bool cam_global = false;
  psba::DevBuf<double> camacc;
  psba::DevBuf<int> cam_obs;
  psba::DevBuf<int4> cam_units;
  int nCamUnits = 0;
  psba::DevBuf<double> red;
  int n32 = 0;
  int nGroups = 0;
  int nWg = 0;
  std::vector<int> gblk0;
  std::vector<int> gnwg;
  std::vector<int> gnblk;
  std::vector<size_t> gslab;
  psba::DevBuf<psba::ReduceGroup> gtab;
  psba::DevBuf<psba::SchurWg> wg;
  psba::DevBuf<unsigned long long> items;
  bool schur_runs = false;
  bool schur_pairs = false;
  psba::DevBuf<double> redp;
  size_t packed_doubles = 0;
  bool packed_pending = false;
  psba::DevBuf<double> diag0;
  int h_diagpos[21] = {0};
  int h_diaggrp[21] = {0};
  bool diag_done = false;
  psba::DevBuf<int> posblock;
  psba::DevBuf<double> slab;
  size_t packedN = 0;
  int ring_nWg = 0, ring_nS = 0;
#ifdef PSBA_BUILD_EXPERIMENTS
  psba::DevBuf<psba::RingWg> ring_wg;
  psba::DevBuf<psba::RingStep> ring_steps;
  psba::DevBuf<unsigned> ring_entries;
  psba::DevBuf<int> ring_ops;
  psba::DevBuf<psba::RingJob> ring_jobs;
  psba::DevBuf<int> ring_bl0;
  psba::DevBuf<int> ring_canon;
  psba::DevBuf<double> ring_slab;
  psba::DevBuf<double> ring_pvi;
  long long ring_products = 0, ring_slots = 0;
  size_t ring_loaded_recs = 0;
  psba::DevBuf<long long> chol_tim_ring;
#endif
  int pcg_iters = 0;
  double pcg_relres = 0.0;
  bool pcg_exhausted = false;
  long long bs_nblk = 0;
  psba::DevBuf<double> bs_val;
  double *bs_ea = nullptr;
  psba::DevBuf<int2> bs_jk;
  psba::DevBuf<int> bs_diag;
  psba::DevBuf<int> bs_rowptr;
  psba::DevBuf<int2> bs_rowent;
  psba::DevBuf<double> pcg_vec;
  psba::DevBuf<double> pcg_minv;
  psba::DevBuf<double> pcg_scal;
  psba::DevBuf<int2> own_prod;
  psba::DevBuf<psba::OwnerWave> own_waves;
  psba::DevBuf<psba::OwnerUnit> own_units;
  int own_nwaves = 0;
  long long own_products = 0;
  unsigned kd_mask = 0x3FFu;
  psba::DevBuf<int> kd_cuptr;
  psba::DevBuf<double> kd_Be;
  psba::DevBuf<double> kd_upart;
  psba::DevBuf<double> kd_Y;
  psba::DevBuf<double> kd_eapart;
  psba::DevBuf<int2> kd_blocks, kd_prods;
  psba::DevBuf<int4> kd_segs, kd_multi;
  psba::DevBuf<double> kd_tiles;
  int kd_nsegs = 0, kd_nmulti = 0;
  psba::DevBuf<double> kd_red;
  psba::DevBuf<double> dp;
  psba::DevBuf<double> trv[2];
  psba::DevBuf<double> jmul_out;
  psba::GraphExec chol_graph[2];
  int chol_graph_n32[2] = {0, 0};
  double *chol_graph_red[2] = {nullptr, nullptr};
  psba::DevBuf<long long> chol_tim;
  psba::DevBuf<double> chol_L;
  psba::DevBuf<double> dist_buf;
  psba::DevBuf<double> chol_ws;
  psba::DevBuf<double> dbg_ex, dbg_JA, dbg_JB, dbg_Y, dbg_Vinv, dbg_eb;

  bool uploaded = false, linearized = false, assembled = false, solved = false, backsubbed = false;
  bool backsub_pending = false;
  bool publish_deferred = false, publish_in_k1 = false;
  int cur = 0;
  double coeff = 1.0, coeff_g = 1.0, mu = 0.0;
  double coeff_w = 1.0;
  bool mu_applied = false;
};

struct psba_ctx : ProblemState {
  int device = 0;
  hipStream_t stream = nullptr;
  std::string err;

  ncclComm_t comm = nullptr;
  int nranks = 1, rank = 0;

  double *h_scal_dev = nullptr;
  hipEvent_t scal_event = nullptr;
  hipStream_t stream2 = nullptr;
  hipEvent_t k3_event = nullptr;
  hipStream_t chol_side = nullptr;
  std::vector<hipEvent_t> chol_events;

  int solver = 0;
  int cnp = 6;
  double pcg_tol = 1e-10;
  int pcg_maxit = 500;
  psba::PinnedBuf<double> pcg_host;
  std::vector<unsigned char> bs_pattern;

  psba::DevBuf<double> scal;
  int *status = nullptr;
  int try_id = 0;
  double pub_seq = 0.0;
  psba::PinnedBuf<double> h_scal;
  int *h_status = nullptr;

  bool lds_attr_set = false, atomic_attr_set = false, chol_attr_set = false, lin_attr_set = false, ring_attr_set = false;

  unsigned prof = 0;
  struct Span { hipEvent_t a, b; int kind; };
  std::vector<Span> spans;
  size_t spans_used = 0;
  double prof_ms[PSBA_K_COUNT] = {0};
  int prof_n[PSBA_K_COUNT] = {0};
};

namespace psba {

int fail(psba_ctx *h, int code, const char *fmt, ...);
#define PSBA_HIP(h, call)                                                              \
  do {                                                                                 \
    hipError_t e__ = (call);                                                           \
    if (e__ != hipSuccess)                                                             \
      return psba::fail((h), PSBA_E_HIP, "%s failed: %s (%s:%d)", #call,               \
                        hipGetErrorString(e__), __FILE__, __LINE__);                   \
  } while (0)

struct ProfScope {
  psba_ctx *h;
  int idx = -1;
  ProfScope(psba_ctx *h, int kind);
  ~ProfScope();
};

int launch_linearize(psba_ctx *h, bool dump, bool ahead = false, bool publish = false);
int launch_residual(psba_ctx *h, int which, double *ex_out_dev, double *s_out_dev = nullptr);
int launch_max_diag(psba_ctx *h);
int build_schur_plan(psba_ctx *h, int nCams, int nPts, int nObs, const int *iidx, const int *jidx,
                     const int *ptr, SchurPlanHost &out);
int build_owner_plan(int nCams, int nObs, const int *iidx, const int *jidx, const int *ptr, OwnerPlanHost &out,
                     const unsigned char *pattern = nullptr);
int sparse_pattern(int nCams, int nObs, const int *iidx, const int *jidx, const int *ptr, unsigned char *flags);
#ifdef PSBA_BUILD_EXPERIMENTS
int build_ring_plan(int nCams, int nPts, int nObs, const int *iidx, const int *jidx, const int *ptr, RingPlanHost &out,
                    bool force = false);
int launch_schur_ring(psba_ctx *h, double mu, bool dump);
struct SchurLdsArgs;
bool launch_schur_lds_mode(int mode, dim3 G, dim3 B, size_t lds, hipStream_t s, const SchurLdsArgs &a);
#endif
int launch_schur(psba_ctx *h, double mu, bool dump);
int launch_schur_expand(psba_ctx *h);
int launch_chol_solve(psba_ctx *h);
int launch_linearize_fk(psba_ctx *h, bool ahead, bool publish);
int launch_residual_fk(psba_ctx *h, int which);
int launch_max_diag_fk(psba_ctx *h);
int launch_schur_fk(psba_ctx *h, double mu);
int launch_backsub_fk(psba_ctx *h, double mu);
int build_blockprod_plan(int nCams, int nObs, const int *iidx, const int *jidx, const int *ptr, int seg_len,
                         BlockProdPlanHost &out);
int launch_linearize_kd(psba_ctx *h, bool ahead, bool publish);
int launch_residual_kd(psba_ctx *h, int which);
int launch_max_diag_kd(psba_ctx *h);
int launch_schur_kd(psba_ctx *h, double mu);
int launch_backsub_kd(psba_ctx *h, double mu);
int launch_bsr_finalize(psba_ctx *h, double mu);
int launch_pcg_solve(psba_ctx *h);
int launch_bsr_gershgorin(psba_ctx *h, double *lambda, double *info3);
int launch_chol_graph(psba_ctx *h);
int chol_dist_shape(psba_ctx *h, int *NB, int *blocked);
int chol_shape(psba_ctx *h, int *out8);
int chol_dist_exchange_plan(int n32, int NB, int nranks, int JE, long long (*out)[4], int cap);
int chol_dist_begin(psba_ctx *h);
int chol_dist_superpanel(psba_ctx *h, int J);
int chol_dist_block(psba_ctx *h, int B, double *buf_dev, int set);
int chol_dist_finish(psba_ctx *h);
int launch_backsub(psba_ctx *h, double mu, bool dump);
int launch_publish_scal(psba_ctx *h, hipStream_t s);
int launch_struct_only_try(psba_ctx *h, double mu);
int launch_jmul(psba_ctx *h, const double *x1_dev, const double *x2_dev, double *out1_dev, double *dots_dev);
int launch_pack_g(psba_ctx *h, double *g_dev);
int launch_newp(psba_ctx *h, double *dp_dev);
int launch_cholmod(psba_ctx *h, double *out4_dev);

}
```

psba_amd/csrc/schur_lds_args.h:

```cpp
#pragma once
#include "psba_internal.h"

namespace psba {

constexpr int SCHUR_THREADS = 1024;
constexpr int BLK_STRIDE = 37;

struct SchurLdsArgs {
  const double *W, *PV;
  const SchurWg *wg;
  const unsigned long long *items;
  double *slab;
  int *status;
  double *dbg_Y, *dbg_Vinv;
  double mu;
  int nWg, try_id;
  double *diag0;
  int diag_grp[21], diag_pos[21];
};

}
```

Baseline: 2104 M-obs/s.

## Defer camera-partial reduction into the Schur kernel prologue and prefetch slab loads

Linearization can now skip launching k_cam_reduce and mark the camera sums as pending. The Schur LDS kernel then folds the per-partition camera partials into U and ga in its prologue, overlapping that work with slab zeroing. Any other consumer flushes the pending reduction first. It also prefetches slab partials into registers in the standalone reduce and adds an opt-in DPP segmented scan. This saves a kernel launch and its serialization, at the cost of subtle state tracking that could break correctness when ordering differs.

```diff
diff --git a/include/psba_hip.h b/include/psba_hip.h
--- a/include/psba_hip.h
+++ b/include/psba_hip.h
@@ -89,6 +89,8 @@
 int psba_linearize_ahead(psba_handle h);
 int psba_backsub_wait(psba_handle h, psba_try_scalars *out);
 int psba_accept(psba_handle h);
+int psba_cam_sums_pending(psba_handle h, int *pending);
+int psba_cam_sums_repend(psba_handle h);
 
 int psba_compute_exQT(psba_handle h, int which, double *ex);
 int psba_compute_jacobiQT(psba_handle h, double *jac_A, double *jac_B);
diff --git a/psba_amd/build.py b/psba_amd/build.py
--- a/psba_amd/build.py
+++ b/psba_amd/build.py
@@ -11,7 +11,7 @@
 if EXPERIMENTS:
     SOURCES += ["kernels_schur_ring.hip", "schur_ring_plan.cpp", "kernels_schur_modes.hip"]
 OUT = os.path.join(HERE, "libpsba_hip_exp.so" if EXPERIMENTS else "libpsba_hip.so")
-HEADERS = ["psba_internal.h", "dev_buf.h", "camera_model.h", "chol_factor32.h", "schur_common.h", "schur_lds_args.h", os.path.join("..", "..", "include", "psba_hip.h")]
+HEADERS = ["psba_internal.h", "dev_buf.h", "camera_model.h", "chol_factor32.h", "schur_common.h", "schur_lds_args.h", "cam_sums.h", "dpp_scan.h", os.path.join("..", "..", "include", "psba_hip.h")]
 ROCM = os.environ.get("ROCM_PATH", "/opt/rocm")
 FLAGS = ["--offload-arch=gfx950", "-O3", "-std=c++17", "-fPIC", "-munsafe-fp-atomics",
          "-Wall", "-Wno-unused-result", "-x", "hip"] + (["-DPSBA_BUILD_EXPERIMENTS"] if EXPERIMENTS else [])
diff --git a/psba_amd/capi.py b/psba_amd/capi.py
--- a/psba_amd/capi.py
+++ b/psba_amd/capi.py
@@ -93,6 +93,8 @@
     ("psba_linearize_ahead", C.c_int, [_h]),
     ("psba_backsub_wait", C.c_int, [_h, C.POINTER(TryScalars)]),
     ("psba_accept", C.c_int, [_h]),
+    ("psba_cam_sums_pending", C.c_int, [_h, _ip]),
+    ("psba_cam_sums_repend", C.c_int, [_h]),
     ("psba_compute_exQT", C.c_int, [_h, C.c_int, _dp]),
     ("psba_compute_jacobiQT", C.c_int, [_h, _dp, _dp]),
     ("psba_compute_U", C.c_int, [_h, C.c_double, _dp]),
@@ -585,6 +587,14 @@
     def accept(self):
         self._ck(lib.psba_accept(self._h))
 
+    def cam_sums_pending(self):
+        v = C.c_int()
+        self._ck(lib.psba_cam_sums_pending(self._h, C.byref(v)))
+        return bool(v.value)
+
+    def cam_sums_repend(self):
+        self._ck(lib.psba_cam_sums_repend(self._h))
+
     def _out(self, fn, n, *pre):
         out = np.empty(n)
         rc = self._ck(fn(self._h, *pre, _d(out)))
diff --git a/psba_amd/csrc/cam_sums.h b/psba_amd/csrc/cam_sums.h
--- /dev/null
+++ b/psba_amd/csrc/cam_sums.h
@@ -0,0 +1,98 @@
+#pragma once
+#include "psba_internal.h"
+
+namespace psba {
+
+constexpr int CAM_SEQ = 32;
+constexpr int CAM_PRE = 24;
+
+struct CamFoldArgs {
+  const double *part;
+  double *U, *ga;
+  double coeff, coeff_g;
+  int nPart, nC;
+};
+
+__device__ __forceinline__ void cam_seq_issue(const double *src, size_t stride, int nPart, int s, double (&x)[CAM_PRE]) {
+#pragma unroll
+  for (int k = 0; k < CAM_PRE; k++) {
+    const int q = s + CAM_SEQ * k;
+    x[k] = src[(size_t)(q < nPart ? q : nPart - 1) * stride];
+  }
+}
+
+__device__ __forceinline__ double cam_seq_tail(const double *src, size_t stride, int nPart, int q, double acc) {
+  for (; q + 3 * CAM_SEQ < nPart; q += 4 * CAM_SEQ) {
+    const double x0 = src[(size_t)q * stride], x1 = src[(size_t)(q + CAM_SEQ) * stride];
+    const double x2 = src[(size_t)(q + 2 * CAM_SEQ) * stride], x3 = src[(size_t)(q + 3 * CAM_SEQ) * stride];
+    acc += x0;
+    acc += x1;
+    acc += x2;
+    acc += x3;
+  }
+  for (; q < nPart; q += CAM_SEQ) acc += src[(size_t)q * stride];
+  return acc;
+}
+
+__device__ __forceinline__ double cam_seq_sum(const double *src, size_t stride, int nPart, int s, const double (&x)[CAM_PRE]) {
+  double acc = 0.0;
+#pragma unroll
+  for (int k = 0; k < CAM_PRE; k++) acc += s + CAM_SEQ * k < nPart ? x[k] : 0.0;
+  return cam_seq_tail(src, stride, nPart, s + CAM_SEQ * CAM_PRE, acc);
+}
+
+__device__ __forceinline__ void cam_entry_store(int j, int e, double t, double coeff, double coeff_g, double *U, double *ga) {
+  if (e >= 21) {
+    ga[6 * (size_t)j + e - 21] = coeff_g * t;
+    return;
+  }
+  int lo = 0, k = e;
+  while (k >= 6 - lo) {
+    k -= 6 - lo;
+    lo++;
+  }
+  const int hi = lo + k;
+  const double v = coeff * t;
+  U[36 * (size_t)j + 6 * lo + hi] = v;
+  if (hi != lo) U[36 * (size_t)j + 6 * hi + lo] = v;
+}
+
+struct CamFoldLane {
+  const double *src;
+  int f, s;
+};
+
+__device__ __forceinline__ void cam_fold_range(const CamFoldArgs &c, int &f0, int &f1) {
+  const long long nOut = (long long)c.nC * CAM_ACC;
+  f0 = (int)(nOut * blockIdx.x / gridDim.x);
+  f1 = (int)(nOut * (blockIdx.x + 1) / gridDim.x);
+}
+
+__device__ __forceinline__ CamFoldLane cam_fold_issue(const CamFoldArgs &c, double (&x)[CAM_PRE]) {
+  CamFoldLane l;
+  int f0, f1;
+  cam_fold_range(c, f0, f1);
+  l.f = f0 + (int)(threadIdx.x >> 5);
+  l.s = threadIdx.x & (CAM_SEQ - 1);
+  l.src = l.f < f1 ? c.part + l.f : nullptr;
+  if (l.src) cam_seq_issue(l.src, (size_t)c.nC * CAM_ACC, c.nPart, l.s, x);
+  return l;
+}
+
+__device__ __forceinline__ void cam_fold_reduce_store(const CamFoldArgs &c, int f, int s, double acc) {
+  double t = __shfl(acc, 0, CAM_SEQ);
+  for (int q = 1; q < CAM_SEQ; q++) t += __shfl(acc, q, CAM_SEQ);
+  if (s == 0) cam_entry_store(f / CAM_ACC, f % CAM_ACC, t, c.coeff, c.coeff_g, c.U, c.ga);
+}
+
+__device__ __forceinline__ void cam_fold_finish(const CamFoldArgs &c, const CamFoldLane &l, const double (&x)[CAM_PRE]) {
+  const size_t stride = (size_t)c.nC * CAM_ACC;
+  if (l.src) cam_fold_reduce_store(c, l.f, l.s, cam_seq_sum(l.src, stride, c.nPart, l.s, x));
+  int f0, f1;
+  cam_fold_range(c, f0, f1);
+  const int step = (int)(blockDim.x >> 5);
+  for (int f = l.f + step; f < f1; f += step)
+    cam_fold_reduce_store(c, f, l.s, cam_seq_tail(c.part + f, stride, c.nPart, l.s, 0.0));
+}
+
+}
diff --git a/psba_amd/csrc/dpp_scan.h b/psba_amd/csrc/dpp_scan.h
--- /dev/null
+++ b/psba_amd/csrc/dpp_scan.h
@@ -0,0 +1,40 @@
+#pragma once
+#include <hip/hip_runtime.h>
+
+namespace psba {
+
+constexpr int DPP_NO_KEY = -2147483647 - 1;
+
+template <int CTRL, int ROWS>
+__device__ __forceinline__ int dpp_mov(int old, int src) {
+  return __builtin_amdgcn_update_dpp(old, src, CTRL, ROWS, 0xf, false);
+}
+template <int CTRL, int ROWS>
+__device__ __forceinline__ double dpp_mov_f64(double src) {
+  const int lo = dpp_mov<CTRL, ROWS>(0, __double2loint(src));
+  const int hi = dpp_mov<CTRL, ROWS>(0, __double2hiint(src));
+  return __hiloint2double(hi, lo);
+}
+
+template <int CTRL, int ROWS, int N>
+__device__ __forceinline__ bool dpp_seg_step(int key, double (&v)[N]) {
+  const bool ok = dpp_mov<CTRL, ROWS>(DPP_NO_KEY, key) == key;
+  if (!__any(ok)) return false;
+#pragma unroll
+  for (int k = 0; k < N; k++) {
+    const double vu = dpp_mov_f64<CTRL, ROWS>(v[k]);
+    v[k] += ok ? vu : 0.0;
+  }
+  return true;
+}
+
+template <int N>
+__device__ __forceinline__ void dpp_seg_scan(int key, double (&v)[N]) {
+  if (dpp_seg_step<0x111, 0xf>(key, v) && dpp_seg_step<0x112, 0xf>(key, v) && dpp_seg_step<0x114, 0xf>(key, v))
+    dpp_seg_step<0x118, 0xf>(key, v);
+  dpp_seg_step<0x142, 0x2>(key, v);
+  dpp_seg_step<0x143, 0x4>(key, v);
+  dpp_seg_step<0x142, 0x8>(key, v);
+}
+
+}
diff --git a/psba_amd/csrc/kernels_linearize.hip b/psba_amd/csrc/kernels_linearize.hip
--- a/psba_amd/csrc/kernels_linearize.hip
+++ b/psba_amd/csrc/kernels_linearize.hip
@@ -1,6 +1,9 @@
 #include <cstdlib>
-
+#include <cstring>
+
+#include "cam_sums.h"
 #include "camera_model.h"
+#include "dpp_scan.h"
 #include "psba_internal.h"
 
 namespace psba {
@@ -15,6 +18,7 @@
   double coeff, coeff_g;
   int nC, nTiles;
   int mode;
+  int scan_shfl;
   const double *pub_src;
   double *pub_dst;
   double pub_stamp;
@@ -258,7 +262,9 @@
       lens_load_w<LM>(p.wl, dn.z + tid, wl);
       m = reinterpret_cast<const double2 *>(p.impts)[dn.z + tid];
     }
-    if (p.mode != 3) {
+    if (p.mode != 3 && !p.scan_shfl) {
+      dpp_seg_scan(pi, v);
+    } else if (p.mode != 3) {
 #pragma unroll
       for (int d = 1; d < 64; d <<= 1) {
         const int pu = __shfl_up(pi, d, 64);
@@ -446,16 +452,9 @@
   if (e < CAM_ACC) {
     const double *src = campart + (size_t)j * CAM_ACC + e;
     const size_t stride = (size_t)nC * CAM_ACC;
-    int q = s;
-    for (; q + 96 < nPart; q += 128) {
-      const double x0 = src[(size_t)q * stride], x1 = src[(size_t)(q + 32) * stride];
-      const double x2 = src[(size_t)(q + 64) * stride], x3 = src[(size_t)(q + 96) * stride];
-      acc += x0;
-      acc += x1;
-      acc += x2;
-      acc += x3;
-    }
-    for (; q < nPart; q += 32) acc += src[(size_t)q * stride];
+    double x[CAM_PRE];
+    cam_seq_issue(src, stride, nPart, s, x);
+    acc = cam_seq_sum(src, stride, nPart, s, x);
   }
   sPart[s][e] = acc;
   __syncthreads();
@@ -465,14 +464,7 @@
     sPart[0][e] = t;
   }
   __syncthreads();
-  if (threadIdx.x < 36) {
-    const int r = threadIdx.x / 6, c = threadIdx.x % 6;
-    const int lo = r < c ? r : c, hi = r < c ? c : r;
-    const int k = lo * 6 - lo * (lo - 1) / 2 + (hi - lo);
-    U[36 * j + threadIdx.x] = coeff * sPart[0][k];
-  } else if (threadIdx.x < 42) {
-    ga[6 * j + threadIdx.x - 36] = coeff_g * sPart[0][21 + threadIdx.x - 36];
-  }
+  if (threadIdx.x < CAM_ACC) cam_entry_store(j, threadIdx.x, sPart[0][threadIdx.x], coeff, coeff_g, U, ga);
 }
 
 __global__ __launch_bounds__(256) void k_fixed_diag(FixedMask fm, int nC, int nP, double coeff, double cam_diag, double *U,
@@ -582,7 +574,7 @@
 }
 
 template <int LM>
-static void enqueue_linearize(psba_ctx *h, const LinArgs &a, const RobustLoss &rl, const FixedMask &fm, bool dump, bool v1, size_t lds, double *Uo, double *gao) {
+static void enqueue_linearize(psba_ctx *h, const LinArgs &a, const RobustLoss &rl, const FixedMask &fm, bool dump, bool v1, size_t lds, double *Uo, double *gao, bool defer) {
   const Dims &d = h->d;
   if (h->cam_global) {
     const int grid = d.nTiles < 2048 ? d.nTiles : 2048;
@@ -622,12 +614,29 @@
         hipLaunchKernelGGL((k_linearize_long<false, false, LM>), dim3(h->nLong), dim3(TILE_OBS), 0, h->stream, a, h->long_pts, slab, rl, fm);
       nslab++;
     }
-    hipLaunchKernelGGL(k_cam_reduce, dim3(d.nC), dim3(1024), 0, h->stream, h->campart, nslab, d.nC, h->coeff,
-                       h->coeff_g, Uo, gao);
-  }
-}
-
-int launch_linearize(psba_ctx *h, bool dump, bool ahead, bool publish) {
+    h->cam_slab_U = Uo;
+    h->cam_slab_ga = gao;
+    h->cam_slab_n = nslab;
+    h->cam_slab_coeff = h->coeff;
+    h->cam_slab_coeff_g = h->coeff_g;
+    if (defer)
+      h->cam_pend_U = Uo;
+    else
+      hipLaunchKernelGGL(k_cam_reduce, dim3(d.nC), dim3(1024), 0, h->stream, h->campart, nslab, d.nC, h->coeff,
+                         h->coeff_g, Uo, gao);
+  }
+}
+
+int cam_sums_flush(psba_ctx *h) {
+  if (!h->cam_pend_U) return PSBA_OK;
+  h->cam_pend_U = nullptr;
+  hipLaunchKernelGGL(k_cam_reduce, dim3(h->d.nC), dim3(1024), 0, h->stream, h->campart, h->cam_slab_n, h->d.nC,
+                     h->cam_slab_coeff, h->cam_slab_coeff_g, h->cam_slab_U, h->cam_slab_ga);
+  PSBA_HIP(h, hipGetLastError());
+  return PSBA_OK;
+}
+
+int launch_linearize(psba_ctx *h, bool dump, bool ahead, bool publish, bool may_defer) {
   if (h->cnp != 6) return dump ? fail(h, PSBA_E_STATE, "the sba_func.h mirror is six-parameter only (not PSBA_CAMERA_FREE_K / PSBA_CAMERA_FREE_KD)") : h->cnp == KD_CNP ? launch_linearize_kd(h, ahead, publish) : launch_linearize_fk(h, ahead, publish);
   const Dims &d = h->d;
   LinArgs a;
@@ -662,6 +671,8 @@
   {
     const char *m = getenv("PSBA_LIN_MODE");
     a.mode = m ? atoi(m) : 0;
+    const char *sc = getenv("PSBA_LIN_SCAN");
+    a.scan_shfl = !(sc && !strcmp(sc, "dpp"));
   }
   const bool v1 = getenv("PSBA_LIN_V1") != nullptr;
   const size_t lds = h->cam_global ? 0 : sizeof(double) * CAM_ACC * (size_t)d.nC;
@@ -673,6 +684,15 @@
     h->lin_attr_set = true;
   }
   double *Uo = ahead ? h->U_alt : h->U, *gao = ahead ? h->ga_alt : h->ga;
+  if (h->cam_pend_U && h->cam_pend_U != Uo) {
+    const int rc = cam_sums_flush(h);
+    if (rc != PSBA_OK) return rc;
+  }
+  h->cam_pend_U = h->cam_slab_U = h->cam_slab_ga = nullptr;
+  bool lds_route = h->nGroups > 0 && h->ring_nWg == 0 && !getenv("PSBA_SCHUR_ATOMIC");
+  const bool defer = may_defer && (ahead || getenv("PSBA_CAM_REDUCE_DEFER")) && !getenv("PSBA_CAM_REDUCE_SEPARATE") &&
+                     h->nranks == 1 && !h->comm && lds_route && !h->cam_global && !h->has_fixed &&
+                     h->solver == PSBA_SOLVER_DENSE && !dump;
   {
     ProfScope ps(h, PSBA_K_LINEARIZE);
     if (h->cam_global)
@@ -680,7 +700,7 @@
     else if (h->nLong)
       PSBA_HIP(h, hipMemsetAsync(h->campart + (size_t)h->nPart * d.nC * CAM_ACC, 0, sizeof(double) * CAM_ACC * (size_t)d.nC,
                                  h->stream));
-    lens_dispatch_fixed(h->lens, h->has_fixed, [&](auto m) { enqueue_linearize<decltype(m)::value>(h, a, rl, fm, dump, v1, lds, Uo, gao); });
+    lens_dispatch_fixed(h->lens, h->has_fixed, [&](auto m) { enqueue_linearize<decltype(m)::value>(h, a, rl, fm, dump, v1, lds, Uo, gao, defer); });
     if (h->has_fixed)
       hipLaunchKernelGGL(k_fixed_diag, dim3((d.nC + d.nP + 255) / 256), dim3(256), 0, h->stream, fm, d.nC, d.nP, h->coeff,
                          h->rank == 0 ? h->coeff : 0.0, Uo, gao, a.PV);
diff --git a/psba_amd/csrc/kernels_schur.hip b/psba_amd/csrc/kernels_schur.hip
--- a/psba_amd/csrc/kernels_schur.hip
+++ b/psba_amd/csrc/kernels_schur.hip
@@ -212,7 +212,11 @@
   int w = blockIdx.x;
   if ((p.nWg & 7) == 0) w = (blockIdx.x & 7) * (p.nWg >> 3) + (blockIdx.x >> 3);
   const SchurWg wg = p.wg[w];
+  double cx[CAM_PRE];
+  CamFoldLane cl;
+  if (p.cam.part) cl = cam_fold_issue(p.cam, cx);
   for (int t = tid; t < BLK_STRIDE * wg.nblk; t += SCHUR_THREADS) sPart[t] = 0.0;
+  if (p.cam.part) cam_fold_finish(p.cam, cl, cx);
   __syncthreads();
 
 #ifdef PSBA_BUILD_EXPERIMENTS
@@ -317,7 +321,11 @@
   int w = blockIdx.x;
   if ((p.nWg & 7) == 0) w = (blockIdx.x & 7) * (p.nWg >> 3) + (blockIdx.x >> 3);
   const SchurWg wg = p.wg[w];
+  double cx[CAM_PRE];
+  CamFoldLane cl;
+  if (p.cam.part) cl = cam_fold_issue(p.cam, cx);
   for (int t = tid; t < BLK_STRIDE * wg.nblk; t += RUN_THREADS) sPart[t] = 0.0;
+  if (p.cam.part) cam_fold_finish(p.cam, cl, cx);
   __syncthreads();
   double acc[36];
 #pragma unroll
@@ -685,6 +693,22 @@
   for (int b = 0; b < 21; b++) {
     a.diag_grp[b] = h->h_diaggrp[b];
     a.diag_pos[b] = h->h_diagpos[b];
+  }
+  const char *m = getenv("PSBA_SCHUR_MODE");
+  const int mode = m ? atoi(m) : 0;
+  a.cam.part = nullptr;
+  if (h->cam_pend_U == (double *)h->U && (h->schur_runs || mode <= 0 || dump || h->schur_pairs)) {
+    a.cam.part = h->campart;
+    a.cam.U = h->cam_slab_U;
+    a.cam.ga = h->cam_slab_ga;
+    a.cam.coeff = h->cam_slab_coeff;
+    a.cam.coeff_g = h->cam_slab_coeff_g;
+    a.cam.nPart = h->cam_slab_n;
+    a.cam.nC = d.nC;
+    h->cam_pend_U = nullptr;
+  } else if (h->cam_pend_U == (double *)h->U) {
+    const int rc = cam_sums_flush(h);
+    if (rc != PSBA_OK) return rc;
   }
   SchurReduceArgs r;
   r.slab = h->slab;
@@ -728,8 +752,6 @@
     ProfScope pp(h, pair ? PSBA_K_SCHUR : -1);
     {
       ProfScope ps(h, pair ? -1 : PSBA_K_SCHUR);
-      const char *m = getenv("PSBA_SCHUR_MODE");
-      const int mode = m ? atoi(m) : 0;
       const dim3 G(h->nWg), B(SCHUR_THREADS);
       bool launched = false;
       if (h->schur_runs) {
@@ -800,6 +822,11 @@
   h->try_id++;
   h->diag_done = false;
   h->packed_pending = false;
+  if (h->cam_pend_U == (double *)h->U &&
+      !(h->solver != PSBA_SOLVER_PCG && h->ring_nWg == 0 && h->nGroups > 0 && !getenv("PSBA_SCHUR_ATOMIC"))) {
+    const int rc = cam_sums_flush(h);
+    if (rc != PSBA_OK) return rc;
+  }
   if (h->solver == PSBA_SOLVER_PCG) {
     if (dump) return fail(h, PSBA_E_INVALID, "the sba_func.h mirror verbs need the dense S: PSBA_SOLVER_DENSE");
     return launch_schur_sparse(h, mu);
diff --git a/psba_amd/csrc/psba_api.cpp b/psba_amd/csrc/psba_api.cpp
--- a/psba_amd/csrc/psba_api.cpp
+++ b/psba_amd/csrc/psba_api.cpp
@@ -55,12 +55,20 @@
     if (!(h)) return PSBA_E_INVALID;      \
     (void)hipSetDevice((h)->device);      \
   } while (0)
-#define CHECK_H(h)                                                         \
+#define CHECK_H_TRYPATH(h)                                                 \
   do {                                                                     \
     CHECK_H_NOJOIN(h);                                                     \
     if ((h)->scal_side) {                                                  \
       (void)hipStreamWaitEvent((h)->stream, (h)->scal_event, 0);           \
       (h)->scal_side = false;                                              \
+    }                                                                      \
+  } while (0)
+#define CHECK_H(h)                                                         \
+  do {                                                                     \
+    CHECK_H_TRYPATH(h);                                                    \
+    if ((h)->cam_pend_U) {                                                 \
+      const int rc_cam__ = psba::cam_sums_flush(h);                        \
+      if (rc_cam__ < 0) return rc_cam__;                                   \
     }                                                                      \
   } while (0)
 #define NEED(h, cond, what)                                             \
@@ -317,7 +325,7 @@
 }
 
 int psba_set_fixed(psba_handle h, const unsigned char *fixed_cams, const unsigned char *fixed_pts) {
-  CHECK_H(h);
+  CHECK_H_TRYPATH(h);
   TRY(lens_settable(h, __func__));
   const int nC = h->d.nC, nP = h->d.nP;
   int nfc = 0, nfp = 0;
@@ -355,6 +363,7 @@
   h->has_fixed = nfc > 0 || nfp > 0;
   h->struct_only = nfc == nC;
   h->try_shortcut = false;
+  h->cam_pend_U = nullptr;
   lens_changed(h);
   return PSBA_OK;
 }
@@ -822,8 +831,9 @@
 }
 
 int psba_reset_params(psba_handle h) {
-  CHECK_H(h);
-  NEED(h, h->uploaded, "no problem uploaded");
+  CHECK_H_TRYPATH(h);
+  NEED(h, h->uploaded, "no problem uploaded");
+  h->cam_pend_U = nullptr;
   PSBA_HIP(h, hipMemcpyAsync(h->cams[h->cur], h->params0, sizeof(double) * h->d.nA, hipMemcpyDeviceToDevice,
                              h->stream));
   PSBA_HIP(h, hipMemcpyAsync(h->pts[h->cur], h->params0 + h->d.nA, sizeof(double) * h->d.nB,
@@ -873,12 +883,12 @@
 }
 
 int psba_linearize(psba_handle h, double coeff, double coeff_g) {
-  CHECK_H(h);
+  CHECK_H_TRYPATH(h);
   NEED(h, h->uploaded, "no problem uploaded");
   if (!(h->lin_is_ahead && coeff == h->coeff && coeff_g == h->coeff_g)) {
     h->coeff = coeff;
     h->coeff_g = coeff_g;
-    TRY(launch_linearize(h, false));
+    TRY(launch_linearize(h, false, false, false, true));
   }
   h->lin_is_ahead = false;
   h->ahead = false;
@@ -888,6 +898,7 @@
 }
 
 static int enqueue_max_diag(psba_ctx *h) {
+  TRY(cam_sums_flush(h));
   if (h->comm) {
     double *tmp = h->dp;
     PSBA_HIP(h, hipMemcpyAsync(tmp, h->U, sizeof(double) * 36 * h->d.nC, hipMemcpyDeviceToDevice,
@@ -933,7 +944,7 @@
 }
 
 int psba_schur_assemble(psba_handle h, double mu) {
-  CHECK_H(h);
+  CHECK_H_TRYPATH(h);
   NEED(h, h->linearized, "psba_linearize first");
   h->mu = mu;
   h->try_shortcut = h->struct_only && h->cnp == 6 && !getenv("PSBA_FIXED_NO_SHORTCUT");
@@ -965,7 +976,7 @@
 }
 
 int psba_schur_reduce(psba_handle h) {
-  CHECK_H(h);
+  CHECK_H_TRYPATH(h);
   NEED(h, h->assembled, "psba_schur_assemble first");
   if (!h->comm || h->try_shortcut) return PSBA_OK;
   ProfScope ps(h, PSBA_K_ALLREDUCE);
@@ -974,7 +985,7 @@
 }
 
 int psba_schur_solve(psba_handle h) {
-  CHECK_H(h);
+  CHECK_H_TRYPATH(h);
   NEED(h, h->assembled, "psba_schur_assemble first");
   if (h->try_shortcut) {
     h->assembled = false;
@@ -1012,7 +1023,7 @@
 }
 
 int psba_backsub_async(psba_handle h, double mu) {
-  CHECK_H(h);
+  CHECK_H_TRYPATH(h);
   NEED(h, h->solved, "psba_schur_solve first");
   TRY(launch_backsub(h, mu, false));
   hipStream_t s = h->stream;
@@ -1039,7 +1050,7 @@
   NEED(h, h->backsub_pending || h->backsubbed, "psba_backsub_async / psba_backsub first");
   const bool carry = h->backsub_pending && h->publish_deferred;
   if (carry) h->pub_seq += 1.0;
-  TRY(launch_linearize(h, false, true, carry));
+  TRY(launch_linearize(h, false, true, carry, true));
   if (carry) {
     h->publish_deferred = false;
     h->publish_in_k1 = true;
@@ -1098,7 +1109,7 @@
 }
 
 int psba_accept(psba_handle h) {
-  CHECK_H(h);
+  CHECK_H_TRYPATH(h);
   NEED(h, h->backsubbed, "psba_backsub first");
   h->cur = 1 - h->cur;
   h->linearized = h->assembled = h->solved = h->backsubbed = false;
@@ -1110,6 +1121,21 @@
   }
   h->lin_is_ahead = h->ahead;
   h->ahead = false;
+  return PSBA_OK;
+}
+
+int psba_cam_sums_repend(psba_handle h) {
+  CHECK_H(h);
+  NEED(h, h->linearized, "psba_linearize first");
+  NEED(h, h->cam_slab_U && h->cam_slab_U == (double *)h->U, "the camera slabs do not belong to the current linearization");
+  NEED(h, !h->has_fixed, "a fixed mask is set: k_fixed_diag runs behind the camera sums");
+  h->cam_pend_U = h->cam_slab_U;
+  return PSBA_OK;
+}
+
+int psba_cam_sums_pending(psba_handle h, int *pending) {
+  CHECK_H_NOJOIN(h);
+  if (pending) *pending = h->cam_pend_U ? 1 : 0;
   return PSBA_OK;
 }
 
diff --git a/psba_amd/csrc/psba_internal.h b/psba_amd/csrc/psba_internal.h
--- a/psba_amd/csrc/psba_internal.h
+++ b/psba_amd/csrc/psba_internal.h
@@ -170,6 +170,10 @@
   bool scal_side = false;
   psba::DevBuf<double> campart;
   int nPart = 0;
+  double *cam_slab_U = nullptr, *cam_slab_ga = nullptr;
+  double *cam_pend_U = nullptr;
+  int cam_slab_n = 0;
+  double cam_slab_coeff = 1.0, cam_slab_coeff_g = 1.0;
   bool cam_global = false;
   psba::DevBuf<double> camacc;
   psba::DevBuf<int> cam_obs;
@@ -320,7 +324,8 @@
   ~ProfScope();
 };
 
-int launch_linearize(psba_ctx *h, bool dump, bool ahead = false, bool publish = false);
+int launch_linearize(psba_ctx *h, bool dump, bool ahead = false, bool publish = false, bool may_defer = false);
+int cam_sums_flush(psba_ctx *h);
 int launch_residual(psba_ctx *h, int which, double *ex_out_dev, double *s_out_dev = nullptr);
 int launch_max_diag(psba_ctx *h);
 int build_schur_plan(psba_ctx *h, int nCams, int nPts, int nObs, const int *iidx, const int *jidx,
diff --git a/psba_amd/csrc/schur_lds_args.h b/psba_amd/csrc/schur_lds_args.h
--- a/psba_amd/csrc/schur_lds_args.h
+++ b/psba_amd/csrc/schur_lds_args.h
@@ -1,4 +1,5 @@
 #pragma once
+#include "cam_sums.h"
 #include "psba_internal.h"
 
 namespace psba {
@@ -17,6 +18,7 @@
   int nWg, try_id;
   double *diag0;
   int diag_grp[21], diag_pos[21];
+  CamFoldArgs cam;
 };
 
 }
```

Result: faster. 2133 M-obs/s (median of 6 runs) (+1.4%).
